# taintpro98/rnd-semantic-segmentation

Hardware: AMD Instinct MI355X
Metric: train images/sec at 769x769 bf16 (DeepLabV2-ResNet101 + ASPP) (higher is better)
Workload: dtype bf16; 1 GPU; train_src.py DeepLabV2-R101 bf16, 769x769 synthetic Cityscapes crops, batch 8 per GPU, 1xMI355X; global_batch=8, parallelism=dp1, weights=formula (synthetic), hip_graph_replay=False

## Files before the change

### include/mi355seg.h

```cpp
#ifndef MI355SEG_H
#define MI355SEG_H

#include <stddef.h>
#include <stdint.h>

#ifdef __cplusplus
extern "C" {
#endif

#define MI355SEG_VERSION 100

#define MI_OK 0
#define MI_EINVAL (-22)
#define MI_ENOMEM (-12)
#define MI_EHIP (-5)

#define MI_EPI_SCALE_BIAS 1
#define MI_EPI_RESIDUAL 2
#define MI_EPI_RELU 4
#define MI_EPI_MASK 8
#define MI_EPI_OUT_F32 16
#define MI_EPI_ZSPLIT 32
#define MI_EPI_WRITE_MASK 64
#define MI_EPI_LEAKY 256
// ... 57 lines not shown
                          const float* scale_o, int accumulate, int out_map, int ncls, size_t dw_elems,
                          void* workspace, size_t workspace_bytes, void* job, void* stream);
int mi_conv_wgrad_reduce(const void* jobs, int n, void* stream);

#define MI_ASPP_NRATES 4
#define MI_ASPP_ZGW 20
#define MI_ASPP_KPAD 704
int mi_aspp_pack_fwd(const float* w4 , void* wall_bf16, int C, int K, void* stream);
int mi_aspp_pack_dgrad(const float* w4, void* wallT_bf16, int C, int K, void* stream);
int mi_aspp_col2im(const float* z , const float* bias4 , float* low ,
                   int B, int H, int W, int K, const int* rates4 , void* stream);
int mi_aspp_im2col(const float* dlow , void* g_bf16 ,
                   int B, int H, int W, int K, const int* rates4 , void* stream);
size_t mi_colsum_workspace(int M, int N);
int mi_aspp_bias_grad(const float* dlow, float* dbias4 , int M, int K, int accumulate,
                      void* workspace, size_t workspace_bytes, void* stream);

int mi_upsample_ac_fwd(const float* low, float* up, int B, int h, int w, int K, int H, int W, void* stream);
int mi_upsample_ac_bwd(const float* dup, float* dlow, int B, int h, int w, int K, int H, int W, void* stream);

size_t mi_ce_workspace(int B, int H, int W);
int mi_softmax_ce_fwd(const float* logits, const int64_t* labels, float* loss_out ,
                      int B, int K, int H, int W, int ignore_index, void* workspace, size_t workspace_bytes, void* stream);
int mi_softmax_ce_bwd(const float* logits, const int64_t* labels, const float* loss_out, float* dlogits,
                      int B, int K, int H, int W, int ignore_index, float grad_scale, void* stream);

size_t mi_upsample_ce_workspace(int B, int h, int w, int K, int H, int W);
int mi_upsample_ce(const float* low, const int64_t* labels, float* loss_out , float* dlow,
                   int B, int h, int w, int K, int H, int W, int ignore_index, float grad_scale,
                   void* workspace, size_t workspace_bytes, void* stream);

int mi_upsample_ce_ex(const float* low, const int64_t* labels, float* loss_out , float* dlow,
                      int B, int h, int w, int K, int H, int W, int ignore_index, float grad_scale, int align_corners,
                      void* workspace, size_t workspace_bytes, void* stream);

int mi_upsample_ce_w(const float* low, const int64_t* labels, const float* class_weights , float* loss_out , float* dlow,
                     int B, int h, int w, int K, int H, int W, int ignore_index, float label_smoothing, float grad_scale, int align_corners,
                     void* workspace, size_t workspace_bytes, void* stream);

int mi_upsample_ce_focal(const float* low, const int64_t* labels, const float* class_weights , float* loss_out , float* dlow,
                         int B, int h, int w, int K, int H, int W, int ignore_index, float gamma, float grad_scale, int align_corners,
                         void* workspace, size_t workspace_bytes, void* stream);

size_t mi_upsample_ce_ohem_workspace(int B, int h, int w, int K, int H, int W);
int mi_upsample_ce_ohem(const float* low, const int64_t* labels, float* loss_out , float* dlow, float* prob ,
                        int B, int h, int w, int K, int H, int W, int ignore_index, float thresh, int64_t min_kept, float grad_scale,
                        int align_corners, void* workspace, size_t workspace_bytes, void* stream);

#define MI_GDL_SQUARE 0
#define MI_GDL_IDENTITY 1
#define MI_GDL_SQRT 2
size_t mi_upsample_gdl_workspace(int B, int h, int w, int K, int H, int W);
int mi_upsample_gdl(const float* low, const int64_t* labels, float* loss_out , float* dlow, float* sums ,
                    int B, int h, int w, int K, int H, int W, int ignore_index, int weight_type, float eps, float grad_scale,
                    int align_corners, void* workspace, size_t workspace_bytes, void* stream);

size_t mi_upsample_tversky_bce_workspace(int B, int h, int w, int H, int W);
int mi_upsample_tversky_bce(const float* low, const float* mask, float* loss_out , float* dlow, float* sums ,
                            int B, int h, int w, int H, int W, float alpha, float eps, float w_tversky, float w_bce, float grad_scale,
                            int align_corners, void* workspace, size_t workspace_bytes, void* stream);

int mi_upsample_softmax(const float* low, float* probs, uint8_t* pred, int B, int h, int w, int K, int H, int W, void* stream);

typedef struct { const float* low; int h, w; int mirror; } MiProbSource;
int mi_upsample_softmax_multi(const MiProbSource* src, int n, float* probs, int K, int H, int W, float div_a, float div_b, void* stream);

int mi_upsample_predict_score(const MiProbSource* src, int n, int K, int H, int W, float div_a, float div_b, const int64_t* labels,
                              int ignore_index, float threshold, uint8_t* pred, uint8_t* pseudo, int64_t* counts, void* stream);

int mi_upsample_predict_score_cw(const MiProbSource* src, int n, int K, int H, int W, float div_a, float div_b, const int64_t* labels,
                                 int ignore_index, const float* class_threshold, uint8_t* pred, uint8_t* pseudo, int64_t* counts, int bins,
                                 int64_t* hist, void* stream);

#define MI_POLYP_SUMS 24
#define MI_POLYP_COUNTS 4
size_t mi_polyp_score_workspace(int B, int h, int w, int H, int W);
int mi_polyp_score(const float* low, const int64_t* labels, int B, int h, int w, int H, int W, int64_t* hist, double* sums, int64_t* counts,
                   float* prob, uint8_t* pred, void* workspace, size_t workspace_bytes, void* stream);

int mi_image_resize_ac(const float* x, float* out, int B, int C, int H, int W, int Ho, int Wo, int with_mirror, void* stream);

int mi_sgd_step(float* p, const float* g, float* buf, size_t n, float lr, float momentum, float weight_decay, void* stream);
int mi_sgd_step_dev(float* p, const float* g, float* buf, size_t n, const float* hyper , void* stream);

int mi_stem_pool_fwd(const void* y, const float* scale, const float* shift, void* pool, uint8_t* idx,
                     int B, int Hc, int Wc, int C, int Hp, int Wp, void* stream);
int mi_stem_pool_bwd(const void* dpool, const uint8_t* idx, const float* scale, void* dy,
                     int B, int Hc, int Wc, int C, int Hp, int Wp, void* stream);
int mi_stem_im2col(const void* x_bf16_nhwc, void* col_bf16, int B, int H, int W, int Ho, int Wo, int ncols, void* stream);
int mi_stem_direct_enabled(void);
int mi_stem_pack_image(const void* x, int x_is_bf16_nhwc, void* x4, int B, int H, int W, void* stream);
int mi_stem_conv_fwd(const void* x4, const float* w, void* wpack, void* y, int B, int H, int W, int O, int Ho, int Wo, void* stream);
size_t mi_stem_conv_wgrad_workspace(int B, int Ho, int Wo);
int mi_stem_conv_wgrad(const void* dy, const void* x4, float* dw, int B, int H, int W, int O, int Ho, int Wo, void* workspace,
                       size_t workspace_bytes, void* stream);

int mi_bias_grad_bf16(const void* dy_bf16, float* db, int M, int N, int accumulate,
                      void* workspace , size_t workspace_bytes, void* stream);
size_t mi_upsample_softce_workspace(int B, int h, int w, int K, int H, int W);
int mi_upsample_softce(const float* seg_low, float inv_temperature, float clip, const float* d_low, int ldD, int domain,
                       float* loss_out, float* dd_low, int B, int h, int w, int K, int H, int W, float grad_scale,
                       void* workspace, size_t workspace_bytes, void* stream);
size_t mi_upsample_softce_2grid_workspace(int B, int hd, int wd, int K, int H, int W);
int mi_upsample_softce_2grid(const float* seg_low, int hs, int ws, int seg_align_corners, float inv_temperature, float clip,
                             const float* d_low, int hd, int wd, int ldD, int d_align_corners, int domain, float grad_scale,
                             float* loss_out, float* dd_low, int B, int K, int H, int W, void* workspace, size_t workspace_bytes, void* stream);
int mi_adam_step(float* p, const float* g, float* exp_avg, float* exp_avg_sq, size_t n, float lr, float beta1, float beta2,
                 float eps, int step, void* stream);
int mi_adam_step_clamped(float* p, float* g, float* exp_avg, float* exp_avg_sq, size_t n, float lr, float beta1, float beta2,
                         float eps, int step, float grad_clamp, void* stream);

int mi_adam_step_dev(float* p, float* g, float* exp_avg, float* exp_avg_sq, size_t n, const float* hyper , void* stream);

int mi_pack_weight_f32(const float* w_oihw, float* wp, int O, int I, int ksize, void* stream);
int mi_conv_f32(const float* a, const float* wp, float* out, int B, int Ha, int Wa, int Ca, int Ho, int Wo, int N,
                int ksize, int stride, int pad, int dil, const float* scale, const float* bias, const float* res,
                int flags, void* stream);
int mi_stem_f32(const float* x_nchw, const float* w, const float* scale, const float* shift, float* y_nhwc,
                int B, int H, int W, void* stream);
int mi_maxpool_f32(const float* y_nhwc, float* pool_nhwc, int B, int Hc, int Wc, int C, void* stream);

int mi_comm_unique_id(void* id128 );
int mi_comm_init_rank(void** comm , int nranks, const void* id128 , int rank);
int mi_comm_destroy(void* comm);
int mi_allreduce_bucket(void* ptr, size_t count, int dtype, int average, void* comm, void* stream);

int mi_relu_mask(const void* x_bf16, const void* msk, void* y_bf16, size_t n, int bits, void* stream);
int mi_frozen_bn_fold(const float* w, const float* b, const float* mean, const float* var, float* scale, float* shift, int n, void* stream);

size_t mi_bn_workspace(long M, int C);
int mi_bn_colsum(const void* y_bf16, const float* mean, long M, int C, float* out, void* workspace, size_t workspace_bytes, void* stream);
int mi_bn_colsum2(const void* y_bf16, const float* pilot, long M, int C, float* s1, float* s2, void* workspace, size_t workspace_bytes, void* stream);
size_t mi_conv_gemm_stats_workspace(long M, int N);
int mi_conv_gemm_stats(const void* a, const void* wp, void* out, int B, int Ha, int Wa, int Ca, int Ho, int Wo, int N, int ksize, int stride, int pad,
                       int dil, const float* pilot, float* sums, void* workspace, size_t workspace_bytes, const float* gamma, const float* beta,
                       float* running_mean, float* running_var, long long* num_batches_tracked, float momentum, float eps, float* out4, void* stream);
int mi_bn_finalize(const float* s1, const float* s2, const float* pilot, double count, const float* gamma, const float* beta, float* running_mean,
                   float* running_var, long long* num_batches_tracked, float momentum, float eps, float* out4, int C, void* stream);
int mi_bn_apply(const void* y_bf16, const float* mean, const float* scale, const float* beta, const void* res_bf16, void* out_bf16,
                void* mask_out, int relu, long M, int C, void* stream);
int mi_bn_bwd_colsums(const void* g_bf16, const void* y_bf16, const float* mean, const float* invstd, const void* relu_bits, long M, int C,
                      float* dbeta, float* dgamma, void* workspace, size_t workspace_bytes, void* stream);
int mi_bn_bwd_apply(const void* g_bf16, const void* y_bf16, const float* mean, const float* invstd, const float* gamma, const float* dbeta,
                    const float* dgamma, float inv_count, const void* relu_bits, void* dy_bf16, long M, int C, void* stream);

size_t mi_structure_loss_workspace(int B, int H, int W);
int mi_structure_loss(const float* pred, const float* mask, int B, int H, int W, float* out, float* grad, float grad_scale,
                      void* workspace, size_t workspace_bytes, void* stream);

size_t mi_gconv_pack_elems(int O, int I, int kh, int kw);
int mi_gconv_pack_multi(const float* wflat, void* wp_bf16, void* wpt_bf16, const int64_t* table_dev, int n_desc, int total_blocks, void* stream);
size_t mi_gconv_stats_elems(int B, int Ho, int Wo, int N);
int mi_gconv(const void* a, long lda, const void* wp, void* out, long ldo, int B, int Ha, int Wa, int Ca, int Ho, int Wo, int N,
             int kh, int kw, int sh, int sw, int ph, int pw, int dh, int dw, int mode, const float* bias, float* stats, int out_f32,
             void* stream);
#define MI_GROUTE_GCONV 0
#define MI_GROUTE_GCONV3 1
#define MI_GROUTE_LEN 10
int mi_gconv_route(const void* a, long lda, const void* out, long ldo, int B, int Ha, int Wa, int Ca, int Ho, int Wo, int N, int kh, int kw, int sh, int sw,
                   int ph, int pw, int dh, int dw, int mode, int out_f32, int bn_finalize, int* route);
size_t mi_gconv_wgrad_workspace(int B, int Ho, int Wo, int O, int I, int kh, int kw);
int mi_gconv_wgrad(const void* dy, long ldy, const void* x, long ldx, float* dw, int B, int Ha, int Wa, int I, int Ho, int Wo, int O,
                   int kh, int kw, int sh, int sw, int ph, int pw, int dh, int dw_, int accumulate, void* workspace, size_t workspace_bytes, unsigned* tickets, int n_tickets,
                   void* stream);
typedef struct MiWgradJob {
    const void* dy; long ldy; const void* x; long ldx; float* dw;
    int B, Ha, Wa, I, Ho, Wo, O, kh, kw, sh, sw, ph, pw, dh, dw_, accumulate;
} MiWgradJob;
size_t mi_gconv_wgrad_multi_table_bytes(int n);
size_t mi_gconv_wgrad_multi_workspace(const MiWgradJob* jobs, int n);
int mi_gconv_wgrad_multi(const MiWgradJob* jobs, int n, void* table_dev, size_t table_bytes, void* workspace, size_t workspace_bytes, void* stream);
#define MI_GWROUTE_LEN 6
int mi_gconv_wgrad_route(const void* dy, long ldy, const void* x, long ldx, int B, int Ha, int Wa, int I, int Ho, int Wo, int O, int kh, int kw, int sh, int sw,
                         int ph, int pw, int dh, int dw_, int multi, int* route);
int mi_gbn_finalize(const float* partials, int tiles, int C, long count, const float* gamma, const float* beta, float* running_mean, float* running_var,
                    float momentum, float eps, float* mean_out, float* invstd_out, float* scale_out, float* shift_out, void* stream);
int mi_gbn_fold(const float* gamma, const float* beta, const float* running_mean, const float* running_var, float eps, float* scale, float* shift, int C,
                void* stream);
int mi_gbn_apply(const void* y, long ldy, const float* scale, const float* shift, const void* add, long ldadd, void* out, long ldo, int out_f32, long M, int C,
                 int relu, void* stream);
int mi_gbn_apply_multi(const void* y, long ldy, const float* scale, const float* shift, const void* add, long ldadd, void* out, long ldo, long M, int C, int relu,
                       int n_extra, const int* c0, const int* c1, void* const* dst, const long* ldd, const void* const* add2, const long* lda2, void* stream);
size_t mi_gcolsum_workspace(long M, int C);
int mi_gbn_bwd_sums(const void* g, long ldg, int g_f32, const void* y, long ldy, const void* mask, long ldm, int mask_f32, const float* mean,
                    const float* invstd, long M, int C, float* dbeta, float* dgamma, int accumulate, void* workspace, size_t workspace_bytes, void* stream);
int mi_gbn_bwd_apply(const void* g, long ldg, int g_f32, const void* y, long ldy, const void* mask, long ldm, int mask_f32, const float* mean,
                     const float* invstd, const float* gamma, const float* dbeta, const float* dgamma, float inv_count, void* dy, long lddy, long M, int C,
                     void* stream);
int mi_gbinary(int op, int dtype, const void* a, long lda, const void* b, long ldb, void* out, long ldo, long M, int C, void* stream);
int mi_gavgpool(const void* x, long ldx, void* out, long ldo, int B, int H, int W, int C, int Ho, int Wo, int k, int stride, int pad, int include_pad,
                int backward, void* stream);
int mi_gmaxpool(const void* x, long ldx, void* out, long ldo, uint8_t* idx, int B, int H, int W, int C, int Ho, int Wo, int k, int stride, int pad, int backward,
                void* stream);
size_t mi_gce_workspace(long M);
int mi_gce(const float* logits, long ld, const int64_t* labels, long M, int K, int ignore_index, float* loss_out, float* dlogits, long ldd, float grad_scale,
           void* workspace, size_t workspace_bytes, void* stream);
int mi_gresize(const void* x, long ldx, void* out, long ldo, int f32, int B, int H, int W, int C, int Ho, int Wo, int align_corners, float scale_h, float scale_w,
               int backward, void* stream);
#define MI_GRESIZE_FWD 0
#define MI_GRESIZE_FWD8 1
#define MI_GRESIZE_BWD_GATHER 2
#define MI_GRESIZE_BWD_WAVE 3
#define MI_GRESIZE_BWD_PIX 4
#define MI_GRESIZE_BWD8 5
#define MI_GRESIZE_ROUTE_LEN 3
int mi_gresize_route(const void* x, long ldx, const void* out, long ldo, int f32, int B, int H, int W, int C, int Ho, int Wo, int align_corners, float scale_h,
                     float scale_w, int backward, int* route);
int mi_gra_fwd(const float* gate, const void* feat, long ldfeat, void* out, long ldo, long M, int C, void* stream);
int mi_gra_bwd(const float* gate, const void* feat, long ldfeat, const void* dy, long lddy, void* dfeat, long lddf, float* dgate, long M, int C, void* stream);

// ... 74 lines not shown
```

### rnd_semantic_segmentation_amd/_lib.py

```python
import ctypes
import os

import torch
from ctypes import c_char_p, c_double, c_float, c_int, c_long, c_size_t, c_void_p

_HERE = os.path.dirname(os.path.abspath(__file__))
LIB_PATH = os.environ.get("MI355SEG_LIB") or os.path.join(_HERE, "libmi355seg.so")
HEADER_PATH = os.path.join(os.path.dirname(_HERE), "include", "mi355seg.h")

P, I, F, Z, L = c_void_p, c_int, c_float, c_size_t, c_long

SIGNATURES = {
    "mi_version": (I, []),
    "mi_last_error": (c_char_p, []),
    "mi_pack_weight_fwd": (I, [P, P, I, I, I, P]),
    "mi_pack_weight_dgrad": (I, [P, P, P, I, I, I, P]),
    "mi_pack_weights_multi": (I, [P, P, P, P, P, I, I, P]),
    "mi_conv_gemm": (I, [P, P, P] + [I] * 12 + [P, P, P, P, P, I, I, F, P]),
    "mi_conv_gemm_route": (I, [I] * 10),
    "mi_conv_gemm_plan": (I, [I] * 13 + [P]),
    "mi_conv_gemm_pp": (I, [P, P, P] + [I] * 12 + [P, P, P, P, P, I, I, F, I, P]),
    "mi_conv_chain": (I, [P] * 6 + [L, I, I, I] + [P] * 8 + [I, I, P]),
    "mi_conv_wgrad_workspace": (Z, [I] * 6),
    "mi_conv_wgrad_route": (I, [I] * 12),
    "mi_conv_wgrad_plan": (I, [I] * 13 + [P]),
    "mi_conv_wgrad": (I, [P, P, P] + [I] * 11 + [P, I, I, I, Z, P, Z, P]),
    "mi_conv_wgrad_job_bytes": (Z, []),
    "mi_conv_wgrad_partial": (I, [P, P, P] + [I] * 11 + [P, I, I, I, Z, P, Z, P, P]),
    "mi_conv_wgrad_reduce": (I, [P, I, P]),
    "mi_aspp_pack_fwd": (I, [P, P, I, I, P]),
    "mi_aspp_pack_dgrad": (I, [P, P, I, I, P]),
    "mi_aspp_col2im": (I, [P, P, P, I, I, I, I, P, P]),
    "mi_aspp_im2col": (I, [P, P, I, I, I, I, P, P]),
    "mi_colsum_workspace": (Z, [I, I]),
    "mi_aspp_bias_grad": (I, [P, P, I, I, I, P, Z, P]),
    "mi_upsample_ac_fwd": (I, [P, P] + [I] * 6 + [P]),
    "mi_upsample_ac_bwd": (I, [P, P] + [I] * 6 + [P]),
    "mi_ce_workspace": (Z, [I, I, I]),
    "mi_softmax_ce_fwd": (I, [P, P, P, I, I, I, I, I, P, Z, P]),
    "mi_softmax_ce_bwd": (I, [P, P, P, P, I, I, I, I, I, F, P]),
    "mi_upsample_ce_workspace": (Z, [I] * 6),
    "mi_upsample_ce": (I, [P, P, P, P] + [I] * 7 + [F, P, Z, P]),
    "mi_upsample_ce_ex": (I, [P, P, P, P] + [I] * 7 + [F, I, P, Z, P]),
    "mi_upsample_ce_w": (I, [P, P, P, P, P] + [I] * 7 + [F, F, I, P, Z, P]),
    "mi_upsample_ce_focal": (I, [P, P, P, P, P] + [I] * 7 + [F, F, I, P, Z, P]),
    "mi_upsample_ce_ohem_workspace": (Z, [I] * 6),
    "mi_upsample_ce_ohem": (I, [P, P, P, P, P] + [I] * 7 + [F, L, F, I, P, Z, P]),
    "mi_upsample_gdl_workspace": (Z, [I] * 6),
    "mi_upsample_gdl": (I, [P, P, P, P, P] + [I] * 8 + [F, F, I, P, Z, P]),
    "mi_upsample_tversky_bce_workspace": (Z, [I] * 5),
    "mi_upsample_tversky_bce": (I, [P, P, P, P, P] + [I] * 5 + [F] * 5 + [I, P, Z, P]),
    "mi_upsample_softmax": (I, [P, P, P] + [I] * 6 + [P]),
    "mi_upsample_softmax_multi": (I, [P, I, P, I, I, I, F, F, P]),
    "mi_upsample_predict_score": (I, [P, I, I, I, I, F, F, P, I, F, P, P, P, P]),
    "mi_upsample_predict_score_cw": (I, [P, I, I, I, I, F, F, P, I, P, P, P, P, I, P, P]),
    "mi_polyp_score_workspace": (Z, [I] * 5),
    "mi_polyp_score": (I, [P, P] + [I] * 5 + [P, P, P, P, P, P, Z, P]),
    "mi_image_resize_ac": (I, [P, P] + [I] * 7 + [P]),
    "mi_stem_pool_fwd": (I, [P, P, P, P, P] + [I] * 6 + [P]),
    "mi_stem_pool_bwd": (I, [P, P, P, P] + [I] * 6 + [P]),
    "mi_stem_im2col": (I, [P, P] + [I] * 6 + [P]),
    "mi_stem_direct_enabled": (I, []),
    "mi_stem_pack_image": (I, [P, I, P, I, I, I, P]),
    "mi_stem_conv_fwd": (I, [P, P, P, P] + [I] * 6 + [P]),
    "mi_stem_conv_wgrad_workspace": (Z, [I] * 3),
    "mi_stem_conv_wgrad": (I, [P, P, P] + [I] * 6 + [P, Z, P]),
    "mi_bias_grad_bf16": (I, [P, P, I, I, I, P, Z, P]),
    "mi_upsample_softce_workspace": (Z, [I] * 6),
    "mi_upsample_softce": (I, [P, F, F, P, I, I, P, P] + [I] * 6 + [F, P, Z, P]),
    "mi_upsample_softce_2grid_workspace": (Z, [I] * 6),
    "mi_upsample_softce_2grid": (I, [P, I, I, I, F, F, P, I, I, I, I, I, F, P, P, I, I, I, I, P, Z, P]),
    "mi_adam_step": (I, [P, P, P, P, Z, F, F, F, F, I, P]),
    "mi_adam_step_clamped": (I, [P, P, P, P, Z, F, F, F, F, I, F, P]),
    "mi_adam_step_dev": (I, [P, P, P, P, Z, P, P]),
    "mi_sgd_step": (I, [P, P, P, Z, F, F, F, P]),
    "mi_sgd_step_dev": (I, [P, P, P, Z, P, P]),
    "mi_pack_weight_f32": (I, [P, P, I, I, I, P]),
    "mi_conv_f32": (I, [P, P, P] + [I] * 11 + [P, P, P, I, P]),
    "mi_stem_f32": (I, [P, P, P, P, P, I, I, I, P]),
    "mi_maxpool_f32": (I, [P, P, I, I, I, I, P]),
    "mi_comm_unique_id": (I, [P]),
    "mi_comm_init_rank": (I, [P, I, P, I]),
    "mi_comm_destroy": (I, [P]),
    "mi_allreduce_bucket": (I, [P, Z, I, I, P, P]),
    "mi_relu_mask": (I, [P, P, P, Z, I, P]),
    "mi_frozen_bn_fold": (I, [P, P, P, P, P, P, I, P]),
    "mi_structure_loss_workspace": (Z, [I, I, I]),
    "mi_structure_loss": (I, [P, P, I, I, I, P, P, F, P, Z, P]),
    "mi_bn_workspace": (Z, [L, I]),
    "mi_bn_colsum": (I, [P, P, L, I, P, P, Z, P]),
    "mi_bn_apply": (I, [P, P, P, P, P, P, P, I, L, I, P]),
    "mi_bn_colsum2": (I, [P, P, L, I, P, P, P, Z, P]),
    "mi_conv_gemm_stats_workspace": (Z, [L, I]),
    "mi_conv_gemm_stats": (I, [P, P, P] + [I] * 11 + [P, P, P, Z, P, P, P, P, P, F, F, P, P]),
    "mi_bn_finalize": (I, [P, P, P, c_double, P, P, P, P, P, F, F, P, I, P]),
    "mi_bn_bwd_colsums": (I, [P, P, P, P, P, L, I, P, P, P, Z, P]),
    "mi_bn_bwd_apply": (I, [P, P, P, P, P, P, P, F, P, P, L, I, P]),
    "mi_gconv_pack_elems": (Z, [I] * 4),
    "mi_gconv_pack_multi": (I, [P, P, P, P, I, I, P]),
    "mi_gconv_stats_elems": (Z, [I] * 4),
    "mi_gconv": (I, [P, L, P, P, L] + [I] * 16 + [P, P, I, P]),
    "mi_gconv_route": (I, [P, L, P, L] + [I] * 18 + [P]),
    "mi_gconv_wgrad_workspace": (Z, [I] * 7),
    "mi_gconv_wgrad": (I, [P, L, P, L, P] + [I] * 16 + [P, Z, P, I, P]),
    "mi_gconv_wgrad_multi_table_bytes": (Z, [I]),
    "mi_gconv_wgrad_multi_workspace": (Z, [P, I]),
    "mi_gconv_wgrad_multi": (I, [P, I, P, Z, P, Z, P]),
    "mi_gconv_wgrad_route": (I, [P, L, P, L] + [I] * 16 + [P]),
    "mi_gbn_finalize": (I, [P, I, I, L, P, P, P, P, F, F, P, P, P, P, P]),
    "mi_gbn_fold": (I, [P, P, P, P, F, P, P, I, P]),
    "mi_gbn_apply": (I, [P, L, P, P, P, L, P, L, I, L, I, I, P]),
    "mi_gbn_apply_multi": (I, [P, L, P, P, P, L, P, L, L, I, I, I, P, P, P, P, P, P, P]),
    "mi_gcolsum_workspace": (Z, [L, I]),
    "mi_gbn_bwd_sums": (I, [P, L, I, P, L, P, L, I, P, P, L, I, P, P, I, P, Z, P]),
    "mi_gbn_bwd_apply": (I, [P, L, I, P, L, P, L, I, P, P, P, P, P, F, P, L, L, I, P]),
    "mi_gbinary": (I, [I, I, P, L, P, L, P, L, L, I, P]),
    "mi_gavgpool": (I, [P, L, P, L] + [I] * 11 + [P]),
    "mi_gmaxpool": (I, [P, L, P, L, P] + [I] * 10 + [P]),
    "mi_gce_workspace": (Z, [L]),
    "mi_gce": (I, [P, L, P, L, I, I, P, P, L, F, P, Z, P]),
    "mi_gresize": (I, [P, L, P, L, I] + [I] * 7 + [F, F, I, P]),
    "mi_gresize_route": (I, [P, L, P, L, I] + [I] * 7 + [F, F, I, P]),
    "mi_gra_fwd": (I, [P, P, L, P, L, L, I, P]),
    "mi_gra_bwd": (I, [P, P, L, P, L, P, L, P, L, I, P]),
    "mi_gdwconv_stats_elems": (Z, [I] * 4),
    "mi_gdwconv": (I, [P, L, P, P, P, L] + [I] * 8 + [P, P]),
    "mi_gdwconv_dgrad": (I, [P, L, P, P, L] + [I] * 8 + [P]),
    "mi_gdwconv_wgrad_workspace": (Z, [I] * 4),
    "mi_gdwconv_wgrad": (I, [P, L, P, L, P, P] + [I] * 9 + [P, Z, P]),
    "mi_gcca_fwd": (I, [P, L, P, L, P, L, P, P, L] + [I] * 5 + [P]),
    "mi_gcca_bwd": (I, [P, L, P, L, P, L, P, P, L, P, P, L, P, L, P, L] + [I] * 5 + [P]),
    "mi_ggate": (I, [P, L, P, L, P, L, P, L, P, L, L, I, P]),
    "mi_gconv_bn_inlaunch_max_pixels": (I, []),
    "mi_gconv_bn": (I, [P, L, P, P, L] + [I] * 15 + [P, P, P, P, P, P, P, F, F, P, P]),
    "mi_gconv_f32": (I, [P, L, P, P, P, P, P, L, I, P, L] + [I] * 15 + [P]),
    "mi_gpool_f32": (I, [P, L, P, L] + [I] * 10 + [P]),
    "mi_gdwconv_f32": (I, [P, L, P, P, P, P, I, P, L] + [I] * 8 + [P]),
    "mi_gcca_f32": (I, [P, L, P, L, P, L, P, L] + [I] * 5 + [P]),
    "mi_gpoint_f32": (I, [I, P, L, P, L, P, P, I, P, L, L, I, P]),
    "mi_augment_batch": (I, [P, P, I, I, I, I, I, P, P, P]),
    "mi_augment_pra_batch": (I, [P, P, I, I, I, P, P, P]),
}

class MiProbSource(ctypes.Structure):
    _fields_ = [("low", c_void_p), ("h", c_int), ("w", c_int), ("mirror", c_int)]


class MiAugSample(ctypes.Structure):
    _fields_ = [("img", c_void_p), ("lab", c_void_p), ("jit", c_void_p), ("tmp", c_void_p), ("hcoef", c_void_p), ("hbound", c_void_p),
                ("vcoef", c_void_p), ("vbound", c_void_p), ("grey_sum", ctypes.c_uint64),
                ("H", c_int), ("W", c_int), ("sh", c_int), ("sw", c_int), ("hk", c_int), ("vk", c_int),
                ("off_y", c_int), ("off_x", c_int), ("flip", c_int),
                ("cy0", c_int), ("cy1", c_int), ("cx0", c_int), ("cx1", c_int), ("ry0", c_int), ("ry1", c_int), ("rx0", c_int), ("rx1", c_int),
                ("tstride", c_int), ("lab_sh", c_int), ("lab_sw", c_int),
                ("n_ops", c_int), ("op", c_int * 4), ("hue_shift", c_int), ("factor", c_float * 4),
                ("to_bgr255", c_int), ("mean", c_float * 3), ("std", c_float * 3), ("lab_table", ctypes.c_uint8 * 256)]


class MiPraSample(ctypes.Structure):
# ... 35 lines not shown
```

### rnd_semantic_segmentation_amd/csrc/elementwise.hip

```cpp
#include "mi_common.h"
#include <mutex>
#include <stdlib.h>
#include <string.h>

static thread_local char g_err[512] = "";

int mi_set_error(int code, const char* fmt, ...) {
    va_list ap;
    va_start(ap, fmt);
    vsnprintf(g_err, sizeof(g_err), fmt, ap);
    va_end(ap);
    return code;
}

const MiSwitches& mi_sw() {
    static MiSwitches sw;
    static std::once_flag once;
    std::call_once(once, [] {
        auto env = [](const char* name, int dflt) {
            const char* e = getenv(name);
            return e ? atoi(e) : dflt;
        };
        sw.igemm_staged = env("MI_IGEMM_STAGED", 1);
        sw.igemm_pp = env("MI_IGEMM_PP", 1);
        sw.igemm_pp_mink = env("MI_IGEMM_PP_MINK", 512);
        sw.igemm_mt = env("MI_IGEMM_MT", 0);
        sw.igemm_bn = env("MI_IGEMM_BN", 0);
        sw.igemm_pref = env("MI_IGEMM_PREF", 1);
        sw.pp_korder = env("MI_IGEMM_PP_KORDER", 1);
#ifdef MI_EXPERIMENTS
        sw.pp_loop = env("MI_IGEMM_PP_LOOP", 0);
#else
        sw.pp_loop = 0;
#endif
        sw.igemm_pw = env("MI_IGEMM_PW", 0);
        sw.wgrad_q3_slots = env("MI_WGRAD_Q3_SLOTS", 512);
        sw.wgrad_q3_slots_beside = env("MI_WGRAD_Q3_SLOTS_BESIDE", 448);
        sw.wgrad_s4_slots = env("MI_WGRAD_S4_SLOTS", 512);
        if (sw.wgrad_s4_slots < 64) sw.wgrad_s4_slots = 512;
        sw.wgrad_ti256 = env("MI_WGRAD_TI256", -1);
        sw.wgrad_p3 = env("MI_WGRAD_P3", 0);
        sw.wgrad_q3 = env("MI_WGRAD_Q3", 1);
        sw.wgrad_s4 = env("MI_WGRAD_S4", 1);
        sw.gconv_bn128 = env("MI_GCONV_BN128", 0);
        sw.gconv_kc = env("MI_GCONV_KC", 0);
        sw.gconv_remap = env("MI_GCONV_REMAP", 1);
        sw.gconv_ks2_wgs = env("MI_GCONV_KS2_WGS", 320);
        sw.gconv_kc32_wgs = env("MI_GCONV_KC32_WGS", 1536);
        sw.gconv_bn32_wgs = env("MI_GCONV_BN32_WGS", 256);
        sw.gconv_bn_any = env("MI_GCONV_BN_ANY", 1);
        sw.gconv_bn_c = env("MI_GCONV_BN_C", 64);
        sw.gconv_bn_force = env("MI_GCONV_BN_FORCE", 0);
        sw.gconv3_wgs = env("MI_GCONV3_WGS", 512);
#ifdef MI_EXPERIMENTS
        sw.gconv_dbg = env("MI_GC_DBG", 0);
        sw.gw_dbg = env("MI_GW_DBG", 0);
#else
        sw.gconv_dbg = sw.gw_dbg = 0;
#endif
        sw.gwm_steps = env("MI_GWM_STEPS", 48);
        if (sw.gwm_steps < 1) sw.gwm_steps = 48;
        sw.gwm_fused3 = env("MI_GWM_FUSED3", 1);
        sw.gwgrad3 = env("MI_GWGRAD3", 1);
#ifdef MI_EXPERIMENTS
        sw.p3_dbg = env("MI_P3_DBG", 0);
#else
        sw.p3_dbg = 0;
#endif
        sw.pp_trace_wg = env("MI_PP_TRACE_WG", 0);
        sw.stem_direct = env("MI_STEM_DIRECT", 1);
        sw.stem_wgrad_splits = env("MI_STEM_WGRAD_SPLITS", 512);
        if (sw.stem_wgrad_splits < 1 || sw.stem_wgrad_splits > 4096) sw.stem_wgrad_splits = 512;
    });
    return sw;
}

extern "C" int mi_version(void) { return MI355SEG_VERSION; }
extern "C" const char* mi_last_error(void) { return g_err; }

namespace {

__global__ void sgd_kernel(float* __restrict__ p, const float* __restrict__ g, float* __restrict__ buf, size_t n4, size_t n, float lr,
                           float mu, float wd) {
    const size_t stride = (size_t)gridDim.x * blockDim.x;
    for (size_t i = (size_t)blockIdx.x * blockDim.x + threadIdx.x; i < n4; i += stride) {
        f32x4 pv = reinterpret_cast<f32x4*>(p)[i];
        const f32x4 gv = reinterpret_cast<const f32x4*>(g)[i];
        f32x4 bv = reinterpret_cast<f32x4*>(buf)[i];
#pragma unroll
        for (int e = 0; e < 4; ++e) {
            const float gg = gv[e] + wd * pv[e];
            bv[e] = mu * bv[e] + gg;
            pv[e] = pv[e] - lr * bv[e];
        }
        reinterpret_cast<f32x4*>(buf)[i] = bv;
        reinterpret_cast<f32x4*>(p)[i] = pv;
    }
    if (blockIdx.x == 0 && threadIdx.x < (n & 3)) {
        const size_t i = (n4 << 2) + threadIdx.x;
        const float gg = g[i] + wd * p[i];
        const float b = mu * buf[i] + gg;
        buf[i] = b;
        p[i] = p[i] - lr * b;
    }
}

__global__ void sgd_dev_kernel(float* __restrict__ p, const float* __restrict__ g, float* __restrict__ buf, size_t n4, size_t n,
                               const float* __restrict__ hyper) {
    const float lr = hyper[0], mu = hyper[1], wd = hyper[2];
    const size_t stride = (size_t)gridDim.x * blockDim.x;
    for (size_t i = (size_t)blockIdx.x * blockDim.x + threadIdx.x; i < n4; i += stride) {
        f32x4 pv = reinterpret_cast<f32x4*>(p)[i];
        const f32x4 gv = reinterpret_cast<const f32x4*>(g)[i];
        f32x4 bv = reinterpret_cast<f32x4*>(buf)[i];
#pragma unroll
        for (int e = 0; e < 4; ++e) {
            const float gg = gv[e] + wd * pv[e];
            bv[e] = mu * bv[e] + gg;
            pv[e] = pv[e] - lr * bv[e];
        }
        reinterpret_cast<f32x4*>(buf)[i] = bv;
        reinterpret_cast<f32x4*>(p)[i] = pv;
    }
    if (blockIdx.x == 0 && threadIdx.x < (n & 3)) {
        const size_t i = (n4 << 2) + threadIdx.x;
        const float gg = g[i] + wd * p[i];
        const float b = mu * buf[i] + gg;
        buf[i] = b;
        p[i] = p[i] - lr * b;
    }
}

__global__ void relu_mask_kernel(const bf16x8* __restrict__ x, const bf16x8* __restrict__ m, bf16x8* __restrict__ y, size_t n8) {
    const size_t stride = (size_t)gridDim.x * blockDim.x;
    for (size_t i = (size_t)blockIdx.x * blockDim.x + threadIdx.x; i < n8; i += stride) {
        const bf16x8 xv = x[i], mv = m[i];
        bf16x8 o;
#pragma unroll
        for (int e = 0; e < 8; ++e) o[e] = ((float)mv[e] > 0.f) ? xv[e] : (__bf16)0.f;
        y[i] = o;
    }
}

__global__ void bn_fold_kernel(const float* w, const float* b, const float* mean, const float* var, float* scale, float* shift, int n) {
    const int i = blockIdx.x * blockDim.x + threadIdx.x;
    if (i >= n) return;
    const float s = w[i] * (1.0f / sqrtf(var[i]));
    scale[i] = s;
    shift[i] = b[i] - mean[i] * s;
}


extern "C" int mi_sgd_step(float* p, const float* g, float* buf, size_t n, float lr, float momentum, float weight_decay, void* stream) {
    MI_REQUIRE(p && g && buf && n > 0, "mi_sgd_step: bad argument");
    MI_REQUIRE(mi_aligned16(p) && mi_aligned16(g) && mi_aligned16(buf), "mi_sgd_step: flat buffers must be 16-byte aligned");
    const size_t n4 = n >> 2;
    size_t blocks = (n4 + 255) / 256;
    if (blocks > 2048) blocks = 2048;
    if (blocks < 1) blocks = 1;
    hipLaunchKernelGGL(sgd_kernel, dim3((unsigned)blocks), dim3(256), 0, (hipStream_t)stream, p, g, buf, n4, n, lr, momentum, weight_decay);
    MI_CHECK_LAUNCH("mi_sgd_step");
    return MI_OK;
}

extern "C" int mi_sgd_step_dev(float* p, const float* g, float* buf, size_t n, const float* hyper, void* stream) {
    MI_REQUIRE(p && g && buf && hyper && n > 0, "mi_sgd_step_dev: bad argument");
    MI_REQUIRE(mi_aligned16(p) && mi_aligned16(g) && mi_aligned16(buf), "mi_sgd_step_dev: flat buffers must be 16-byte aligned");
    const size_t n4 = n >> 2;
    size_t blocks = (n4 + 255) / 256;
    if (blocks > 2048) blocks = 2048;
    if (blocks < 1) blocks = 1;
    hipLaunchKernelGGL(sgd_dev_kernel, dim3((unsigned)blocks), dim3(256), 0, (hipStream_t)stream, p, g, buf, n4, n, hyper);
    MI_CHECK_LAUNCH("mi_sgd_step_dev");
    return MI_OK;
}

__global__ void relu_mask_bits_kernel(const bf16x8* __restrict__ x, const uint8_t* __restrict__ m, bf16x8* __restrict__ y, size_t n8) {
    const size_t stride = (size_t)gridDim.x * blockDim.x;
    for (size_t i = (size_t)blockIdx.x * blockDim.x + threadIdx.x; i < n8; i += stride) {
        const bf16x8 xv = x[i];
        const unsigned bits = m[i];
        bf16x8 o;
#pragma unroll
        for (int e = 0; e < 8; ++e) o[e] = ((bits >> e) & 1u) ? xv[e] : (__bf16)0.f;
        y[i] = o;
    }
}

}

extern "C" int mi_relu_mask(const void* x, const void* msk, void* y, size_t n, int bits, void* stream) {
    MI_REQUIRE(x && msk && y && n > 0 && n % 8 == 0, "mi_relu_mask: bad argument (n %% 8 == 0)");
    MI_REQUIRE(mi_aligned16(x) && mi_aligned16(y) && (bits || mi_aligned16(msk)), "mi_relu_mask: alignment");
    const size_t n8 = n >> 3;
    size_t blocks = (n8 + 255) / 256;
    if (blocks > 2048) blocks = 2048;
    if (bits) {
        MI_REQUIRE(n % 16 == 0, "mi_relu_mask: packed mask needs n %% 16 == 0");
        hipLaunchKernelGGL(relu_mask_bits_kernel, dim3((unsigned)blocks), dim3(256), 0, (hipStream_t)stream, (const bf16x8*)x,
                           (const uint8_t*)msk, (bf16x8*)y, n8);
        MI_CHECK_LAUNCH("mi_relu_mask (bits)");
        return MI_OK;
    }
    hipLaunchKernelGGL(relu_mask_kernel, dim3((unsigned)blocks), dim3(256), 0, (hipStream_t)stream, (const bf16x8*)x, (const bf16x8*)msk,
                       (bf16x8*)y, n8);
    MI_CHECK_LAUNCH("mi_relu_mask");
    return MI_OK;
}

extern "C" int mi_frozen_bn_fold(const float* w, const float* b, const float* mean, const float* var, float* scale, float* shift, int n,
                                 void* stream) {
    MI_REQUIRE(w && b && mean && var && scale && shift && n > 0, "mi_frozen_bn_fold: bad argument");
    hipLaunchKernelGGL(bn_fold_kernel, dim3((n + 255) / 256), dim3(256), 0, (hipStream_t)stream, w, b, mean, var, scale, shift, n);
    MI_CHECK_LAUNCH("mi_frozen_bn_fold");
    return MI_OK;
}
```

### rnd_semantic_segmentation_amd/csrc/mi_common.h

```cpp
#pragma once
#include <hip/hip_runtime.h>
#include <stdint.h>
#include <stdio.h>
#include <stdarg.h>
#include <atomic>
#include "../../include/mi355seg.h"

typedef __attribute__((ext_vector_type(8))) __bf16 bf16x8;
typedef __attribute__((ext_vector_type(4))) __bf16 bf16x4;
typedef __attribute__((ext_vector_type(2))) __bf16 bf16x2;
typedef __attribute__((ext_vector_type(4))) float f32x4;
typedef __attribute__((ext_vector_type(4))) short s16x4;
typedef __attribute__((ext_vector_type(4))) uint32_t u32x4;
typedef __attribute__((ext_vector_type(2))) uint32_t u32x2;

int mi_set_error(int code, const char* fmt, ...);

struct MiSwitches {
    int igemm_staged;
    int igemm_pp;
    int igemm_pp_mink;
    int igemm_mt;
    int igemm_bn;
    int igemm_pref;
    int pp_korder;
    int pp_loop;
    int igemm_pw;
    int wgrad_q3_slots;
    int wgrad_q3_slots_beside;
    int wgrad_s4_slots;
    int wgrad_ti256;
    int wgrad_p3;
    int wgrad_q3;
    int wgrad_s4;
    int gconv_bn128;
    int gconv_kc;
    int gconv_remap;
    int gconv_ks2_wgs;
    int gconv_kc32_wgs;
    int gconv_bn32_wgs;
    int gconv_bn_any;
    int gconv_bn_c;
    int gconv_bn_force;
    int gconv3_wgs;
    int gconv_dbg;
    int gw_dbg;
    int gwm_steps;
    int gwm_fused3;
    int gwgrad3;
    int p3_dbg;
    int pp_trace_wg;
    int stem_wgrad_splits;
    int stem_direct;
};
const MiSwitches& mi_sw();

struct MiConvStats {
    float* partial;
    const float* pilot;
    int nparts;
};
int mi_conv_gemm_impl(const void* a, const void* wp, void* out, int B, int Ha, int Wa, int Ca, int Ho, int Wo, int N, int ksize, int stride, int pad,
                      int dil, int gather_mode, const float* scale, const float* bias, const void* res, const void* msk, void* mask_out, int flags,
                      int zgw, float alpha, void* stream, MiConvStats* st);
int mi_conv_gemm_pp_impl(const void* a, const void* wp, void* out, int B, int Ha, int Wa, int Ca, int Ho, int Wo, int N, int ksize, int stride, int pad,
                         int dil, int gather_mode, const float* scale, const float* bias, const void* res, const void* msk, void* mask_out, int flags,
                         int zgw, float alpha, int mtg, void* stream, MiConvStats* st);
struct MiConvPlan {
    int kernel;
    int mt;
    int bn;
    int unit, pref, staged;
    int epi;
    int korder;
    int m_tiles, n_tiles;
    int slots, rounds;
};
int mi_conv_plan(int B, int Ha, int Wa, int Ca, int Ho, int Wo, int N, int ksize, int stride, int pad, int dil, int flags, int pp_mtg, MiConvPlan* pl);
struct MiBnFinal {
    const float* pilot;
    double count;
    const float* gamma;
    const float* beta;
    float* running_mean;
    float* running_var;
    long long* num_batches_tracked;
    float momentum, eps;
    float* out4;
};
size_t mi_bn_reduce_tmp_floats(int nparts, int C);
int mi_bn_reduce_partials(const float* partial, int nparts, int C, float* tmp, float* s1, float* s2, const MiBnFinal* fin, void* stream);

#define MI_REQUIRE(cond, ...)                         \
    do {                                              \
        if (!(cond)) return mi_set_error(MI_EINVAL, __VA_ARGS__); \
    } while (0)

#define MI_CHECK_LAUNCH(name)                                                      \
    do {                                                                           \
        hipError_t e_ = hipGetLastError();                                         \
        if (e_ != hipSuccess) return mi_set_error(MI_EHIP, "%s: %s", name, hipGetErrorString(e_)); \
    } while (0)

static inline void mi_allow_dynamic_lds(const void* kern, int bytes, std::atomic<uint64_t>& done) {
    int dev = 0;
    (void)hipGetDevice(&dev);
    const uint64_t bit = 1ull << (dev & 63);
    if (done.load(std::memory_order_acquire) & bit) return;
    (void)hipFuncSetAttribute(kern, hipFuncAttributeMaxDynamicSharedMemorySize, bytes);
    done.fetch_or(bit, std::memory_order_release);
}
constexpr int MI_LDS_MAX = 160 * 1024;

static inline bool mi_aligned16(const void* p) { return (reinterpret_cast<uintptr_t>(p) & 15) == 0; }

__device__ __forceinline__ int mi_xcd_remap(int bid, int nwg) {
    const int q = nwg >> 3, r = nwg & 7, xcd = bid & 7;
    const int base = (xcd < r) ? xcd * (q + 1) : r * (q + 1) + (xcd - r) * q;
    return base + (bid >> 3);
}

__device__ __forceinline__ float mi_bf16_to_f32(__bf16 v) { return (float)v; }

struct MiBnFin {
    float mean, invstd, scale, shift;
    double var;
};
__device__ __forceinline__ MiBnFin mi_bn_finalize_channel(double s1, double s2, double count, float eps, float gamma, float beta) {
    MiBnFin r;
    const double mean = s1 / count;
    double var = __dsub_rn(s2 / count, __dmul_rn(mean, mean));
    if (var < 0.0) var = 0.0;
    r.var = var;
    r.mean = (float)mean;
    r.invstd = (float)(1.0 / sqrt(__dadd_rn(var, (double)eps)));
    r.scale = __fmul_rn(gamma, r.invstd);
// ... 43 lines not shown
```

### rnd_semantic_segmentation_amd/csrc/stem_direct.hip

```cpp
#include "mi_common.h"

namespace {

constexpr int SD_TW = 64;
constexpr int SD_ROWPX = 136;
constexpr int SD_ROWB = SD_ROWPX * 8;
constexpr int SD_FWD_TH = 8;
constexpr int SD_FWD_ROWS = 2 * SD_FWD_TH + 5;
constexpr int SD_KB = 6;
constexpr int SD_WG_TH = 4;
constexpr int SD_WG_ROWS = 2 * SD_WG_TH + 5;
constexpr int SD_DYROWB = SD_TW * 128;
constexpr int SD_PART = 64 * 7 * 32;

__global__ __launch_bounds__(256) void stem_pack_f32_kernel(const float* __restrict__ x, bf16x4* __restrict__ x4, long HW, int B) {
    const int b = blockIdx.y;
    const float* img = x + (long)b * 3 * HW;
    const long p0 = (long)blockIdx.x * 1024 + threadIdx.x;
    float v[4][3];
#pragma unroll
    for (int j = 0; j < 4; ++j) {
        const long p = p0 + j * 256;
#pragma unroll
        for (int c = 0; c < 3; ++c) v[j][c] = p < HW ? img[c * HW + p] : 0.f;
    }
#pragma unroll
    for (int j = 0; j < 4; ++j) {
        const long p = p0 + j * 256;
        if (p < HW) {
            bf16x4 o;
            o[0] = (__bf16)v[j][0];
            o[1] = (__bf16)v[j][1];
            o[2] = (__bf16)v[j][2];
            o[3] = (__bf16)0.f;
            x4[(long)b * HW + p] = o;
        }
    }
}

__global__ __launch_bounds__(256) void stem_pack_bf16_kernel(const __bf16* __restrict__ x, bf16x4* __restrict__ x4, long n) {
    const long p = (long)blockIdx.x * 256 + threadIdx.x;
    if (p >= n) return;
    bf16x4 o;
    o[0] = x[p * 3];
    o[1] = x[p * 3 + 1];
    o[2] = x[p * 3 + 2];
    o[3] = (__bf16)0.f;
    x4[p] = o;
}

__global__ __launch_bounds__(256) void stem_pack_weight_kernel(const float* __restrict__ w, __bf16* __restrict__ wp) {
    const int i = blockIdx.x * 256 + threadIdx.x;
    if (i >= SD_KB * 64 * 32) return;
    const int kk = i & 31, o = (i >> 5) & 63, kb = i >> 11;
    const int k = kb * 32 + kk;
    wp[i] = (__bf16)(k < 147 ? w[o * 147 + k] : 0.f);
}

template <int ROWS>
struct ImageRows {
    static constexpr int N = (ROWS * SD_ROWPX + 255) / 256;
    uint2 v[N];
    __device__ __forceinline__ void load(const uint2* __restrict__ img, int h0, int c0, int H, int W, int tid) {
#pragma unroll
        for (int j = 0; j < N; ++j) {
            const int i = tid + j * 256;
            const int r = i / SD_ROWPX, c = i - r * SD_ROWPX;
            const int h = h0 + r, w = c0 + c;
            v[j] = make_uint2(0u, 0u);
            if (i < ROWS * SD_ROWPX && (unsigned)h < (unsigned)H && (unsigned)w < (unsigned)W) v[j] = img[(long)h * W + w];
        }
    }
    __device__ __forceinline__ void store(uint2* sx, int tid) const {
#pragma unroll
        for (int j = 0; j < N; ++j) {
            const int i = tid + j * 256;
            if (i < ROWS * SD_ROWPX) sx[i] = v[j];
        }
    }
};

struct StemFwdParams {
    const uint2* x4;
    const bf16x8* wp;
    __bf16* y;
    int B, H, W, Ho, Wo, tiles_x, tiles_y;
};

__global__ __launch_bounds__(256, 2) void stem_direct_fwd_kernel(StemFwdParams p) {
    __shared__ __attribute__((aligned(16))) uint2 sx[SD_FWD_ROWS * SD_ROWPX];
    const int tid = threadIdx.x, lane = tid & 63;
    const int wave = __builtin_amdgcn_readfirstlane(tid >> 6);
    const int tx = blockIdx.x % p.tiles_x, ty = (blockIdx.x / p.tiles_x) % p.tiles_y, b = blockIdx.x / (p.tiles_x * p.tiles_y);
    const int wo0 = tx * SD_TW, ho0 = ty * SD_FWD_TH;
    ImageRows<SD_FWD_ROWS> rows;
    rows.load(p.x4 + (long)b * p.H * p.W, 2 * ho0 - 3, 2 * wo0 - 3, p.H, p.W, tid);

    const int col = lane & 15, q = lane >> 4;
    bf16x8 wf[SD_KB - 1][4];
#pragma unroll
    for (int kb = 0; kb < SD_KB - 1; ++kb)
#pragma unroll
        for (int ot = 0; ot < 4; ++ot) wf[kb][ot] = p.wp[(kb * 64 + (col >> 2) * 16 + ot * 4 + (col & 3)) * 4 + q];
    int off[SD_KB - 1][8];
#pragma unroll
    for (int kb = 0; kb < SD_KB - 1; ++kb)
#pragma unroll
        for (int j = 0; j < 8; ++j) {
            const int k = kb * 32 + q * 8 + j;
            const int c = k / 49, r = k - c * 49, ky = r / 7, kx = r - ky * 7;
            off[kb][j] = k < 147 ? ky * SD_ROWB + kx * 8 + c * 2 : -1;
        }
    rows.store(sx, tid);
    __syncthreads();

    const char* sxb = reinterpret_cast<const char*>(sx);
    bf16x8 zero8;
#pragma unroll
    for (int e = 0; e < 8; ++e) zero8[e] = (__bf16)0.f;
    for (int rr = wave * 2; rr < wave * 2 + 2; ++rr) {
        const int ho = ho0 + rr;
        if (ho >= p.Ho) break;
        for (int mt = 0; mt < 4; ++mt) {
            if (wo0 + mt * 16 >= p.Wo) break;
            const char* win = sxb + 2 * rr * SD_ROWB + 16 * (mt * 16 + col);
            f32x4 acc[4];
#pragma unroll
            for (int ot = 0; ot < 4; ++ot) acc[ot] = f32x4{0.f, 0.f, 0.f, 0.f};
#pragma unroll
            for (int kb = 0; kb < SD_KB - 1; ++kb) {
                union { bf16x8 v; unsigned short s[8]; } f;
#pragma unroll
                for (int j = 0; j < 8; ++j) {
                    if (kb < 4) {
                        f.s[j] = *reinterpret_cast<const unsigned short*>(win + off[kb][j]);
                    } else {
                        const unsigned short v = *reinterpret_cast<const unsigned short*>(win + (off[kb][j] < 0 ? 0 : off[kb][j]));
                        f.s[j] = off[kb][j] < 0 ? (unsigned short)0 : v;
                    }
                }
#pragma unroll
                for (int ot = 0; ot < 4; ++ot) acc[ot] = __builtin_amdgcn_mfma_f32_16x16x32_bf16(wf[kb][ot], f.v, acc[ot], 0, 0, 0);
            }
#pragma unroll
            for (int ot = 0; ot < 4; ++ot) acc[ot] = __builtin_amdgcn_mfma_f32_16x16x32_bf16(zero8, zero8, acc[ot], 0, 0, 0);
            const int wo = wo0 + mt * 16 + col;
            if (wo < p.Wo) {
                bf16x8 o0, o1;
#pragma unroll
                for (int e = 0; e < 4; ++e) {
                    o0[e] = (__bf16)acc[0][e];
                    o0[4 + e] = (__bf16)acc[1][e];
                    o1[e] = (__bf16)acc[2][e];
                    o1[4 + e] = (__bf16)acc[3][e];
                }
                bf16x8* dst = reinterpret_cast<bf16x8*>(p.y + (((long)b * p.Ho + ho) * p.Wo + wo) * 64 + q * 16);
                dst[0] = o0;
                dst[1] = o1;
            }
        }
    }
}

template <int OFF>
__device__ __forceinline__ s16x4 sd_tr_read(unsigned lds_addr) {
    s16x4 v;
    asm volatile("ds_read_b64_tr_b16 %0, %1 offset:%2" : "=v"(v) : "v"(lds_addr), "n"(OFF));
    return v;
}

__device__ __forceinline__ unsigned sd_lds_address(const void* generic_ptr_into_lds) {
    return (unsigned)(uintptr_t)((__attribute__((address_space(3))) const char*)generic_ptr_into_lds);
}

struct StemWgradParams {
    const uint2* x4;
    const bf16x8* dy;
    float* part;
    int B, H, W, Ho, Wo, tiles_x, tiles_y, tiles, S;
};

__global__ __launch_bounds__(256, 2) void stem_direct_wgrad_kernel(StemWgradParams p) {
    __shared__ __attribute__((aligned(16))) uint2 sx[SD_WG_ROWS * SD_ROWPX];
    __shared__ __attribute__((aligned(16))) bf16x8 sdy[SD_WG_TH * SD_TW * 8];
    const int tid = threadIdx.x, lane = tid & 63;
    const int wave = __builtin_amdgcn_readfirstlane(tid >> 6);
    const int kt = wave & 1, oh = wave >> 1;
    const int s = blockIdx.x;
    const int t_begin = (int)((long)s * p.tiles / p.S), t_end = (int)((long)(s + 1) * p.tiles / p.S);
    const int g = lane >> 4, rq = (lane & 15) >> 2, pc = lane & 3;
    const int pix = 4 * g + rq;
    const unsigned sx_base = sd_lds_address(sx) + 16 * pix + 32 * kt + 8 * pc;
    const unsigned sdy_base = sd_lds_address(sdy) + 128 * pix + 8 * (pc & 1);
    const int sw = pix & 7;

    f32x4 acc[2][7];
#pragma unroll
    for (int a = 0; a < 2; ++a)
#pragma unroll
        for (int ky = 0; ky < 7; ++ky) acc[a][ky] = f32x4{0.f, 0.f, 0.f, 0.f};

    ImageRows<SD_WG_ROWS> nx;
    bf16x8 ny[8];
    auto load_tile = [&](int t) {
        const int tx = t % p.tiles_x, ty = (t / p.tiles_x) % p.tiles_y, b = t / (p.tiles_x * p.tiles_y);
        const int wo0 = tx * SD_TW, ho0 = ty * SD_WG_TH;
        nx.load(p.x4 + (long)b * p.H * p.W, 2 * ho0 - 3, 2 * wo0 - 3, p.H, p.W, tid);
#pragma unroll
        for (int j = 0; j < 8; ++j) {
            const int i = tid + j * 256;
            const int c = i & 7, P = (i >> 3) & 63, rr = i >> 9;
            const int ho = ho0 + rr, wo = wo0 + P;
#pragma unroll
            for (int e = 0; e < 8; ++e) ny[j][e] = (__bf16)0.f;
            if (ho < p.Ho && wo < p.Wo) ny[j] = p.dy[(((long)b * p.Ho + ho) * p.Wo + wo) * 8 + c];
        }
    };
    load_tile(t_begin);
    for (int t = t_begin; t < t_end; ++t) {
        const int tx = t % p.tiles_x, ty = (t / p.tiles_x) % p.tiles_y;
        const int wo0 = tx * SD_TW, ho0 = ty * SD_WG_TH;
        __syncthreads();
        nx.store(sx, tid);
#pragma unroll
        for (int j = 0; j < 8; ++j) {
            const int i = tid + j * 256;
            const int c = i & 7, P = (i >> 3) & 63, rr = i >> 9;
            sdy[(rr * SD_TW + P) * 8 + (c ^ (P & 7))] = ny[j];
        }
        __syncthreads();
        if (t + 1 < t_end) load_tile(t + 1);
        const int nrows = min(SD_WG_TH, p.Ho - ho0);
        for (int rr = 0; rr < nrows; ++rr) {
#pragma unroll
            for (int step = 0; step < 2; ++step) {
                const int left = p.Wo - (wo0 + step * 32);
                if (left <= 0) break;
                union { bf16x8 v; s16x4 h[2]; uint64_t d[2]; } yf[2], xf[7];
                const unsigned ya = sdy_base + rr * SD_DYROWB + step * 32 * 128;
#pragma unroll
                for (int a = 0; a < 2; ++a) {
                    const unsigned addr = ya + (((2 * (oh * 2 + a) + (pc >> 1)) ^ sw) << 4);
                    yf[a].h[0] = sd_tr_read<0>(addr);
                    yf[a].h[1] = sd_tr_read<16 * 128>(addr);
                }
                const unsigned xa = sx_base + 2 * rr * SD_ROWB + step * 32 * 16;
#pragma unroll
                for (int ky = 0; ky < 7; ++ky) {
                    xf[ky].h[0] = sd_tr_read<0>(xa + ky * SD_ROWB);
                    xf[ky].h[1] = sd_tr_read<16 * 16>(xa + ky * SD_ROWB);
                }
                asm volatile("s_waitcnt lgkmcnt(0)" ::: "memory");
                __builtin_amdgcn_sched_barrier(0);
                if (left < 32) {
#pragma unroll
                    for (int h = 0; h < 2; ++h) {
                        const int nv = left - (16 * h + 4 * g);
                        const uint64_t m = nv >= 4 ? ~0ull : (nv <= 0 ? 0ull : ((1ull << (16 * nv)) - 1ull));
#pragma unroll
                        for (int ky = 0; ky < 7; ++ky) xf[ky].d[h] &= m;
                    }
                }
#pragma unroll
                for (int ky = 0; ky < 7; ++ky)
#pragma unroll
                    for (int a = 0; a < 2; ++a) acc[a][ky] = __builtin_amdgcn_mfma_f32_16x16x32_bf16(yf[a].v, xf[ky].v, acc[a][ky], 0, 0, 0);
            }
        }
    }
    float* dst = p.part + (long)s * SD_PART;
#pragma unroll
    for (int a = 0; a < 2; ++a)
#pragma unroll
        for (int ky = 0; ky < 7; ++ky)
#pragma unroll
            for (int e = 0; e < 4; ++e) dst[(((oh * 2 + a) * 16 + 4 * g + e) * 7 + ky) * 32 + kt * 16 + (lane & 15)] = acc[a][ky][e];
}

__global__ __launch_bounds__(256) void stem_direct_wgrad_reduce_kernel(const float* __restrict__ part, float* __restrict__ dw, int S) {
    const int i = blockIdx.x * 256 + threadIdx.x;
    if (i >= SD_PART) return;
    const int k = i & 31, ky = (i >> 5) % 7, o = i / 224;
    const int kx = k >> 2, c = k & 3;
    if (c == 3 || kx >= 7) return;
    float sum = 0.f;
    int s = 0;
    for (; s + 64 <= S; s += 64) {
        float v[64];
#pragma unroll
        for (int j = 0; j < 64; ++j) v[j] = part[(long)(s + j) * SD_PART + i];
#pragma unroll
        for (int j = 0; j < 64; ++j) sum += v[j];
    }
    for (; s < S; ++s) sum += part[(long)s * SD_PART + i];
    dw[((o * 3 + c) * 7 + ky) * 7 + kx] = sum;
}

int stem_wgrad_splits(int B, int Ho, int Wo) {
    const long tiles = (long)B * ((Ho + SD_WG_TH - 1) / SD_WG_TH) * ((Wo + SD_TW - 1) / SD_TW);
    const long slots = mi_sw().stem_wgrad_splits;
    return (int)(tiles < slots ? tiles : slots);
}

const char* stem_direct_geometry(int B, int H, int W, int Ho, int Wo) {
    if (B <= 0 || H <= 0 || W <= 0) return "B, H, W must be positive";
    if (Ho != (H + 6 - 7) / 2 + 1 || Wo != (W + 6 - 7) / 2 + 1) return "output size must be that of a 7x7/2/3 conv";
    if ((long)B * H * W * 4 >= (1l << 31) || (long)B * Ho * Wo * 64 >= (1l << 31)) return "tensor exceeds the 32-bit offset range";
    return nullptr;
}

}

extern "C" int mi_stem_direct_enabled(void) { return mi_sw().stem_direct != 0; }

extern "C" int mi_stem_pack_image(const void* x, int x_is_bf16_nhwc, void* x4, int B, int H, int W, void* stream) {
    MI_REQUIRE(x && x4 && B > 0 && H > 0 && W > 0, "mi_stem_pack_image: bad argument");
    MI_REQUIRE(x_is_bf16_nhwc == 0 || x_is_bf16_nhwc == 1, "mi_stem_pack_image: x_is_bf16_nhwc=%d (0: fp32 NCHW, 1: bf16 NHWC)", x_is_bf16_nhwc);
    MI_REQUIRE((reinterpret_cast<uintptr_t>(x4) & 7) == 0 && (reinterpret_cast<uintptr_t>(x) & (x_is_bf16_nhwc ? 1 : 3)) == 0, "mi_stem_pack_image: alignment");
    MI_REQUIRE((long)B * H * W * 4 < (1l << 31), "mi_stem_pack_image: tensor exceeds the 32-bit offset range");
    MI_REQUIRE(B < 65536, "mi_stem_pack_image: B = %d exceeds the grid", B);
    const long HW = (long)H * W;
    if (x_is_bf16_nhwc)
        hipLaunchKernelGGL(stem_pack_bf16_kernel, dim3((unsigned)((B * HW + 255) / 256)), dim3(256), 0, (hipStream_t)stream, (const __bf16*)x, (bf16x4*)x4,
                           B * HW);
    else
        hipLaunchKernelGGL(stem_pack_f32_kernel, dim3((unsigned)((HW + 1023) / 1024), (unsigned)B), dim3(256), 0, (hipStream_t)stream, (const float*)x,
                           (bf16x4*)x4, HW, B);
    MI_CHECK_LAUNCH("mi_stem_pack_image");
    return MI_OK;
}

extern "C" int mi_stem_conv_fwd(const void* x4, const float* w, void* wpack, void* y, int B, int H, int W, int O, int Ho, int Wo, void* stream) {
    MI_REQUIRE(x4 && w && wpack && y, "mi_stem_conv_fwd: null operand");
    MI_REQUIRE(O == 64, "mi_stem_conv_fwd: O=%d (the stem has 64 output channels)", O);
    const char* bad = stem_direct_geometry(B, H, W, Ho, Wo);
    MI_REQUIRE(!bad, "mi_stem_conv_fwd: %s", bad);
    MI_REQUIRE((reinterpret_cast<uintptr_t>(x4) & 7) == 0 && mi_aligned16(wpack) && mi_aligned16(y), "mi_stem_conv_fwd: alignment");
    hipLaunchKernelGGL(stem_pack_weight_kernel, dim3(SD_KB * 64 * 32 / 256), dim3(256), 0, (hipStream_t)stream, w, (__bf16*)wpack);
    MI_CHECK_LAUNCH("mi_stem_conv_fwd (weight pack)");
    StemFwdParams p;
    p.x4 = (const uint2*)x4;
    p.wp = (const bf16x8*)wpack;
    p.y = (__bf16*)y;
    p.B = B, p.H = H, p.W = W, p.Ho = Ho, p.Wo = Wo;
    p.tiles_x = (Wo + SD_TW - 1) / SD_TW;
    p.tiles_y = (Ho + SD_FWD_TH - 1) / SD_FWD_TH;
    hipLaunchKernelGGL(stem_direct_fwd_kernel, dim3((unsigned)(B * p.tiles_x * p.tiles_y)), dim3(256), 0, (hipStream_t)stream, p);
    MI_CHECK_LAUNCH("mi_stem_conv_fwd");
    return MI_OK;
}

extern "C" size_t mi_stem_conv_wgrad_workspace(int B, int Ho, int Wo) {
    if (B <= 0 || Ho <= 0 || Wo <= 0) return 0;
    return (size_t)stem_wgrad_splits(B, Ho, Wo) * SD_PART * sizeof(float);
}

extern "C" int mi_stem_conv_wgrad(const void* dy, const void* x4, float* dw, int B, int H, int W, int O, int Ho, int Wo, void* workspace,
                                  size_t workspace_bytes, void* stream) {
    MI_REQUIRE(dy && x4 && dw && workspace, "mi_stem_conv_wgrad: null operand");
    MI_REQUIRE(O == 64, "mi_stem_conv_wgrad: O=%d (the stem has 64 output channels)", O);
    const char* bad = stem_direct_geometry(B, H, W, Ho, Wo);
    MI_REQUIRE(!bad, "mi_stem_conv_wgrad: %s", bad);
    MI_REQUIRE((reinterpret_cast<uintptr_t>(x4) & 7) == 0 && mi_aligned16(dy) && mi_aligned16(workspace) && (reinterpret_cast<uintptr_t>(dw) & 3) == 0,
               "mi_stem_conv_wgrad: alignment");
    MI_REQUIRE(workspace_bytes >= mi_stem_conv_wgrad_workspace(B, Ho, Wo), "mi_stem_conv_wgrad: workspace holds %zu bytes, %zu needed", workspace_bytes,
               mi_stem_conv_wgrad_workspace(B, Ho, Wo));
    StemWgradParams p;
    p.x4 = (const uint2*)x4;
    p.dy = (const bf16x8*)dy;
    p.part = (float*)workspace;
    p.B = B, p.H = H, p.W = W, p.Ho = Ho, p.Wo = Wo;
    p.tiles_x = (Wo + SD_TW - 1) / SD_TW;
    p.tiles_y = (Ho + SD_WG_TH - 1) / SD_WG_TH;
    p.tiles = B * p.tiles_x * p.tiles_y;
    p.S = stem_wgrad_splits(B, Ho, Wo);
    hipLaunchKernelGGL(stem_direct_wgrad_kernel, dim3((unsigned)p.S), dim3(256), 0, (hipStream_t)stream, p);
    MI_CHECK_LAUNCH("mi_stem_conv_wgrad");
    hipLaunchKernelGGL(stem_direct_wgrad_reduce_kernel, dim3(SD_PART / 256), dim3(256), 0, (hipStream_t)stream, (const float*)workspace, dw, p.S);
    MI_CHECK_LAUNCH("mi_stem_conv_wgrad (reduce)");
    return MI_OK;
}
```

### rnd_semantic_segmentation_amd/csrc/upsample_ce.hip

```cpp
#include "upsample_common.h"

namespace {

__global__ void upsample_fwd_kernel(const float* __restrict__ low, float* __restrict__ up, int B, int K, Axis ay, Axis ax) {
    const long idx = (long)blockIdx.x * blockDim.x + threadIdx.x;
    const int H = ay.n_out, W = ax.n_out, h = ay.n_in, w = ax.n_in;
    if (idx >= (long)B * H * W) return;
    const int x = (int)(idx % W), y = (int)((idx / W) % H), b = (int)(idx / ((long)W * H));
    int y0, y1, x0, x1;
    float ly, lx;
    ay.src(y, y0, y1, ly);
    ax.src(x, x0, x1, lx);
    const float* p00 = low + (((long)b * h + y0) * w + x0) * K;
    const float* p01 = low + (((long)b * h + y0) * w + x1) * K;
    const float* p10 = low + (((long)b * h + y1) * w + x0) * K;
    const float* p11 = low + (((long)b * h + y1) * w + x1) * K;
    float* o = up + ((long)b * K * H + y) * W + x;
    for (int k = 0; k < K; ++k) o[(long)k * H * W] = lerp2(p00[k], p01[k], p10[k], p11[k], lx, ly);
}

__global__ void upsample_bwd_kernel(const float* __restrict__ dup, float* __restrict__ dlow, int B, int K, Axis ay, Axis ax) {
    const long idx = (long)blockIdx.x * blockDim.x + threadIdx.x;
    const int H = ay.n_out, W = ax.n_out, h = ay.n_in, w = ax.n_in;
    if (idx >= (long)B * K * h * w) return;
    const int j = (int)(idx % w), i = (int)((idx / w) % h), k = (int)((idx / ((long)w * h)) % K), b = (int)(idx / ((long)w * h * K));
    const int ya = ay.first_with_i0_ge(i - 1), yb = ay.first_with_i0_ge(i + 1);
    const int xa = ax.first_with_i0_ge(j - 1), xb = ax.first_with_i0_ge(j + 1);
    const float* src = dup + ((long)b * K + k) * H * W;
    float s = 0.f;
    for (int y = ya; y < yb; ++y) {
        int y0, y1;
        float ly;
        ay.src(y, y0, y1, ly);
        const float wy = (y0 == i ? 1.f - ly : 0.f) + (y1 == i ? ly : 0.f);
        if (wy == 0.f && y0 != i && y1 != i) continue;
        float r = 0.f;
        for (int x = xa; x < xb; ++x) {
            int x0, x1;
            float lx;
            ax.src(x, x0, x1, lx);
            const float wx = (x0 == j ? 1.f - lx : 0.f) + (x1 == j ? lx : 0.f);
            r += wx * src[(long)y * W + x];
        }
        s += wy * r;
    }
    dlow[(((long)b * h + i) * w + j) * K + k] = s;
}

__device__ __forceinline__ void count_bad_label(long lab, int K, int ignore_index, unsigned* bad) {
    if (lab != ignore_index && (lab < 0 || lab >= K)) atomicAdd(bad, 1u);
}

__global__ void ce_fwd_kernel(const float* __restrict__ logits, const int64_t* __restrict__ labels, float* __restrict__ partial,
                              int B, int K, long HW, int ignore_index, unsigned* __restrict__ bad) {
    __shared__ float red[512];
    const long idx = (long)blockIdx.x * 256 + threadIdx.x;
    float loss = 0.f, cnt = 0.f;
    if (idx < (long)B * HW) {
        const long b = idx / HW, pix = idx - b * HW;
        const long lab = labels[idx];
        count_bad_label(lab, K, ignore_index, bad);
        if (lab != ignore_index && lab >= 0 && lab < K) {
            const float* p = logits + b * K * HW + pix;
            float mx = p[0];
            for (int k = 1; k < K; ++k) mx = fmaxf(mx, p[k * HW]);
            float se = 0.f;
            for (int k = 0; k < K; ++k) se += __expf(p[k * HW] - mx);
            loss = (mx + __logf(se)) - p[lab * HW];
            cnt = 1.f;
        }
    }
    block_sum2(loss, cnt, red);
    if (threadIdx.x == 0) {
        partial[2 * blockIdx.x] = loss;
        partial[2 * blockIdx.x + 1] = cnt;
    }
}

__global__ void ce_finalize_kernel(const float* __restrict__ partial, int n, float* __restrict__ loss_out) {
    __shared__ float red[512];
    float s = 0.f, c = 0.f;
    for (int i = threadIdx.x; i < n; i += 256) {
        s += partial[2 * i];
        c += partial[2 * i + 1];
    }
    block_sum2(s, c, red);
    if (threadIdx.x == 0) {
        loss_out[0] = s / c;
        loss_out[1] = c;
        loss_out[2] = (float)*reinterpret_cast<const unsigned*>(loss_out + 3);
    }
}

__global__ void ce_bwd_kernel(const float* __restrict__ logits, const int64_t* __restrict__ labels, const float* __restrict__ loss_out,
                              float* __restrict__ dlogits, int B, int K, long HW, int ignore_index, float grad_scale) {
    const long idx = (long)blockIdx.x * 256 + threadIdx.x;
    if (idx >= (long)B * HW) return;
    const long b = idx / HW, pix = idx - b * HW;
    const long lab = labels[idx];
    const float* p = logits + b * K * HW + pix;
    float* d = dlogits + b * K * HW + pix;
    if (lab == ignore_index || lab < 0 || lab >= K) {
        for (int k = 0; k < K; ++k) d[k * HW] = 0.f;
        return;
    }
    const float inv = grad_scale / loss_out[1];
    float mx = p[0];
    for (int k = 1; k < K; ++k) mx = fmaxf(mx, p[k * HW]);
    float se = 0.f;
    for (int k = 0; k < K; ++k) se += __expf(p[k * HW] - mx);
    const float rse = 1.f / se;
    for (int k = 0; k < K; ++k) d[k * HW] = (__expf(p[k * HW] - mx) * rse - (k == lab ? 1.f : 0.f)) * inv;
}

enum { UPCE_PLAIN = 0, UPCE_WEIGHTED = 1, UPCE_FOCAL = 2 };
struct WceArgs {
    const float* cw;
    float keep;
    float smooth;
};

struct WeightedSum {
    const float* w;
    float& s;
    __device__ __forceinline__ void operator()(int k, float zk) const { s += w[k] * zk; }
};

__host__ __device__ inline TileLds upce_lds(int npx_max, int K, int mode) {
    return TileLds(npx_max, K, true, mode == UPCE_WEIGHTED ? K + 1 : mode == UPCE_FOCAL ? K : 0);
}

__device__ __forceinline__ void focal_factors(float gamma, float u, float q, float nll, float& ug, float& m) {
    ug = u > 0.f ? exp2f(gamma * log2f(u)) : 0.f;
    const float ratio = u > 1e-30f ? nll / u : 1.f;
    m = ug * (1.f + gamma * (q * ratio));
}
__host__ __device__ inline TileLds grad_lds(int npx_max, int K) {
    return TileLds(npx_max, K, false, 0);
}

template <int KT, int MODE = UPCE_PLAIN>
__global__ __launch_bounds__(256) void upce_pass1_kernel(const float* __restrict__ low, const int64_t* __restrict__ labels,
                                                         float* __restrict__ partial, float* __restrict__ tmp, int B, int Krt, Axis ay,
                                                         Axis ax, int ignore_index, int npx_max, unsigned* __restrict__ bad, int jt_cols, WceArgs wce) {
    const int K = KT > 0 ? KT : Krt;
    constexpr int KR = kreg<KT>;
    const XTile t = xtile_begin(upce_lds(npx_max, K, MODE), low, K, ay, ax, npx_max, jt_cols);
    float* wsh = t.extra;
    if constexpr (MODE == UPCE_FOCAL) {
        if (threadIdx.x < K) wsh[threadIdx.x] = wce.cw ? wce.cw[threadIdx.x] : 1.f;
    }
    if constexpr (MODE == UPCE_WEIGHTED) {
        if (threadIdx.x < K) wsh[threadIdx.x] = wce.cw ? wce.cw[threadIdx.x] : 1.f;
        __syncthreads();
        if (threadIdx.x == 0) {
            float s = 0.f;
            for (int k = 0; k < K; ++k) s += wsh[k];
            wsh[K] = s;
        }
    }
    __syncthreads();
    float loss = 0.f, cnt = 0.f;
    for (int px = threadIdx.x; px < t.npx; px += 256) {
        const XPixel q = xtile_pixel(t, ax, K, px);
        const long lab = labels[q.pix];
// ... 890 lines not shown
```

### rnd_semantic_segmentation_amd/host/engine.py

```python
import contextlib
import os

import torch

from .. import kernels as K
from . import arch


class FlatStore:

    ALIGN = 64

    def __init__(self, named_params, device):
        self.names = [n for n, _ in named_params]
        self.params = [p for _, p in named_params]
        self.offsets = []
        off = 0
        for p in self.params:
            self.offsets.append(off)
            off += -(-p.numel() // self.ALIGN) * self.ALIGN
        self.total = off
        self.data = torch.zeros(off, dtype=torch.float32, device=device)
        self.grad = torch.zeros(off, dtype=torch.float32, device=device)
        self.written = set()
# ... 59 lines not shown
    def on(cls, device):
        if os.environ.get("MI_WGRAD_STREAM", "1") == "0" or device.type != "cuda":
            return cls(None)
        if K.PROFILE is not None:
            return cls(None)
        key = device.index if device.index is not None else torch.cuda.current_device()
        if key not in cls._streams:
            cls._streams[key] = torch.cuda.Stream(device=torch.device("cuda", key))
        return cls(cls._streams[key])

    def run(self, fn, *keep):
        if self.side is None:
            fn()
            return
        self.side.wait_stream(torch.cuda.current_stream())
        with torch.cuda.stream(self.side):
            fn()
        for t in keep:
            t.record_stream(self.side)
        self.dirty = True

    def end_block(self, batch, store, params):
        if batch is not None:
            self.run(batch.flush)
        if store is not None and store.grad_hooks:
            lo, hi = store.span(params)
            with torch.cuda.stream(self.side) if self.side is not None else contextlib.nullcontext():
                for hook in store.grad_hooks:
                    hook(store, lo, hi)

    def join(self):
        if self.dirty:
            torch.cuda.current_stream().wait_stream(self.side)
            self.dirty = False


class _Lanes:
    _by_device = {}

    @classmethod
    def get(cls, device, batch):
        if os.environ.get("MI_BATCH_LANES", "2") != "2" or device.type != "cuda" or batch < 2 or batch % 2 or K.PROFILE is not None:
            return None
        key = device.index if device.index is not None else torch.cuda.current_device()
        if key not in cls._by_device:
            cls._by_device[key] = torch.cuda.Stream(device=torch.device("cuda", key))
        return cls._by_device[key]


def bn_fold(bn):
    eps = float(getattr(bn, "eps", 0.0) or 0.0)
    var = bn.running_var if eps == 0.0 else bn.running_var + eps
    return K.frozen_bn_fold(bn.weight.detach(), bn.bias.detach(), bn.running_mean, var)


def bn_versions(bn):
    return bn.weight._version + bn.bias._version + bn.running_mean._version + bn.running_var._version


class _ConvRT:
    __slots__ = ("spec", "weight", "bn", "scale", "shift", "wp", "wpt")

    def __init__(self, spec, weight, bn):
        self.spec, self.weight, self.bn = spec, weight, bn
        self.scale = self.shift = self.wp = self.wpt = None


class StageEngine:

    def __init__(self, owner, plan):
        self.owner = owner
        self.plan = plan
        self.blocks = []
        for blk in plan:
            rts = []
            for c in arch.block_convs(blk):
                rts.append(_ConvRT(c, arch.node_at(owner.backbone, c.key).weight, arch.node_at(owner.backbone, c.bn)))
            self.blocks.append((blk, rts))
        self.convs = [rt for _, rts in self.blocks for rt in rts]
        self._bn_sig = None
        self._pack_sig = None
        self._have_dgrad = False
        self.batch_stats = False

    def _signature(self):
        store = getattr(self.convs[0].weight, "_mi_store", None)
        gen = store.generation if store is not None else -1
        return (gen, sum(rt.weight._version for rt in self.convs), self.convs[0].weight.data_ptr())

    def _build_pack_plan(self, store):
        dev = store.data.device
        n = sum(rt.weight.numel() for rt in self.convs)
        self._wp_flat = torch.empty(n, dtype=torch.bfloat16, device=dev)
        self._wpt_flat = torch.empty(n, dtype=torch.bfloat16, device=dev)
        self._scale_flat = torch.empty(sum(rt.spec.cout for rt in self.convs), dtype=torch.float32, device=dev)
        self._shift_flat = torch.empty_like(self._scale_flat)
        rows, off, soff, blk = [], 0, 0, 0
        for rt in self.convs:
            c = rt.spec
            T = c.k * c.k
            assert T <= 9, "mi_pack_weights_multi packs 1x1 and 3x3 convs"
            rows.append([rt.weight._mi_off, soff, off, off, c.cout, c.cin, T, blk])
            rt.wp = self._wp_flat[off:off + rt.weight.numel()].view(T, c.cout, c.cin)
            rt.wpt = self._wpt_flat[off:off + rt.weight.numel()].view(T, c.cin, c.cout)
            rt.scale = self._scale_flat[soff:soff + c.cout]
            rt.shift = self._shift_flat[soff:soff + c.cout]
            off += rt.weight.numel()
            soff += c.cout
            blk += -(-c.cout // 32) * -(-c.cin // 128)
        self._pack_blocks = blk
        self._table_train = torch.tensor(rows, dtype=torch.int64, device=dev)
        self._table_batch = torch.tensor([r[:1] + [-1] + r[2:] for r in rows], dtype=torch.int64, device=dev)
        for r in rows:
            r[3] = -1
        self._table_eval = torch.tensor(rows, dtype=torch.int64, device=dev)
        self._plan_store = store

    def prepare(self, train):
        store = getattr(self.convs[0].weight, "_mi_store", None)
        if store is None or not store.intact():
            raise RuntimeError("backbone parameters are not in their flat store; call ensure_flat() after moving the module")
        if getattr(self, "_plan_store", None) is not store:
            self._build_pack_plan(store)
            self._bn_sig = self._pack_sig = None
        refold = False
        if not self.batch_stats:
            bn_sig = (sum(bn_versions(rt.bn) for rt in self.convs), self.convs[0].bn.weight.data_ptr())
            refold = bn_sig != self._bn_sig
            if refold:
                for rt in self.convs:
                    sc, sh = bn_fold(rt.bn)
                    rt.scale.copy_(sc)
                    rt.shift.copy_(sh)
                self._bn_sig = bn_sig
        sig = self._signature() + (self.batch_stats,)
        if sig != self._pack_sig or refold or (train and not self._have_dgrad):
            table = self._table_batch if self.batch_stats else (self._table_train if train else self._table_eval)
            K.pack_weights_multi(store.data, self._scale_flat, self._wp_flat, self._wpt_flat, table, len(self.convs), self._pack_blocks)
            self._pack_sig = sig
            self._have_dgrad = train

    @staticmethod
    def chain_mode():
        return os.environ.get("MI_CHAIN", "0")

    def _chain_pair(self, bi):
        if bi < 0 or bi + 1 >= len(self.blocks) or self.batch_stats:
            return None
        (_, rts), (nblk, nrts) = self.blocks[bi], self.blocks[bi + 1]
        c3, c1 = rts[2].spec, nrts[0].spec
        ok = (not nblk.down and c3.k == 1 and c1.k == 1 and c3.stride == 1 and c1.stride == 1 and (c3.cin, c3.cout) == (256, 1024)
              and (c1.cin, c1.cout) == (1024, 256))
        return (rts[2], nrts[0]) if ok else None

    @staticmethod
    def _chain_fits(x):
        return x.is_cuda and x.shape[0] * x.shape[1] * x.shape[2] * 2048 < 2 ** 31

    @staticmethod
    def _fwd_conv(x, rt, relu, res=None, want_mask=False):
        c = rt.spec
        hw = arch.out_hw(x.shape[1], x.shape[2], c)
        bits = torch.empty((x.shape[0], hw[0], hw[1], c.cout // 16), dtype=torch.int16, device=x.device) if want_mask else None
        y = K.conv_gemm(x, rt.wp, hw, c.k, c.stride, c.pad, c.dil, K.GATHER_FWD, scale=rt.scale, bias=rt.shift, res=res, relu=relu,
                        mask_out=bits)
        return (y, bits) if want_mask else y

    @staticmethod
    def _conv_into(x, rt, relu, y, bits=None, res=None):
        c = rt.spec
        K.conv_gemm(x, rt.wp, (y.shape[1], y.shape[2]), c.k, c.stride, c.pad, c.dil, K.GATHER_FWD, scale=rt.scale, bias=rt.shift, res=res,
                    relu=relu, mask_out=bits, out=y)

    def _forward_lanes(self, x, save, extra):
        B, dev = x.shape[0], x.device
        halves = (slice(0, B // 2), slice(B // 2, B))
        main = torch.cuda.current_stream()

        def new(like_hw, ch, dtype=torch.bfloat16):
            return torch.empty((B, like_hw[0], like_hw[1], ch), dtype=dtype, device=dev)

        plan, hw = [], (x.shape[1], x.shape[2])
        for blk, rts in self.blocks:
            hw1 = arch.out_hw(hw[0], hw[1], rts[0].spec)
            hw2 = arch.out_hw(hw1[0], hw1[1], rts[1].spec)
            hw3 = arch.out_hw(hw2[0], hw2[1], rts[2].spec)
            t = {"a1": new(hw1, rts[0].spec.cout), "a2": new(hw2, rts[1].spec.cout), "out": new(hw3, rts[2].spec.cout),
                 "idn": new(arch.out_hw(hw[0], hw[1], rts[3].spec), rts[3].spec.cout) if blk.down else None}
            if save:
                t.update(b1=new(hw1, rts[0].spec.cout // 16, torch.int16), b2=new(hw2, rts[1].spec.cout // 16, torch.int16),
                         ob=new(hw3, rts[2].spec.cout // 16, torch.int16))
            plan.append(t)
            hw = hw3
        fork = torch.cuda.Event()
        fork.record(main)
        extra.wait_event(fork)
        xin = x
        chain = save and self.chain_mode() in ("all", "fwd") and self._chain_fits(x)
        ahead = False
        for bi, ((blk, rts), t) in enumerate(zip(self.blocks, plan)):
            pair = self._chain_pair(bi) if chain else None
            tn = plan[bi + 1] if pair is not None else None
            for lane, h in enumerate(halves):
                with torch.cuda.stream(extra) if lane else contextlib.nullcontext():
                    sl = lambda name: None if t.get(name) is None else t[name][h]
                    if not ahead:
                        self._conv_into(xin[h], rts[0], True, sl("a1"), sl("b1"))
                    self._conv_into(sl("a1"), rts[1], True, sl("a2"), sl("b2"))
                    if blk.down:
                        self._conv_into(xin[h], rts[3], False, sl("idn"))
                    res = sl("idn") if blk.down else xin[h]
                    if pair is not None:
                        K.conv_chain(sl("a2"), pair[0].wp, res, pair[1].wp, pair[0].scale, pair[0].shift, pair[1].scale, pair[1].shift,
                                     mid=sl("out"), out=tn["a1"][h], bits1_out=sl("ob"), bits2_out=tn["b1"][h])
                    else:
                        self._conv_into(sl("a2"), rts[2], True, sl("out"), sl("ob"), res=res)
            ahead = pair is not None
            xin = t["out"]
        main.wait_stream(extra)
        saved, xbits, xin = [], None, x
        if save:
            for t in plan:
                saved.append((xin, t["a1"], t["a2"], xbits, t["b1"], t["b2"]))
                xbits, xin = t["ob"], t["out"]
        return plan[-1]["out"], saved, (plan[-1]["ob"] if save else None)

    def forward(self, x, save):
        extra = _Lanes.get(x.device, x.shape[0])
        if extra is not None:
            return self._forward_lanes(x, save, extra)
        saved = []
        xbits = None
        chain = save and self.chain_mode() in ("all", "fwd") and self._chain_fits(x)
        ahead = None
        for bi, (blk, rts) in enumerate(self.blocks):
            if ahead is not None:
                a1, b1 = ahead
                a2, b2 = self._fwd_conv(a1, rts[1], True, want_mask=True)
            elif save:
                a1, b1 = self._fwd_conv(x, rts[0], True, want_mask=True)
                a2, b2 = self._fwd_conv(a1, rts[1], True, want_mask=True)
            else:
                a1 = self._fwd_conv(x, rts[0], True)
                a2 = self._fwd_conv(a1, rts[1], True)
                b1 = b2 = None
            idn = self._fwd_conv(x, rts[3], False) if blk.down else x
            pair = self._chain_pair(bi) if chain else None
            ahead = None
            if pair is not None:
                out, a1n, obits, b1n = K.conv_chain(a2, pair[0].wp, idn, pair[1].wp, pair[0].scale, pair[0].shift, pair[1].scale, pair[1].shift)
                ahead = (a1n, b1n)
                saved.append((x, a1, a2, xbits, b1, b2))
                xbits = obits
            elif save:
                out, obits = self._fwd_conv(a2, rts[2], True, res=idn, want_mask=True)
                saved.append((x, a1, a2, xbits, b1, b2))
                xbits = obits
            else:
                out = self._fwd_conv(a2, rts[2], True, res=idn)
            x = out
        return x, saved, xbits

    @staticmethod
    def _wgrad(dy, xin, rt, batch=None):
        c = rt.spec
        dw, acc = grad_slot(rt.weight)
        K.conv_wgrad(dy, xin, dw, c.k, c.stride, c.pad, c.dil, scale=rt.scale, accumulate=acc, batch=batch)

    @staticmethod
    def _dgrad(dy, rt, in_hw, res=None, bits=None):
        c = rt.spec
        return K.conv_gemm(dy, rt.wpt, in_hw, c.k, c.stride, c.pad, c.dil, K.GATHER_DGRAD, res=res, bits=bits)

    def backward(self, saved, fbits, dfeat, need_dx):
        g = K.relu_mask(dfeat, fbits)
        store = getattr(self.convs[0].weight, "_mi_store", None)
        sched = WgradScheduler.on(dfeat.device)
        chain = self.chain_mode() in ("all", "bwd") and self._chain_fits(dfeat)
        ga2_ahead = None
        for bi in range(len(self.blocks) - 1, -1, -1):
            blk, rts = self.blocks[bi]
            x, a1, a2, xb, b1, b2 = saved[bi]
            first = bi == 0
            hw_in = (x.shape[1], x.shape[2])
            hw_mid = (a1.shape[1], a1.shape[2])
            wb = K.WgradBatch() if K.PROFILE is None else None
            sched.run(lambda: self._wgrad(g, a2, rts[2], wb), g, a2)
            if ga2_ahead is not None:
                ga2, ga2_ahead = ga2_ahead, None
            else:
                ga2 = self._dgrad(g, rts[2], (a2.shape[1], a2.shape[2]), bits=b2)
            sched.run(lambda: self._wgrad(ga2, a1, rts[1], wb), ga2, a1)
            ga1 = self._dgrad(ga2, rts[1], hw_mid, bits=b1)
            if blk.down:
                sched.run(lambda: self._wgrad(g, x, rts[3], wb), g, x)
            sched.run(lambda: self._wgrad(ga1, x, rts[0], wb), ga1, x)
            sched.end_block(wb, store, [rt.weight for rt in rts])
            pair = self._chain_pair(bi - 1) if chain and not first and not blk.down else None
            if first and not need_dx:
                g = None
            elif pair is not None:
                g, ga2_ahead = K.conv_chain(ga1, rts[0].wpt, g, pair[0].wpt, bits1=xb, bits2=saved[bi - 1][5])
            else:
                skip = self._dgrad(g, rts[3], hw_in) if blk.down else g
                g = self._dgrad(ga1, rts[0], hw_in, res=skip, bits=None if first else xb)
            saved[bi] = None
        sched.join()
        return g



    @staticmethod
    def _bn_unit(x, rt, relu, res=None):
        c = rt.spec
        synced = _bn_synced(rt.bn)
        y, sums, fin = K.conv_gemm_stats(x, rt.wp, arch.out_hw(x.shape[1], x.shape[2], c), c.k, c.stride, c.pad, c.dil, bn_pilot(rt.bn, x.device),
                                         bn=None if synced else rt.bn)
        if synced:
            fin, count = bn_batch_statistics(y, rt.bn, (sums[0], sums[1]))
        else:
            count = y.numel() // y.shape[-1]
        if relu:
            out, bits = K.bn_apply(y, fin[0], fin[2], rt.bn.bias.detach(), res=res, relu=True, want_mask=True)
        else:
            out, bits = K.bn_apply(y, fin[0], fin[2], rt.bn.bias.detach(), res=res, relu=False), None
        return out, y, fin, count, bits

    def forward_batchnorm(self, x):
        saved, xbits = [], None
        for blk, rts in self.blocks:
            u1 = self._bn_unit(x, rts[0], True)
            u2 = self._bn_unit(u1[0], rts[1], True)
            ud = self._bn_unit(x, rts[3], False) if blk.down else None
            u3 = self._bn_unit(u2[0], rts[2], True, res=ud[0] if blk.down else x)
            saved.append((x, xbits, [u1, u2, u3, ud]))
            x, xbits = u3[0], u3[4]
        return x, saved, xbits

    def backward_batchnorm(self, saved, fbits, dfeat, need_dx):
        g = K.relu_mask(dfeat, fbits)
        store = getattr(self.convs[0].weight, "_mi_store", None)
        sched = WgradScheduler.on(dfeat.device)

        def wgrad(dy, xin, rt, wb):
            c = rt.spec

            def go():
                dw, acc = grad_slot(rt.weight)
                K.conv_wgrad(dy, xin, dw, c.k, c.stride, c.pad, c.dil, accumulate=acc, batch=wb)
            sched.run(go, dy, xin)

        for bi in range(len(self.blocks) - 1, -1, -1):
            blk, rts = self.blocks[bi]
            x, xb, (u1, u2, u3, ud) = saved[bi]
            first = bi == 0
            hw_in = (x.shape[1], x.shape[2])
            wb = K.WgradBatch() if K.PROFILE is None else None
            dy3 = bn_backward(g, u3[1], u3[2], u3[3], rts[2].bn)
# ... 128 lines not shown
        self._sig = sig

    def _conv(self, x, c, relu, res=None):
        wp, sc, sh = self._packs[c.key]
        return K.conv_f32(x, wp, arch.out_hw(x.shape[1], x.shape[2], c), c.k, c.stride, c.pad, c.dil, scale=sc, bias=sh, res=res, relu=relu)

    def forward(self, x):
        self.prepare()
        w, sc, sh = self._stem
        y = K.maxpool_f32(K.stem_f32(x.contiguous(), w, sc, sh))
        for blk in self.plan:
            c1, c2, c3 = arch.block_convs(blk)[:3]
            a1 = self._conv(y, c1, True)
            a2 = self._conv(a1, c2, True)
            idn = self._conv(y, arch.block_convs(blk)[3], False) if blk.down else y
            y = self._conv(a2, c3, True, res=idn)
        return y


class Fp32Aspp:

    def __init__(self, owner, rates):
        self.owner, self.rates = owner, rates
        self._sig = None

    def prepare(self):
        convs = [getattr(self.owner.conv2d_list, str(i)) for i in range(4)]
        store = getattr(convs[0].weight, "_mi_store", None)
        sig = (store.generation if store is not None else -1, sum(c.weight._version + c.bias._version for c in convs), convs[0].weight.data_ptr())
        if sig != self._sig:
            self._wp = [K.pack_weight_f32(c.weight.detach().contiguous()) for c in convs]
            self._b = [c.bias.detach().contiguous() for c in convs]
            self._sig = sig

    def forward(self, x):
        self.prepare()
        h, w = x.shape[1], x.shape[2]
        out = None
        for wp, b, d in zip(self._wp, self._b, self.rates):
            out = K.conv_f32(x, wp, (h, w), 3, 1, d, d, bias=b, res=out)
        return out


def stem_conv_forward(x, weight):
    if K.stem_direct_enabled():
        x4 = K.stem_pack_image(x)
        return K.stem_conv_direct(x4, weight), (x4,)
    y, col = K.stem_conv_fwd(x.to(dtype=torch.bfloat16).contiguous(memory_format=torch.channels_last), weight)
    return y, (col,)


def stem_conv_wgrad(dy_nhwc, saved):
    if K.stem_direct_enabled():
        return K.stem_wgrad_direct(dy_nhwc, saved[0])
    return K.stem_wgrad(dy_nhwc, col=saved[0])


class StemConvFn(torch.autograd.Function):

    @staticmethod
    def forward(ctx, x, weight):
        y, saved = stem_conv_forward(x, weight)
        ctx.save_for_backward(*saved)
        return y

    @staticmethod
    def backward(ctx, dy):
        return None, stem_conv_wgrad(dy.contiguous(), ctx.saved_tensors)


class StemFn(torch.autograd.Function):

    @staticmethod
    def forward(ctx, x, weight, scale, shift):
        y, saved = stem_conv_forward(x, weight)
        pool, idx = K.stem_pool_fwd(y, scale, shift)
        ctx.save_for_backward(idx, scale, *saved)
        ctx.conv_hw = (y.shape[1], y.shape[2])
        return pool

    @staticmethod
    def backward(ctx, dpool):
        idx, scale = ctx.saved_tensors[:2]
        dy = K.stem_pool_bwd(dpool.contiguous(), idx, scale, ctx.conv_hw)
        return None, stem_conv_wgrad(dy, ctx.saved_tensors[2:]), None, None


class StagesFn(torch.autograd.Function):

    @staticmethod
    def forward(ctx, x, eng, *weights):
        train = any(ctx.needs_input_grad)
        eng.prepare(train)
        feat, saved, fbits = eng.forward(x, save=train)
        ctx.eng, ctx.saved, ctx.fbits = eng, saved, fbits
        return feat

    @staticmethod
    def backward(ctx, dfeat):
        dfeat = dfeat.contiguous()
        dx = ctx.eng.backward(ctx.saved, ctx.fbits, dfeat, ctx.needs_input_grad[0])
        ctx.saved = ctx.fbits = None
        return (dx, None) + (None,) * (len(ctx.needs_input_grad) - 2)


class AsppEngine:

    def __init__(self, owner, rates, num_classes, in_channels):
        self.owner, self.rates, self.K, self.C = owner, tuple(int(r) for r in rates), num_classes, in_channels
        self.wall = self.wallT = None
        self._sig = None
        self._have_dgrad = False

    @staticmethod
    def _room(t):
        return t.untyped_storage().nbytes() // t.element_size() - t.storage_offset()

    def _w4(self):
        ws = [getattr(self.owner.conv2d_list, str(i)).weight for i in range(4)]
        n = ws[0].numel()
        base = ws[0].data_ptr()
        if all(w.data_ptr() == base + 4 * n * i for i, w in enumerate(ws)) and self._room(ws[0]) >= 4 * n:
            return torch.as_strided(ws[0].detach(), (4,) + tuple(ws[0].shape), (n,) + tuple(ws[0].stride())), ws
        return torch.stack([w.detach() for w in ws]).contiguous(), ws

    def _b4(self):
        bs = [getattr(self.owner.conv2d_list, str(i)).bias for i in range(4)]
        base = bs[0].data_ptr()
        if all(b.data_ptr() == base + 4 * self.K * i for i, b in enumerate(bs)) and self._room(bs[0]) >= 4 * self.K:
            return torch.as_strided(bs[0].detach(), (4, self.K), (self.K, 1)), bs
        return torch.stack([b.detach() for b in bs]).contiguous(), bs

    def prepare(self, train):
        w4, ws = self._w4()
        store = getattr(ws[0], "_mi_store", None)
        sig = (store.generation if store is not None else -1, sum(w._version for w in ws), ws[0].data_ptr())
        if sig != self._sig or (train and not self._have_dgrad):
            self.wall = K.aspp_pack_fwd(w4, out=self.wall)
            if train:
                self.wallT = K.aspp_pack_dgrad(w4, out=self.wallT)
            self._sig = sig
            self._have_dgrad = train

    def forward(self, x):
        B, h, w, _ = x.shape
        z = K.conv_gemm(x, self.wall, (h, w), zsplit=K.ASPP_ZGW, flop_cols=self.K)
        b4, _ = self._b4()
        return K.aspp_col2im(z, b4, B, h, w, self.K, self.rates)

    def backward(self, x, dlow, need_dx, msk=None):
        h, w = x.shape[1], x.shape[2]
        g = K.aspp_im2col(dlow, self.rates)
        w4, ws = self._w4()
        b4, bs = self._b4()
        sched = WgradScheduler.on(x.device)

        def weight_and_bias_grads():
            slots = [grad_slot(p) for p in ws]
            n = ws[0].numel()
            base = slots[0][0].data_ptr()
            stacked = all(s[0].data_ptr() == base + 4 * n * i for i, s in enumerate(slots)) and len({s[1] for s in slots}) == 1
            if stacked:
                dw4 = torch.as_strided(slots[0][0], (4,) + tuple(ws[0].shape), (n,) + tuple(ws[0].stride()))
                K.conv_wgrad(g, x, dw4, out_map=1, ncls=self.K, accumulate=slots[0][1])
            else:
                dw4 = torch.empty((4,) + tuple(ws[0].shape), dtype=torch.float32, device=x.device)
                K.conv_wgrad(g, x, dw4, out_map=1, ncls=self.K)
                for i, (slot, acc) in enumerate(slots):
                    slot.add_(dw4[i]) if acc else slot.copy_(dw4[i])
            bslots = [grad_slot(p) for p in bs]
            bbase = bslots[0][0].data_ptr()
            if all(s[0].data_ptr() == bbase + 4 * self.K * i for i, s in enumerate(bslots)) and len({s[1] for s in bslots}) == 1:
                K.aspp_bias_grad(dlow, torch.as_strided(bslots[0][0], (4, self.K), (self.K, 1)), accumulate=bslots[0][1])
            else:
                db4 = torch.empty((4, self.K), dtype=torch.float32, device=x.device)
                K.aspp_bias_grad(dlow, db4)
                for i, (slot, acc) in enumerate(bslots):
                    slot.add_(db4[i]) if acc else slot.copy_(db4[i])

        sched.run(weight_and_bias_grads, g, x, dlow)
        dx = K.conv_gemm(g, self.wallT, (h, w), msk=msk, flop_cols=36 * self.K) if need_dx else None
        sched.join()
        store = getattr(ws[0], "_mi_store", None)
        if store is not None and store.grad_hooks:
            for hook in store.grad_hooks:
                hook(store, 0, store.total)
        return dx


class AsppFn(torch.autograd.Function):

    @staticmethod
    def forward(ctx, x, eng, *params):
        train = any(ctx.needs_input_grad)
        eng.prepare(train)
        ctx.eng, ctx.x = eng, (x if train else None)
        return eng.forward(x)

    @staticmethod
    def backward(ctx, dlow):
        dx = ctx.eng.backward(ctx.x, dlow.contiguous().float(), ctx.needs_input_grad[0])
        ctx.x = None
        return (dx, None) + (None,) * (len(ctx.needs_input_grad) - 2)


class AsppLossFn(torch.autograd.Function):

    @staticmethod
    def forward(ctx, x, labels, eng, ignore_index, temperature, class_weights, label_smoothing, *params):
        train = any(ctx.needs_input_grad)
        eng.prepare(train)
        low = eng.forward(x)
        eng.last_low = low
        if temperature != 1.0:
            loss_out, dlow = K.upsample_ce(low * (1.0 / temperature), labels, want_grad=train, grad_scale=1.0 / temperature,
                                           ignore_index=ignore_index, class_weights=class_weights, label_smoothing=label_smoothing)
        else:
            loss_out, dlow = K.upsample_ce(low, labels, want_grad=train, ignore_index=ignore_index, class_weights=class_weights,
                                           label_smoothing=label_smoothing)
        ctx.eng, ctx.x, ctx.dlow = eng, (x if train else None), dlow
        ctx.loss_out = eng.last_loss_out = loss_out
        bad = getattr(eng, "bad_labels", None)
        if bad is None or bad.device != loss_out.device:
            bad = eng.bad_labels = torch.zeros(1, dtype=torch.float32, device=loss_out.device)
        bad.add_(loss_out[2:3])
        return loss_out[0].clone()

    @staticmethod
    def backward(ctx, gout):
        dlow = ctx.dlow * gout
        dx = ctx.eng.backward(ctx.x, dlow, ctx.needs_input_grad[0])
        ctx.x = ctx.dlow = None
        return (dx, None, None, None, None, None, None) + (None,) * (len(ctx.needs_input_grad) - 7)


class AsppOhemLossFn(AsppLossFn):

    @staticmethod
    def forward(ctx, x, labels, eng, ignore_index, temperature, thresh, min_kept, *params):
        train = any(ctx.needs_input_grad)
        eng.prepare(train)
        low = eng.forward(x)
        eng.last_low = low
        inv_t = 1.0 / temperature
        loss_out, dlow, _ = K.upsample_ce_ohem(low if temperature == 1.0 else low * inv_t, labels, thresh, min_kept, want_grad=train,
                                               grad_scale=1.0 if temperature == 1.0 else inv_t, ignore_index=ignore_index)
        ctx.eng, ctx.x, ctx.dlow = eng, (x if train else None), dlow
        ctx.loss_out = eng.last_loss_out = loss_out
        bad = getattr(eng, "bad_labels", None)
        if bad is None or bad.device != loss_out.device:
            bad = eng.bad_labels = torch.zeros(1, dtype=torch.float32, device=loss_out.device)
        bad.add_(loss_out[2:3])
        return loss_out[0].clone()


class AsppFocalLossFn(AsppLossFn):

    @staticmethod
    def forward(ctx, x, labels, eng, ignore_index, temperature, class_weights, gamma, *params):
        train = any(ctx.needs_input_grad)
        eng.prepare(train)
        low = eng.forward(x)
        eng.last_low = low
        inv_t = 1.0 / temperature
        loss_out, dlow = K.upsample_ce_focal(low if temperature == 1.0 else low * inv_t, labels, gamma, want_grad=train,
                                             grad_scale=1.0 if temperature == 1.0 else inv_t, ignore_index=ignore_index, class_weights=class_weights)
        ctx.eng, ctx.x, ctx.dlow = eng, (x if train else None), dlow
        ctx.loss_out = eng.last_loss_out = loss_out
        bad = getattr(eng, "bad_labels", None)
        if bad is None or bad.device != loss_out.device:
            bad = eng.bad_labels = torch.zeros(1, dtype=torch.float32, device=loss_out.device)
        bad.add_(loss_out[2:3])
        return loss_out[0].clone()


class UpsampleFn(torch.autograd.Function):

    @staticmethod
    def forward(ctx, low, size):
        ctx.hw = (low.shape[1], low.shape[2])
        return K.upsample_ac_fwd(low, tuple(int(s) for s in size))

    @staticmethod
    def backward(ctx, dup):
        return K.upsample_ac_bwd(dup.contiguous(), ctx.hw), None


class SoftmaxCEFn(torch.autograd.Function):

    @staticmethod
    def forward(ctx, logits, labels, ignore_index):
        logits = logits.contiguous()
        out = K.softmax_ce_fwd(logits, labels, ignore_index)
        K.check_labels(out, logits.shape[1], "CrossEntropyLoss target")
        ctx.save_for_backward(logits, labels, out)
        ctx.ignore_index = ignore_index
        return out[0].clone()

    @staticmethod
    def backward(ctx, gout):
        logits, labels, out = ctx.saved_tensors
        d = K.softmax_ce_bwd(logits, labels, out, 1.0, ctx.ignore_index)
        return d * gout, None, None
```

### rnd_semantic_segmentation_amd/host/modules.py

```python
import logging
import os

import torch
import torch.nn as nn
import torch.nn.functional as F

from .. import _lib
from . import arch, engine


class FrozenBatchNorm2d(nn.Module):

    def __init__(self, n):
        super().__init__()
        self.register_buffer("weight", torch.ones(n))
        self.register_buffer("bias", torch.zeros(n))
        self.register_buffer("running_mean", torch.zeros(n))
        self.register_buffer("running_var", torch.ones(n))

    def fold(self):
        scale = self.weight * self.running_var.rsqrt()
        return scale, self.bias - self.running_mean * scale

    def forward(self, x):
# ... 6 lines not shown
        raise _lib.MiError("%s runs on the MI355X only (got a %s tensor); the CPU restatement of this path is "
                           "oracle/ref_model.py and is test infrastructure, not a fallback" % (who, x.device))
    _lib.lib()


class resnet_feature_extractor(nn.Module):

    def __init__(self, backbone_name, pretrained_weights=None, aux=False, pretrained_backbone=True, freeze_bn=False,
                 layers=None):
        super().__init__()
        self.freeze_bn = bool(freeze_bn)
        if aux:
            raise NotImplementedError("aux (layer3) output is not used by any DeepLab config")
        if layers is None:
            if backbone_name not in arch.LAYERS:
                raise NotImplementedError("backbone %r (have: %s)" % (backbone_name, sorted(arch.LAYERS)))
            layers = arch.LAYERS[backbone_name]
        self.plan = arch.bottleneck_plan(layers)
        self.out_channels = self.plan[-1].cout
        self.backbone = arch.Holder()
        self._add_conv(arch.STEM)
        for blk in self.plan:
            for c in arch.block_convs(blk):
                self._add_conv(c)
        self._engine = engine.StageEngine(self, self.plan)
        self._fp32 = engine.Fp32Backbone(self, self.plan)
        self.precision = "bf16"
        self._store = None
        if pretrained_backbone and pretrained_weights:
            self._load_pretrained(pretrained_weights)

    def set_precision(self, precision):
        if precision not in ("bf16", "fp32"):
            raise ValueError("precision %r (bf16 | fp32)" % (precision,))
        self.precision = precision
        return self

    def _add_conv(self, c):
        node = arch.node_at(self.backbone, c.key)
        w = torch.empty(c.cout, c.cin, c.k, c.k)
        nn.init.kaiming_normal_(w, mode="fan_out", nonlinearity="relu")
        node.weight = nn.Parameter(w)
        parent, leaf = c.bn.rsplit(".", 1) if "." in c.bn else ("", c.bn)
        holder = arch.node_at(self.backbone, parent) if parent else self.backbone
        holder.add_module(leaf, FrozenBatchNorm2d(c.cout) if self.freeze_bn else nn.BatchNorm2d(c.cout))

    def _load_pretrained(self, src):
        log = logging.getLogger(__name__)
        if "://" in src:
            log.warning("MODEL.WEIGHTS=%s is a URL; offline build - keeping the initialised weights", src)
            return
        if not os.path.exists(src):
            raise FileNotFoundError(src)
        sd = torch.load(src, map_location="cpu")
        sd = sd.get("state_dict", sd)
        own = self.backbone.state_dict()
        picked = {k: v for k, v in sd.items() if k in own and own[k].shape == v.shape}
        self.backbone.load_state_dict(picked, strict=False)
        log.info("loaded %d/%d backbone tensors from %s", len(picked), len(own), src)

    def engine_parameters(self):
        return [(k, p) for k, p in self.named_parameters()]

    def ensure_flat(self):
        dev = self.backbone.conv1.weight.device
        if self._store is None or not self._store.intact() or self._store.data.device != dev:
            self._store = engine.FlatStore(self.engine_parameters(), dev)
        return self._store

    def _stem_fold(self):
        bn = self.backbone.bn1
        sig = (engine.bn_versions(bn), bn.weight.data_ptr())
        if getattr(self, "_stem_sig", None) != sig:
            self._stem_scale, self._stem_shift = engine.bn_fold(bn)
            self._stem_sig = sig
        return self._stem_scale, self._stem_shift

    def sync_batchnorm(self, on=True):
        for m in self.backbone.modules():
            if isinstance(m, nn.BatchNorm2d):
                m._mi_sync = bool(on)
        return self

    def forward(self, x):
        _require_gpu(x, "resnet_feature_extractor")
        if self.precision == "fp32":
            if torch.is_grad_enabled() and any(p.requires_grad for p in self.parameters()):
                raise _lib.MiError("the fp32 path is forward-only (evaluation): call it under torch.no_grad(), or "
                                   "set_precision('bf16') to train")
            return self._fp32.forward(x.float()).permute(0, 3, 1, 2)
        self.ensure_flat()
        bb = self.backbone
        xb = x
        self._engine.batch_stats = (not self.freeze_bn) and self.training
        if self._engine.batch_stats:
            y = engine.BnStemFn.apply(xb, bb.conv1.weight, bb.bn1.weight, bb.bn1.bias, bb.bn1)
            params = [p for rt in self._engine.convs for p in (rt.weight, rt.bn.weight, rt.bn.bias)]
            return engine.BnStagesFn.apply(y, self._engine, *params).permute(0, 3, 1, 2)
        scale, shift = self._stem_fold()
        y = engine.StemFn.apply(xb, bb.conv1.weight, scale, shift)
        weights = [rt.weight for rt in self._engine.convs]
        feat = engine.StagesFn.apply(y, self._engine, *weights)
        return feat.permute(0, 3, 1, 2)


class ASPP_Classifier_V2(nn.Module):

    def __init__(self, in_channels, dilation_series, padding_series, num_classes):
        super().__init__()
        if list(dilation_series) != list(padding_series) or len(dilation_series) != 4:
            raise NotImplementedError("ASPP engine expects 4 branches with padding == dilation (build.py:26-28 passes "
                                      "[6, 12, 18, 24] twice)")
        self.in_channels, self.num_classes = in_channels, num_classes
        self.rates = tuple(int(d) for d in dilation_series)
        self.conv2d_list = arch.Holder()
        for i in range(4):
            node = arch.Holder()
            node.weight = nn.Parameter(torch.randn(num_classes, in_channels, 3, 3) * 0.01)
            self.conv2d_list.add_module(str(i), node)
        bound = 1.0 / (in_channels * 9) ** 0.5
        for i in range(4):
            getattr(self.conv2d_list, str(i)).bias = nn.Parameter(torch.empty(num_classes).uniform_(-bound, bound))
        self._engine = engine.AsppEngine(self, self.rates, num_classes, in_channels)
        self._fp32 = engine.Fp32Aspp(self, self.rates)
        self.precision = "bf16"
        self._store = None

    def set_precision(self, precision):
        if precision not in ("bf16", "fp32"):
            raise ValueError("precision %r (bf16 | fp32)" % (precision,))
        self.precision = precision
        return self

    def _low_fp32(self, x):
        if torch.is_grad_enabled() and any(p.requires_grad for p in self.parameters()):
            raise _lib.MiError("the fp32 path is forward-only (evaluation): call it under torch.no_grad()")
        return self._fp32.forward(x.float().permute(0, 2, 3, 1).contiguous())

    def engine_parameters(self):
        named = dict(self.named_parameters())
        order = ["conv2d_list.%d.weight" % i for i in range(4)] + ["conv2d_list.%d.bias" % i for i in range(4)]
        return [(k, named[k]) for k in order]

    def ensure_flat(self):
        dev = self.conv2d_list._modules["0"].weight.device
        if self._store is None or not self._store.intact() or self._store.data.device != dev:
            self._store = engine.FlatStore(self.engine_parameters(), dev)
        return self._store

    def _params(self):
        return [p for _, p in self.engine_parameters()]

    @staticmethod
    def _nhwc(x):
        return x.permute(0, 2, 3, 1).contiguous().to(torch.bfloat16) if x.dtype != torch.bfloat16 else x.permute(0, 2, 3, 1).contiguous()

    def forward(self, x, size=None):
        _require_gpu(x, "ASPP_Classifier_V2")
        if self.precision == "fp32":
            low = self._low_fp32(x)
            if size is not None:
                from .. import kernels
                return kernels.upsample_ac_fwd(low, tuple(int(s) for s in size))
            return low.permute(0, 3, 1, 2)
        self.ensure_flat()
        low = engine.AsppFn.apply(self._nhwc(x), self._engine, *self._params())
        if size is not None:
            return engine.UpsampleFn.apply(low, tuple(int(s) for s in size))
        return low.permute(0, 3, 1, 2)

    def loss(self, x, label, ignore_index=255, temperature=1.0, class_weights=None, label_smoothing=0.0, ohem=None, focal_gamma=0.0):
        engine.K.refuse_ohem_with_weights(ohem, class_weights, label_smoothing)
        focal_gamma = engine.K.refuse_focal_with(focal_gamma, ohem, label_smoothing)
        _require_gpu(x, "ASPP_Classifier_V2")
        self.ensure_flat()
        if focal_gamma > 0.0:
            out = engine.AsppFocalLossFn.apply(self._nhwc(x), label.long().contiguous(), self._engine, int(ignore_index), float(temperature),
                                               class_weights, focal_gamma, *self._params())
            self.last_low = self._engine.last_low.detach().permute(0, 3, 1, 2)
            return out
        if ohem is not None:
            thresh, min_kept = engine.K.check_ohem(ohem)
            out = engine.AsppOhemLossFn.apply(self._nhwc(x), label.long().contiguous(), self._engine, int(ignore_index), float(temperature),
                                              thresh, min_kept, *self._params())
            self.last_low = self._engine.last_low.detach().permute(0, 3, 1, 2)
            return out
        out = engine.AsppLossFn.apply(self._nhwc(x), label.long().contiguous(), self._engine, int(ignore_index), float(temperature),
                                      class_weights, float(label_smoothing), *self._params())
        self.last_low = self._engine.last_low.detach().permute(0, 3, 1, 2)
        return out

    def predict_probs(self, x, size):
        _require_gpu(x, "ASPP_Classifier_V2")
        from .. import kernels
        with torch.no_grad():
            if self.precision == "fp32":
                low = self._low_fp32(x)
            else:
                self._engine.prepare(False)
                low = self._engine.forward(self._nhwc(x))
            probs, _ = kernels.upsample_softmax(low, tuple(int(s) for s in size), want_pred=False)
        return probs

    def _lows_multi(self, feats, mirrors, who):
        lows, flags = [], []
        for feat, mm in zip(feats, mirrors):
            _require_gpu(feat, "ASPP_Classifier_V2")
            if feat.shape[0] != len(mm):
                raise ValueError("%s: %d images but %d mirror flags" % (who, feat.shape[0], len(mm)))
            if self.precision == "fp32":
                low = self._low_fp32(feat)
            else:
                self._engine.prepare(False)
                low = self._engine.forward(self._nhwc(feat))
            lows += list(low.unbind(0))
            flags += list(mm)
        return lows, flags

    def predict_probs_multi(self, feats, mirrors, size, divisors):
        from .. import kernels
        with torch.no_grad():
            lows, flags = self._lows_multi(feats, mirrors, "predict_probs_multi")
            return kernels.upsample_softmax_multi(lows, flags, tuple(int(s) for s in size), float(divisors[0]), float(divisors[1]))

    def predict_mask_multi(self, feats, mirrors, size, divisors, labels=None, ignore_index=255, threshold=0.0, want_pseudo=False, class_threshold=None,
                           hist=None):
        from .. import kernels
        with torch.no_grad():
            lows, flags = self._lows_multi(feats, mirrors, "predict_mask_multi")
            return kernels.upsample_predict_score(lows, flags, tuple(int(s) for s in size), float(divisors[0]), float(divisors[1]), labels=labels,
                                                  ignore_index=ignore_index, threshold=threshold, want_pseudo=want_pseudo,
                                                  class_threshold=class_threshold, hist=hist)

    def predict_mask(self, x, size, labels=None, ignore_index=255, threshold=0.0, want_pseudo=False, class_threshold=None, hist=None):
        _require_gpu(x, "ASPP_Classifier_V2")
        from .. import kernels
        with torch.no_grad():
            if self.precision == "fp32":
                low = self._low_fp32(x)
            else:
                self._engine.prepare(False)
                low = self._engine.forward(self._nhwc(x))
            return kernels.upsample_predict_score([low[0]], [False], tuple(int(s) for s in size), 1.0, 1.0, labels=labels,
                                                  ignore_index=ignore_index, threshold=threshold, want_pseudo=want_pseudo,
                                                  class_threshold=class_threshold, hist=hist)


class CrossEntropyLoss(nn.Module):

    def __init__(self, ignore_index=255):
        super().__init__()
        self.ignore_index = ignore_index

    def forward(self, logits, target):
        _require_gpu(logits, "CrossEntropyLoss")
        return engine.SoftmaxCEFn.apply(logits.float(), target.long().contiguous(), self.ignore_index)


# ... 19 lines not shown
```

### rnd_semantic_segmentation_amd/host/sgd.py

```python
import torch

from .. import kernels as K


class FusedSGD(torch.optim.SGD):
    def __init__(self, params, lr, momentum=0.0, weight_decay=0.0, dampening=0, nesterov=False):
        if dampening != 0 or nesterov:
            raise NotImplementedError("FusedSGD implements the reference's configuration: dampening=0, nesterov=False")
        super().__init__(params, lr=lr, momentum=momentum, weight_decay=weight_decay)
        self._flat_mom = {}
        self.device_hyper = None

    def set_device_hyper(self, enable=True):
        if not enable:
            self.device_hyper = None
            return
        dev = self.param_groups[0]["params"][0].device
        g = self.param_groups[0]
        self.device_hyper = torch.tensor([g["lr"], g["momentum"], g["weight_decay"]], dtype=torch.float32, device=dev)

    def push_hyper(self):
        self.device_hyper[0:1].fill_(float(self.param_groups[0]["lr"]))

    def zero_grad(self, set_to_none=True):
        stores = set()
        for group in self.param_groups:
            for p in group["params"]:
                st = getattr(p, "_mi_store", None)
                if st is not None and st.owns(p):
                    stores.add(st)
                    if id(p) in st.written:
                        continue
                    if p.grad is not None:
                        p.grad.zero_()
                elif p.grad is not None:
                    p.grad = None if set_to_none else p.grad.zero_()
        for st in stores:
            st.written.clear()

    def _momentum_view(self, p, st):
        flat = self._flat_mom.get(id(st))
        if flat is None:
            flat = self._flat_mom[id(st)] = torch.zeros_like(st.data)
        view = flat[p._mi_off:p._mi_off + p.numel()].view_as(p)
        state = self.state[p]
        cur = state.get("momentum_buffer")
        if cur is None:
            state["momentum_buffer"] = view
        elif cur.data_ptr() != view.data_ptr():
            view.copy_(cur)
            state["momentum_buffer"] = view
        return flat

    @torch.no_grad()
    def step(self, closure=None):
        loss = closure() if closure is not None else None
        for group in self.param_groups:
            lr, mu, wd = group["lr"], group["momentum"], group["weight_decay"]
            params = [p for p in group["params"] if p.grad is not None]
            if not params:
                continue
            if not params[0].is_cuda:
                raise RuntimeError("FusedSGD updates parameters on the MI355X; got %s" % params[0].device)
            st = getattr(params[0], "_mi_store", None)
            whole = (st is not None and len(params) == len(st.params) and {id(p) for p in params} == {id(q) for q in st.params}
                     and st.intact() and all(p.grad.data_ptr() == st.grad.data_ptr() + 4 * p._mi_off for p in params))
            if whole:
                for p in params:
                    flat = self._momentum_view(p, st)
                if self.device_hyper is not None:
                    if not torch.cuda.is_current_stream_capturing():
                        self.push_hyper()
                    K.sgd_step_dev(st.data, st.grad, flat, self.device_hyper)
                else:
                    K.sgd_step(st.data, st.grad, flat, lr, mu, wd)
                st.generation += 1
            else:
                for p in params:
                    state = self.state[p]
                    if "momentum_buffer" not in state:
                        state["momentum_buffer"] = torch.zeros_like(p, memory_format=torch.contiguous_format)
                    g = p.grad if p.grad.is_contiguous() else p.grad.contiguous()
                    K.sgd_step(p.data, g, state["momentum_buffer"], lr, mu, wd)
                    ps = getattr(p, "_mi_store", None)
                    if ps is not None:
                        ps.generation += 1
        return loss
```

### rnd_semantic_segmentation_amd/host/trainer.py

```python
import datetime
import os
import time

import torch
import torch.distributed as dist

from . import ddp
from .metrics import MetricLogger, adjust_learning_rate, dump_json, strip_prefix_if_present
from .modules import build_classifier, build_feature_extractor
from .plugin import BaseTrainer
from .sgd import FusedSGD


class ASPPTrainer(BaseTrainer):
    MINED = ("ohem",)

    def __init__(self, name, cfg, train_loader, local_rank, logger=None):
        super(ASPPTrainer, self).__init__(name, cfg, train_loader, local_rank, logger)

    build_feature_extractor = staticmethod(build_feature_extractor)
    build_classifier = staticmethod(build_classifier)

    def make_optimizer(self, params, lr):
        cls = FusedSGD if self.device.type == "cuda" else torch.optim.SGD
        return cls(params, lr=lr, momentum=self.cfg.SOLVER.MOMENTUM, weight_decay=self.cfg.SOLVER.WEIGHT_DECAY)

    def init_params(self):
        self.feature_extractor = self.build_feature_extractor(self.cfg)
        self.feature_extractor.to(self.device)
        self.classifier = self.build_classifier(self.cfg)
        self.classifier.to(self.device)
        if self.ce_kwargs and not (hasattr(self.classifier, "loss") and self.device.type == "cuda"):
            raise NotImplementedError("SOLVER.LOSS 'ohem' and SOLVER.CLASS_WEIGHTS / SOLVER.LABEL_SMOOTHING run inside the fused head (classifier.loss on the GPU); "
                                      "this classifier / device trains through the unfused fallback, which does not know them")
        for m in (self.feature_extractor, self.classifier):
            if hasattr(m, "ensure_flat") and self.device.type == "cuda":
                m.ensure_flat()
        self.optimizer_fea = self.make_optimizer(self._ordered_params(self.feature_extractor), self.cfg.SOLVER.BASE_LR)
        self.optimizer_cls = self.make_optimizer(self._ordered_params(self.classifier), self.cfg.SOLVER.BASE_LR * 10)
        self.iteration = 0
        self.world_size = dist.get_world_size() if dist.is_available() and dist.is_initialized() else 1
        self.rank = dist.get_rank() if self.world_size > 1 else 0
        self.distributed = self.world_size > 1
        self.reducer = None
        if self.distributed or (dist.is_available() and dist.is_initialized() and os.environ.get("MI_DDP_FORCE") == "1"):
            stores = [m.ensure_flat() if hasattr(m, "ensure_flat") else _cpu_store(m) for m in (self.classifier, self.feature_extractor)]
            self.reducer = ddp.GradAllReducer(stores)
            self.reducer.broadcast_parameters(0, modules=(self.feature_extractor, self.classifier))
            if hasattr(self.feature_extractor, "sync_batchnorm") and not self.cfg.MODEL.FREEZE_BN:
                self.feature_extractor.sync_batchnorm(True)

    @staticmethod
    def _ordered_params(module):
        return list(module.parameters())

    def _load_checkpoint(self):
        self.checkpoint = torch.load(self.cfg.resume, map_location=self.device)
        self.feature_extractor.load_state_dict(strip_prefix_if_present(self.checkpoint["feature_extractor"], "module."))
        self.classifier.load_state_dict(strip_prefix_if_present(self.checkpoint["classifier"], "module."))
        if "optimizer_fea" in self.checkpoint:
            self.logger.info("Loading optimizer_fea from {}".format(self.cfg.resume))
            self.optimizer_fea.load_state_dict(self.checkpoint["optimizer_fea"])
        if "optimizer_cls" in self.checkpoint:
            self.logger.info("Loading optimizer_cls from {}".format(self.cfg.resume))
            self.optimizer_cls.load_state_dict(self.checkpoint["optimizer_cls"])
        if "iteration" in self.checkpoint:
            self.iteration = self.checkpoint["iteration"]
        if "epoch" in self.checkpoint:
            self.start_epoch = self.checkpoint["epoch"] + 1

    def _save_checkpoint(self, epoch, save_path):
        clone = lambda sd: {k: v.detach().clone() for k, v in sd.items()}
        checkpoint = {
            "epoch": epoch,
            "iteration": self.iteration,
            "feature_extractor": clone(self.feature_extractor.state_dict()),
            "classifier": clone(self.classifier.state_dict()),
            "optimizer_fea": self.optimizer_fea.state_dict(),
            "optimizer_cls": self.optimizer_cls.state_dict(),
        }
        torch.save(checkpoint, save_path)

    GRAPH_WARMUP = 3

    def _graph_enabled(self):
        return (os.environ.get("MI_GRAPH") == "1" and self.device.type == "cuda" and self.reducer is None
                and isinstance(self.optimizer_fea, FusedSGD) and hasattr(self.classifier, "loss"))

    def _graph_signature(self):
        from . import engine
        fe, cls = self.feature_extractor, self.classifier
        sig = [getattr(m, "_store", None) is not None and m._store.data.data_ptr() for m in (fe, cls)]
        eng = getattr(fe, "_engine", None)
        if eng is not None:
            sig.append(sum(engine.bn_versions(rt.bn) for rt in eng.convs) if getattr(fe, "freeze_bn", True) else -1)
            sig.append(bool(eng._have_dgrad))
        return tuple(sig)

    def _graph_step(self, src_input, src_label, current_lr):
        st = getattr(self, "_graph", None)
        if st is None:
            st = self._graph = {"eager": 0, "graph": None}
        if st["graph"] is None:
            if st["eager"] < self.GRAPH_WARMUP or src_input.shape != st.get("shape", src_input.shape):
                st["eager"] += 1
                st["shape"] = src_input.shape
                return None
            st["x"] = torch.empty_like(src_input, device=self.device)
            st["y"] = torch.empty(src_label.shape, dtype=torch.int64, device=self.device)
            for opt in (self.optimizer_fea, self.optimizer_cls):
                opt.set_device_hyper(True)
            st["x"].copy_(src_input, non_blocking=True)
            st["y"].copy_(src_label, non_blocking=True)
            torch.cuda.synchronize()
            g = torch.cuda.CUDAGraph()
            with torch.cuda.graph(g):
                st["loss"] = self._step_core(st["x"], st["y"])
            st["graph"] = g
            st["sig"] = self._graph_signature()
        if src_input.shape != st["x"].shape or self._graph_signature() != st["sig"]:
            self._graph = {"eager": 0, "graph": None}
            return None
        st["x"].copy_(src_input, non_blocking=True)
        st["y"].copy_(src_label, non_blocking=True)
        self.optimizer_fea.push_hyper()
        self.optimizer_cls.push_hyper()
        st["graph"].replay()
        return st["loss"].clone()

    def _step_core(self, src_input, src_label):
        self.optimizer_fea.zero_grad()
        self.optimizer_cls.zero_grad()
        feat = self.feature_extractor(src_input)
        loss = self.classifier.loss(feat, src_label, self.cfg.INPUT.IGNORE_LABEL, **self.ce_kwargs)
        loss.backward()
        self.optimizer_fea.step()
        self.optimizer_cls.step()
        return loss.detach()

    RUN_AHEAD = 2

    def _throttle(self):
        if self.device.type != "cuda":
            return
        q = self.__dict__.setdefault("_inflight", [])
        if len(q) >= self.RUN_AHEAD:
            q.pop(0).synchronize()
        ev = torch.cuda.Event()
        ev.record(torch.cuda.current_stream(self.device))
        q.append(ev)

    def train_step(self, src_input, src_label, max_iter):
        self._throttle()
        current_lr = adjust_learning_rate(self.cfg.SOLVER.LR_METHOD, self.cfg.SOLVER.BASE_LR, self.iteration, max_iter,
                                          power=self.cfg.SOLVER.LR_POWER)
        for group in self.optimizer_fea.param_groups:
            group["lr"] = current_lr
        for group in self.optimizer_cls.param_groups:
            group["lr"] = current_lr * 10
        if self._graph_enabled():
            loss = self._graph_step(src_input.to(self.device, non_blocking=True), src_label.to(self.device, non_blocking=True).long(), current_lr)
            if loss is not None:
                return loss, current_lr
        self.optimizer_fea.zero_grad()
        self.optimizer_cls.zero_grad()
        src_input = src_input.to(self.device, non_blocking=True)
        src_label = src_label.to(self.device, non_blocking=True).long()
        feat = self.feature_extractor(src_input)
        if hasattr(self.classifier, "loss"):
            loss = self.classifier.loss(feat, src_label, self.cfg.INPUT.IGNORE_LABEL, **self.ce_kwargs)
        else:
            output = self.classifier(feat, src_label.shape[-2:])
            loss = torch.nn.functional.cross_entropy(output, src_label, ignore_index=self.cfg.INPUT.IGNORE_LABEL)
        loss.backward()
        if self.reducer is not None:
            self.reducer.finish()
        self.optimizer_fea.step()
        self.optimizer_cls.step()
        return loss.detach(), current_lr

    def train(self):
        output_dir = self.cfg.OUTPUT_DIR
        save_to_disk = self.local_rank == 0 and self.rank == 0
        self.iteration = (self.start_epoch - 1) * len(self.train_loader)
        max_iter = self.cfg.SOLVER.EPOCHS * len(self.train_loader)
        if self.rank == 0:
            self.logger.info("#" * 20 + " Start Training " + "#" * 20)
        meters = MetricLogger(delimiter="  ")
        self.feature_extractor.train()
        self.classifier.train()
        start_training_time = time.time()
        end = time.time()
        pending = []
        images = 0

        def flush():
            bad = getattr(getattr(self.classifier, "_engine", None), "bad_labels", None)
            if bad is not None and pending:
                if self.world_size > 1 and torch.distributed.is_initialized():
                    torch.distributed.all_reduce(bad)
                n = int(bad.item())
                bad.zero_()
                if n:
                    raise ValueError("train labels: %d label values in the last %d steps lie outside [0, %d) and are not ignore_index - "
                                     "torch.nn.CrossEntropyLoss would raise a device assert; map the label ids to train ids first"
                                     % (n, len(pending), self.cfg.MODEL.NUM_CLASSES))
            for l, lr in pending:
                v = float(l)
                meters.update(loss_seg=v)
                self.loss_data.append(v)
                self.lr_data.append(lr)
            pending.clear()

        for epoch in range(self.start_epoch, self.cfg.SOLVER.EPOCHS + 1):
            sampler = getattr(self.train_loader, "sampler", None)
            if hasattr(sampler, "set_epoch"):
                sampler.set_epoch(epoch)
            for i, (src_input, src_label, _) in enumerate(self.train_loader):
                data_time = time.time() - end
                loss, lr = self.train_step(src_input, src_label, max_iter)
                pending.append((loss, lr))
                self.iteration += 1
                images += src_input.shape[0] * self.world_size
                log_now = self.iteration % 20 == 0 or self.iteration == max_iter
                if log_now:
                    flush()
                batch_time = time.time() - end
                end = time.time()
                meters.update(time=batch_time, data=data_time)
                if log_now and self.rank == 0:
                    eta_seconds = meters.time.global_avg * (max_iter - self.iteration)
                    mem = torch.cuda.max_memory_allocated() / 1024.0 / 1024.0 if self.device.type == "cuda" else 0.0
                    self.logger.info(meters.delimiter.join([
                        "Epoch: {epoch}", "eta: {eta}", "iter: {iter}", "{meters}", "lr: {lr:.6f}", "max mem: {memory:.0f}",
                        "img/s: {ips:.2f}"]).format(
                        epoch=epoch, eta=str(datetime.timedelta(seconds=int(eta_seconds))), iter=self.iteration, meters=str(meters),
                        lr=self.optimizer_fea.param_groups[0]["lr"], memory=mem, ips=images / max(time.time() - start_training_time, 1e-9)))
            flush()
            if epoch % self.cfg.SOLVER.CHECKPOINT_PERIOD == 0 and save_to_disk:
                os.makedirs(output_dir, exist_ok=True)
                self._save_checkpoint(epoch, os.path.join(output_dir, "Aspp-{}.pth".format(epoch)))
        total_training_time = time.time() - start_training_time
        if self.rank == 0:
            self.logger.info("Total training time: {} ({:.4f} s / epoch)".format(
                str(datetime.timedelta(seconds=total_training_time)), total_training_time / max(self.cfg.SOLVER.EPOCHS, 1)))
        if save_to_disk:
            os.makedirs(output_dir, exist_ok=True)
            dump_json(os.path.join(output_dir, "aspp_chart_params.json"), {"learning rate": self.lr_data, "loss": self.loss_data})


def _cpu_store(module):
    from .engine import FlatStore
    named = list(module.named_parameters())
# ... 2 lines not shown
```

### rnd_semantic_segmentation_amd/kernels.py

```python
import collections
import ctypes

import torch

from . import _lib
from ._lib import check

EPI_SCALE_BIAS, EPI_RESIDUAL, EPI_RELU, EPI_MASK, EPI_OUT_F32, EPI_ZSPLIT, EPI_WRITE_MASK, EPI_BITMASK, EPI_LEAKY = 1, 2, 4, 8, 16, 32, 64, 128, 256
GATHER_FWD, GATHER_DGRAD = 0, 1
ASPP_ZGW, ASPP_KPAD = 20, 704


def _stream():
    return ctypes.c_void_p(torch.cuda.current_stream().cuda_stream)


PROFILE = None


def _timed(name, flops, launch, tag=None):
    if PROFILE is None:
        return launch()
    e0, e1 = torch.cuda.Event(enable_timing=True), torch.cuda.Event(enable_timing=True)
    e0.record()
# ... 674 lines not shown
    xn = x.permute(0, 2, 3, 1)
    if not xn.is_contiguous():
        xn = xn.contiguous()
    col = torch.empty((B, Ho, Wo, ncols), dtype=torch.bfloat16, device=x.device)
    check(_lib.lib().mi_stem_im2col(_p(xn), _p(col), B, H, W, Ho, Wo, ncols, _stream()), "mi_stem_im2col")
    return col


def stem_conv_fwd(x, weight):
    col = stem_im2col(x, 192)
    O = weight.shape[0]
    wp = torch.zeros((1, O, 192), dtype=torch.bfloat16, device=x.device)
    wp[0, :, :147] = weight.detach().reshape(O, 147).to(torch.bfloat16)
    return conv_gemm(col, wp, (col.shape[1], col.shape[2]), 1, 1, 0, 1, GATHER_FWD), col


def stem_wgrad(dy, x=None, col=None):
    _chk(dy, torch.bfloat16, "dy")
    if col is None:
        col = stem_im2col(x, 160)
    O, n = dy.shape[-1], col.shape[-1]
    dw = torch.empty((O, n, 1, 1), dtype=torch.float32, device=dy.device)
    conv_wgrad(dy, col, dw, 1, 1, 0, 1)
    return dw.view(O, n)[:, :147].reshape(O, 3, 7, 7)


def stem_direct_enabled():
    return bool(_lib.lib().mi_stem_direct_enabled())


def _stem_out_hw(H, W):
    return (H + 6 - 7) // 2 + 1, (W + 6 - 7) // 2 + 1


def stem_pack_image(x):
    if not x.is_cuda:
        raise _lib.MiError("stem_pack_image: x must live on the GPU (no CPU path exists)")
    if x.dim() != 4 or x.shape[1] != 3:
        raise _lib.MiError("stem_pack_image: x must be [B,3,H,W], got %s" % (tuple(x.shape),))
    B, _, H, W = x.shape
    if x.dtype == torch.float32 and x.is_contiguous():
        src, nhwc = x, 0
    else:
        src = x.to(dtype=torch.bfloat16).permute(0, 2, 3, 1)
        if not src.is_contiguous():
            src = src.contiguous()
        nhwc = 1
    x4 = torch.empty((B, H, W, 4), dtype=torch.bfloat16, device=x.device)
    check(_lib.lib().mi_stem_pack_image(_p(src), nhwc, _p(x4), B, H, W, _stream()), "mi_stem_pack_image")
    return x4


def stem_conv_direct(x4, weight):
    _chk(x4, torch.bfloat16, "x4")
    w = _chk(weight.detach(), torch.float32, "weight")
    B, H, W, C4 = x4.shape
    if C4 != 4 or tuple(w.shape[1:]) != (3, 7, 7):
        raise _lib.MiError("stem_conv_direct: x4 %s, weight %s" % (tuple(x4.shape), tuple(w.shape)))
    O = w.shape[0]
    Ho, Wo = _stem_out_hw(H, W)
    y = torch.empty((B, Ho, Wo, O), dtype=torch.bfloat16, device=x4.device)
    wpack = _workspace(6 * 64 * 32 * 2, x4.device, "stem_wpack")
    check(_timed("stem_direct_fwd_kernel", 2.0 * B * Ho * Wo * O * 147, lambda: _lib.lib().mi_stem_conv_fwd(
        _p(x4), _p(w), _p(wpack), _p(y), B, H, W, O, Ho, Wo, _stream()), tag=("fwd", 7, 4, O, B * Ho * Wo, 0, 1)), "mi_stem_conv_fwd")
    return y


def stem_wgrad_direct(dy, x4):
    _chk(dy, torch.bfloat16, "dy")
    _chk(x4, torch.bfloat16, "x4")
    B, H, W, C4 = x4.shape
    Ho, Wo = _stem_out_hw(H, W)
    O = dy.shape[-1]
    if C4 != 4 or tuple(dy.shape[:3]) != (B, Ho, Wo):
        raise _lib.MiError("stem_wgrad_direct: dy %s does not belong to x4 %s" % (tuple(dy.shape), tuple(x4.shape)))
    L = _lib.lib()
    dw = torch.empty((O, 3, 7, 7), dtype=torch.float32, device=dy.device)
    ws = _workspace(L.mi_stem_conv_wgrad_workspace(B, Ho, Wo), dy.device, "stem_wgrad")
    check(_timed("stem_direct_wgrad_kernel+reduce", 2.0 * B * Ho * Wo * O * 147, lambda: L.mi_stem_conv_wgrad(
        _p(dy), _p(x4), _p(dw), B, H, W, O, Ho, Wo, _p(ws), ws.numel(), _stream()), tag=("wgrad", 7, 4, O, B * Ho * Wo, 0, 1)), "mi_stem_conv_wgrad")
    return dw


def bias_grad_bf16(dy, db, accumulate=False):
    _chk(dy, torch.bfloat16, "dy")
    _chk(db, torch.float32, "db")
    N = dy.shape[-1]
    L = _lib.lib()
    ws = _workspace(L.mi_colsum_workspace(dy.numel() // N, N), dy.device, "colsum")
    check(L.mi_bias_grad_bf16(_p(dy), _p(db), dy.numel() // N, N, int(accumulate), _p(ws), ws.numel(), _stream()), "mi_bias_grad_bf16")
    return db


def upsample_softce(seg_low, d_low, size, domain, temperature=1.8, clip=0.9, want_grad=True, grad_scale=1.0):
    _chk(seg_low, torch.float32, "seg_low")
    _chk(d_low, torch.float32, "d_low")
    B, h, w, Kc = seg_low.shape
    ldD = d_low.shape[-1]
    H, W = size
    L = _lib.lib()
    ws = _workspace(L.mi_upsample_softce_workspace(B, h, w, Kc, H, W), seg_low.device, "softce")
    out = torch.empty(2, dtype=torch.float32, device=seg_low.device)
    dd = torch.empty_like(d_low) if want_grad else None
    check(L.mi_upsample_softce(_p(seg_low), 1.0 / float(temperature), float(clip), _p(d_low), ldD, int(domain), _p(out), _p(dd), B, h, w, Kc,
                               H, W, float(grad_scale), _p(ws), ws.numel(), _stream()), "mi_upsample_softce")
    return out, dd


def upsample_softce_2grid(seg_low, d_low, size, domain, temperature=1.8, clip=0.9, want_grad=True, grad_scale=1.0, seg_align_corners=False,
                          d_align_corners=True):
    _chk(seg_low, torch.float32, "seg_low")
    _chk(d_low, torch.float32, "d_low")
    B, hs, ws, Kc = seg_low.shape
    Bd, hd, wd, ldD = d_low.shape
    if Bd != B:
        raise _lib.MiError("upsample_softce_2grid: seg_low holds %d images, d_low %d" % (B, Bd))
    H, W = size
    L = _lib.lib()
    ws_buf = _workspace(L.mi_upsample_softce_2grid_workspace(B, hd, wd, Kc, H, W), seg_low.device, "softce2")
    out = torch.empty(2, dtype=torch.float32, device=seg_low.device)
    dd = torch.empty_like(d_low) if want_grad else None
    check(L.mi_upsample_softce_2grid(_p(seg_low), hs, ws, int(bool(seg_align_corners)), 1.0 / float(temperature), float(clip), _p(d_low), hd, wd,
                                     ldD, int(bool(d_align_corners)), int(domain), float(grad_scale), _p(out), _p(dd), B, Kc, H, W, _p(ws_buf),
                                     ws_buf.numel(), _stream()), "mi_upsample_softce_2grid")
    return out, dd


def adam_step(p, g, exp_avg, exp_avg_sq, lr, beta1, beta2, eps, step, grad_clamp=None):
    for t, n in ((p, "p"), (g, "g"), (exp_avg, "exp_avg"), (exp_avg_sq, "exp_avg_sq")):
        _chk(t, torch.float32, n)
    if grad_clamp is not None:
        check(_lib.lib().mi_adam_step_clamped(_p(p), _p(g), _p(exp_avg), _p(exp_avg_sq), p.numel(), float(lr), float(beta1), float(beta2), float(eps),
                                              int(step), float(grad_clamp), _stream()), "mi_adam_step_clamped")
        return
    check(_lib.lib().mi_adam_step(_p(p), _p(g), _p(exp_avg), _p(exp_avg_sq), p.numel(), float(lr), float(beta1), float(beta2), float(eps),
                                  int(step), _stream()), "mi_adam_step")


def adam_step_dev(p, g, exp_avg, exp_avg_sq, hyper):
    for t, n in ((p, "p"), (g, "g"), (exp_avg, "exp_avg"), (exp_avg_sq, "exp_avg_sq"), (hyper, "hyper")):
        _chk(t, torch.float32, n)
    check(_lib.lib().mi_adam_step_dev(_p(p), _p(g), _p(exp_avg), _p(exp_avg_sq), p.numel(), _p(hyper), _stream()), "mi_adam_step_dev")


def sgd_step(p, g, buf, lr, momentum, weight_decay):
    for t, n in ((p, "p"), (g, "g"), (buf, "buf")):
        _chk(t, torch.float32, n)
    check(_lib.lib().mi_sgd_step(_p(p), _p(g), _p(buf), p.numel(), float(lr), float(momentum), float(weight_decay), _stream()),
          "mi_sgd_step")


def sgd_step_dev(p, g, buf, hyper):
    for t, n in ((p, "p"), (g, "g"), (buf, "buf"), (hyper, "hyper")):
        _chk(t, torch.float32, n)
    check(_lib.lib().mi_sgd_step_dev(_p(p), _p(g), _p(buf), p.numel(), _p(hyper), _stream()), "mi_sgd_step_dev")


def relu_mask(x, msk, out=None):
    _chk(x, torch.bfloat16, "x")
    bits = msk.dtype == torch.int16
    _chk(msk, torch.int16 if bits else torch.bfloat16, "msk")
    if out is None:
        out = torch.empty_like(x)
    check(_lib.lib().mi_relu_mask(_p(x), _p(msk), _p(out), x.numel(), int(bits), _stream()), "mi_relu_mask")
    return out


def frozen_bn_fold(w, b, mean, var):
    for t in (w, b, mean, var):
        _chk(t, torch.float32, "bn buffer")
    scale, shift = torch.empty_like(w), torch.empty_like(w)
    check(_lib.lib().mi_frozen_bn_fold(_p(w), _p(b), _p(mean), _p(var), _p(scale), _p(shift), w.numel(), _stream()),
          "mi_frozen_bn_fold")
    return scale, shift


def structure_loss(pred, mask, want_grad=True, grad_scale=1.0):
    _chk(pred, torch.float32, "pred")
    _chk(mask, torch.float32, "mask")
    if pred.shape != mask.shape or (pred.dim() == 4 and pred.shape[1] != 1):
        raise _lib.MiError("structure_loss: pred / mask must be [B,1,H,W] of the same shape, got %s / %s" % (tuple(pred.shape), tuple(mask.shape)))
    B, H, W = pred.shape[0], pred.shape[-2], pred.shape[-1]
    L = _lib.lib()
    ws = torch.empty(int(L.mi_structure_loss_workspace(B, H, W)), dtype=torch.uint8, device=pred.device)
    out = torch.empty(1 + 2 * B, dtype=torch.float32, device=pred.device)
    grad = torch.empty_like(pred) if want_grad else None
    check(L.mi_structure_loss(_p(pred), _p(mask), B, H, W, _p(out), _p(grad), ctypes.c_float(grad_scale), _p(ws), ws.numel(), _stream()),
          "mi_structure_loss")
    return out[0], grad


_bn_ws = {}


def _bn_workspace(dev, M, C):
    need = int(_lib.lib().mi_bn_workspace(M, C))
    key = (dev, torch.cuda.current_stream(dev).cuda_stream)
    w = _bn_ws.get(key)
    if w is None or w.numel() < need:
        w = _bn_ws[key] = torch.empty(need, dtype=torch.uint8, device=dev)
    return w


def bn_colsum(y, mean=None):
    _chk(y, torch.bfloat16, "y")
    C = y.shape[-1]
    M = y.numel() // C
    out = torch.empty(C, dtype=torch.float32, device=y.device)
    ws = _bn_workspace(y.device, M, C)
    _timed("bn_kernels", 0.0, lambda: check(_lib.lib().mi_bn_colsum(_p(y), _p(mean), M, C, _p(out), _p(ws), ws.numel(), _stream()), "mi_bn_colsum"),
           ("bn", 0, C, C, M, 0, 0))
    return out


def bn_colsum2(y, pilot):
    _chk(y, torch.bfloat16, "y")
    C = y.shape[-1]
    M = y.numel() // C
    s1, s2 = torch.empty((2, C), dtype=torch.float32, device=y.device)
    ws = _bn_workspace(y.device, M, C)
    _timed("bn_kernels", 0.0, lambda: check(_lib.lib().mi_bn_colsum2(_p(y), _p(pilot), M, C, _p(s1), _p(s2), _p(ws), ws.numel(), _stream()), "mi_bn_colsum2"),
           ("bn", 4, C, C, M, 0, 0))
    return s1, s2


def bn_finalize(s1, s2, pilot, count, bn):
    C = s1.numel()
    out = torch.empty((4, C), dtype=torch.float32, device=s1.device)
    track = bn.track_running_stats and bn.running_mean is not None
    if track and bn.momentum is None:
        raise NotImplementedError("BatchNorm2d(momentum=None) (cumulative average) is not used by the reference")
    check(_lib.lib().mi_bn_finalize(_p(s1), _p(s2), _p(pilot), float(count), _p(bn.weight.detach()), _p(bn.bias.detach()),
                                    _p(bn.running_mean) if track else None, _p(bn.running_var) if track else None,
                                    _p(bn.num_batches_tracked) if track else None, float(bn.momentum or 0.0), float(bn.eps), _p(out), C, _stream()),
          "mi_bn_finalize")
    return out


# ... 132 lines not shown
```

Measured before the change: 301.9 images/s.

## Fuse SGD step with bf16 weight packing, stem pool into wgrad, head mask

Adds a fused SGD kernel that updates fp32 parameters and also writes the packed bf16 forward weights and the scaled transposed copies, so the separate repack pass after each step goes away. It also folds the stem maxpool backward into the stem weight-gradient kernel, and passes the backbone's final ReLU mask to the ASPP head so the feature map is used by one consumer only. All three are on by default through env switches. The fused SGD kernel does more per-block work, relies on a descriptor table and gap ranges being built correctly, and changes the FMA rounding of the update.

```diff
diff --git a/include/mi355seg.h b/include/mi355seg.h
--- a/include/mi355seg.h
+++ b/include/mi355seg.h
@@ -163,6 +163,11 @@
 
 int mi_sgd_step(float* p, const float* g, float* buf, size_t n, float lr, float momentum, float weight_decay, void* stream);
 int mi_sgd_step_dev(float* p, const float* g, float* buf, size_t n, const float* hyper , void* stream);
+int mi_sgd_pack_enabled(void);
+int mi_sgd_step_pack(float* p, const float* g, float* buf, size_t n, float lr, float momentum, float weight_decay, const float* sflat, void* wp,
+                     void* wpt, const int64_t* table_dev, int n_desc, int total_blocks, const int64_t* gaps_dev, int n_gaps, void* stream);
+int mi_sgd_step_pack_dev(float* p, const float* g, float* buf, size_t n, const float* hyper , const float* sflat, void* wp, void* wpt,
+                         const int64_t* table_dev, int n_desc, int total_blocks, const int64_t* gaps_dev, int n_gaps, void* stream);
 
 int mi_stem_pool_fwd(const void* y, const float* scale, const float* shift, void* pool, uint8_t* idx,
                      int B, int Hc, int Wc, int C, int Hp, int Wp, void* stream);
@@ -175,6 +180,9 @@
 size_t mi_stem_conv_wgrad_workspace(int B, int Ho, int Wo);
 int mi_stem_conv_wgrad(const void* dy, const void* x4, float* dw, int B, int H, int W, int O, int Ho, int Wo, void* workspace,
                        size_t workspace_bytes, void* stream);
+int mi_stem_pool_wgrad_enabled(void);
+int mi_stem_conv_wgrad_pool(const void* dpool, const uint8_t* idx, const float* scale, const void* x4, float* dw, int B, int H, int W, int O,
+                            int Ho, int Wo, int Hp, int Wp, void* workspace, size_t workspace_bytes, void* stream);
 
 int mi_bias_grad_bf16(const void* dy_bf16, float* db, int M, int N, int accumulate,
                       void* workspace , size_t workspace_bytes, void* stream);
@@ -207,6 +215,7 @@
 int mi_allreduce_bucket(void* ptr, size_t count, int dtype, int average, void* comm, void* stream);
 
 int mi_relu_mask(const void* x_bf16, const void* msk, void* y_bf16, size_t n, int bits, void* stream);
+int mi_head_mask_enabled(void);
 int mi_frozen_bn_fold(const float* w, const float* b, const float* mean, const float* var, float* scale, float* shift, int n, void* stream);
 
 size_t mi_bn_workspace(long M, int C);
diff --git a/rnd_semantic_segmentation_amd/_lib.py b/rnd_semantic_segmentation_amd/_lib.py
--- a/rnd_semantic_segmentation_amd/_lib.py
+++ b/rnd_semantic_segmentation_amd/_lib.py
@@ -65,6 +65,9 @@
     "mi_stem_conv_fwd": (I, [P, P, P, P] + [I] * 6 + [P]),
     "mi_stem_conv_wgrad_workspace": (Z, [I] * 3),
     "mi_stem_conv_wgrad": (I, [P, P, P] + [I] * 6 + [P, Z, P]),
+    "mi_stem_pool_wgrad_enabled": (I, []),
+    "mi_stem_conv_wgrad_pool": (I, [P, P, P, P, P] + [I] * 8 + [P, Z, P]),
+    "mi_head_mask_enabled": (I, []),
     "mi_bias_grad_bf16": (I, [P, P, I, I, I, P, Z, P]),
     "mi_upsample_softce_workspace": (Z, [I] * 6),
     "mi_upsample_softce": (I, [P, F, F, P, I, I, P, P] + [I] * 6 + [F, P, Z, P]),
@@ -75,6 +78,9 @@
     "mi_adam_step_dev": (I, [P, P, P, P, Z, P, P]),
     "mi_sgd_step": (I, [P, P, P, Z, F, F, F, P]),
     "mi_sgd_step_dev": (I, [P, P, P, Z, P, P]),
+    "mi_sgd_pack_enabled": (I, []),
+    "mi_sgd_step_pack": (I, [P, P, P, Z, F, F, F, P, P, P, P, I, I, P, I, P]),
+    "mi_sgd_step_pack_dev": (I, [P, P, P, Z, P, P, P, P, P, I, I, P, I, P]),
     "mi_pack_weight_f32": (I, [P, P, I, I, I, P]),
     "mi_conv_f32": (I, [P, P, P] + [I] * 11 + [P, P, P, I, P]),
     "mi_stem_f32": (I, [P, P, P, P, P, I, I, I, P]),
diff --git a/rnd_semantic_segmentation_amd/csrc/elementwise.hip b/rnd_semantic_segmentation_amd/csrc/elementwise.hip
--- a/rnd_semantic_segmentation_amd/csrc/elementwise.hip
+++ b/rnd_semantic_segmentation_amd/csrc/elementwise.hip
@@ -69,6 +69,9 @@
 #endif
         sw.pp_trace_wg = env("MI_PP_TRACE_WG", 0);
         sw.stem_direct = env("MI_STEM_DIRECT", 1);
+        sw.stem_pool_wgrad = env("MI_STEM_POOL_WGRAD", 1);
+        sw.head_mask = env("MI_HEAD_MASK", 1);
+        sw.sgd_pack = env("MI_SGD_PACK", 1);
         sw.stem_wgrad_splits = env("MI_STEM_WGRAD_SPLITS", 512);
         if (sw.stem_wgrad_splits < 1 || sw.stem_wgrad_splits > 4096) sw.stem_wgrad_splits = 512;
     });
@@ -128,6 +131,162 @@
         const float b = mu * buf[i] + gg;
         buf[i] = b;
         p[i] = p[i] - lr * b;
+    }
+}
+
+__device__ __forceinline__ void sgd_update(float& p, float g, float& b, float lr, float mu, float wd) {
+    const float gg = __builtin_fmaf(wd, p, g);
+    b = __builtin_fmaf(mu, b, gg);
+    p = __builtin_fmaf(-lr, b, p);
+}
+__device__ __forceinline__ void sgd_update_tail(float& p, float g, float& b, float lr, float mu, float wd) {
+    const float gg = __fadd_rn(g, __fmul_rn(wd, p));
+    b = __fadd_rn(__fmul_rn(mu, b), gg);
+    p = __builtin_fmaf(-lr, b, p);
+}
+
+struct SgdPackArgs {
+    float* p;
+    const float* g;
+    float* buf;
+    size_t n;
+    const float* sflat;
+    __bf16* wp;
+    __bf16* wpt;
+    const long* table;
+    const long* gaps;
+    int n_desc, pack_blocks, n_gaps;
+    float lr, mu, wd;
+    const float* hyper;
+};
+
+constexpr int SP_TILES = 4;
+constexpr int SP_BATCH = 3;
+
+template <bool DEV>
+__global__ __launch_bounds__(256) void sgd_pack_kernel(SgdPackArgs a) {
+    __shared__ float tile[32][32 * 9 + 1];
+    __shared__ float ssc[32];
+    const float lr = DEV ? a.hyper[0] : a.lr, mu = DEV ? a.hyper[1] : a.mu, wd = DEV ? a.hyper[2] : a.wd;
+    const int tid = threadIdx.x;
+    const size_t n_vec = a.n & ~(size_t)3;
+    if ((int)blockIdx.x >= a.pack_blocks) {
+        const long first = ((long)blockIdx.x - a.pack_blocks) * 256 + tid, stride = ((long)gridDim.x - a.pack_blocks) * 256;
+        for (int k = 0; k < a.n_gaps; ++k) {
+            const long lo = a.gaps[2 * k], hi = a.gaps[2 * k + 1];
+            for (long i = lo + first; i < hi; i += stride) {
+                float pv = a.p[i], bv = a.buf[i];
+                if ((size_t)i < n_vec) sgd_update(pv, a.g[i], bv, lr, mu, wd); else sgd_update_tail(pv, a.g[i], bv, lr, mu, wd);
+                a.buf[i] = bv;
+                a.p[i] = pv;
+            }
+        }
+        return;
+    }
+    int lo = 0, hi = a.n_desc - 1;
+    while (lo < hi) {
+        const int mid = (lo + hi + 1) >> 1;
+        if (a.table[mid * 8 + 7] <= (long)blockIdx.x) lo = mid; else hi = mid - 1;
+    }
+    const long* d = a.table + lo * 8;
+    const int O = (int)d[4], I = (int)d[5], T = (int)d[6];
+    const int tiles_i = (I + 31) >> 5, groups_i = (tiles_i + SP_TILES - 1) / SP_TILES;
+    const int local = (int)((long)blockIdx.x - d[7]);
+    const int ot = local / groups_i;
+    const int o0 = ot * 32, it0 = (local - ot * groups_i) * SP_TILES;
+    if (o0 >= O) return;
+    const int no = min(32, O - o0);
+    const long plane = (long)O * I;
+    const bool have_t = d[3] >= 0;
+    const bool vec_ld = ((d[0] | ((long)I * T)) & 3) == 0;
+    const bool vec_wp = ((d[2] | (long)I) & 7) == 0;
+    const bool vec_wpt = have_t && ((d[3] | (long)O) & 7) == 0;
+    if (tid < 32) ssc[tid] = (have_t && d[1] >= 0 && tid < no) ? a.sflat[d[1] + o0 + tid] : 1.f;
+    for (int it = it0; it < it0 + SP_TILES && it < tiles_i; ++it) {
+        const int i0 = it * 32;
+        const int ni = min(32, I - i0);
+        const int rowlen = ni * T;
+        if (it != it0) __syncthreads();
+        if (vec_ld) {
+            const int r4 = rowlen >> 2, items = no * r4;
+            for (int base = tid; base < items; base += 256 * SP_BATCH) {
+                f32x4 pv[SP_BATCH], gv[SP_BATCH], bv[SP_BATCH];
+                long idx[SP_BATCH];
+                int oo[SP_BATCH], ee[SP_BATCH];
+#pragma unroll
+                for (int j = 0; j < SP_BATCH; ++j) {
+                    const int item = base + j * 256;
+                    oo[j] = item / r4;
+                    ee[j] = (item - oo[j] * r4) << 2;
+                    idx[j] = d[0] + ((long)(o0 + oo[j]) * I + i0) * T + ee[j];
+                    if (item < items) {
+                        pv[j] = *reinterpret_cast<const f32x4*>(a.p + idx[j]);
+                        gv[j] = *reinterpret_cast<const f32x4*>(a.g + idx[j]);
+                        bv[j] = *reinterpret_cast<const f32x4*>(a.buf + idx[j]);
+                    }
+                }
+#pragma unroll
+                for (int j = 0; j < SP_BATCH; ++j) {
+                    if (base + j * 256 < items) {
+#pragma unroll
+                        for (int e = 0; e < 4; ++e) {
+                            float pe = pv[j][e], be = bv[j][e];
+                            sgd_update(pe, gv[j][e], be, lr, mu, wd);
+                            pv[j][e] = pe;
+                            bv[j][e] = be;
+                            tile[oo[j]][ee[j] + e] = pe;
+                        }
+                        *reinterpret_cast<f32x4*>(a.buf + idx[j]) = bv[j];
+                        *reinterpret_cast<f32x4*>(a.p + idx[j]) = pv[j];
+                    }
+                }
+            }
+        } else {
+            for (int item = tid; item < no * rowlen; item += 256) {
+                const int o = item / rowlen, e = item - o * rowlen;
+                const long idx = d[0] + ((long)(o0 + o) * I + i0) * T + e;
+                float pv = a.p[idx], bv = a.buf[idx];
+                if ((size_t)idx < n_vec) sgd_update(pv, a.g[idx], bv, lr, mu, wd); else sgd_update_tail(pv, a.g[idx], bv, lr, mu, wd);
+                a.buf[idx] = bv;
+                a.p[idx] = pv;
+                tile[o][e] = pv;
+            }
+        }
+        __syncthreads();
+        if (vec_wp) {
+            const int c8n = ni >> 3, per_t = no * c8n;
+            for (int item = tid; item < T * per_t; item += 256) {
+                const int t = item / per_t, rem = item - t * per_t;
+                const int o = rem / c8n, c = (rem - o * c8n) << 3;
+                bf16x8 v;
+#pragma unroll
+                for (int k = 0; k < 8; ++k) v[k] = (__bf16)tile[o][(c + k) * T + t];
+                *reinterpret_cast<bf16x8*>(a.wp + d[2] + t * plane + (long)(o0 + o) * I + i0 + c) = v;
+            }
+        } else {
+            for (int item = tid; item < T * no * ni; item += 256) {
+                const int t = item / (no * ni), rem = item - t * (no * ni);
+                const int o = rem / ni, c = rem - o * ni;
+                a.wp[d[2] + t * plane + (long)(o0 + o) * I + i0 + c] = (__bf16)tile[o][c * T + t];
+            }
+        }
+        if (vec_wpt) {
+            const int o8n = no >> 3, per_t = ni * o8n;
+            for (int item = tid; item < T * per_t; item += 256) {
+                const int t = item / per_t, rem = item - t * per_t;
+                const int i = rem / o8n, o = (rem - i * o8n) << 3;
+                bf16x8 v;
+#pragma unroll
+                for (int k = 0; k < 8; ++k) v[k] = (__bf16)__fmul_rn(tile[o + k][i * T + t], ssc[o + k]);
+                *reinterpret_cast<bf16x8*>(a.wpt + d[3] + t * plane + (long)(i0 + i) * O + o0 + o) = v;
+            }
+        } else if (have_t) {
+            for (int item = tid; item < T * ni * no; item += 256) {
+                const int t = item / (ni * no), rem = item - t * (ni * no);
+                const int i = rem / no, o = rem - i * no;
+                a.wpt[d[3] + t * plane + (long)(i0 + i) * O + o0 + o] = (__bf16)__fmul_rn(tile[o][i * T + t], ssc[o]);
+            }
+        }
     }
 }
 
@@ -175,6 +334,41 @@
     return MI_OK;
 }
 
+int sgd_pack_launch(const char* who, float* p, const float* g, float* buf, size_t n, float lr, float mu, float wd, const float* hyper, bool dev,
+                    const float* sflat, void* wp, void* wpt, const int64_t* table_dev, int n_desc, int total_blocks, const int64_t* gaps_dev, int n_gaps,
+                    void* stream) {
+    MI_REQUIRE(p && g && buf && n > 0 && wp && table_dev && n_desc > 0 && total_blocks > 0 && (!dev || hyper), "%s: bad argument", who);
+    MI_REQUIRE(n_gaps >= 0 && (n_gaps == 0 || gaps_dev), "%s: n_gaps=%d without a gap table", who, n_gaps);
+    MI_REQUIRE(mi_aligned16(p) && mi_aligned16(g) && mi_aligned16(buf) && mi_aligned16(wp) && mi_aligned16(wpt), "%s: buffers must be 16-byte aligned", who);
+    SgdPackArgs a;
+    a.p = p, a.g = g, a.buf = buf, a.n = n;
+    a.sflat = sflat, a.wp = (__bf16*)wp, a.wpt = (__bf16*)wpt;
+    a.table = (const long*)table_dev, a.gaps = (const long*)gaps_dev;
+    a.n_desc = n_desc, a.pack_blocks = total_blocks, a.n_gaps = n_gaps;
+    a.lr = lr, a.mu = mu, a.wd = wd, a.hyper = hyper;
+    const unsigned grid = (unsigned)total_blocks + (n_gaps > 0 ? 64u : 0u);
+    if (dev)
+        hipLaunchKernelGGL(sgd_pack_kernel<true>, dim3(grid), dim3(256), 0, (hipStream_t)stream, a);
+    else
+        hipLaunchKernelGGL(sgd_pack_kernel<false>, dim3(grid), dim3(256), 0, (hipStream_t)stream, a);
+    MI_CHECK_LAUNCH(who);
+    return MI_OK;
+}
+
+extern "C" int mi_sgd_pack_enabled(void) { return mi_sw().sgd_pack != 0; }
+
+extern "C" int mi_sgd_step_pack(float* p, const float* g, float* buf, size_t n, float lr, float momentum, float weight_decay, const float* sflat, void* wp,
+                                void* wpt, const int64_t* table_dev, int n_desc, int total_blocks, const int64_t* gaps_dev, int n_gaps, void* stream) {
+    return sgd_pack_launch("mi_sgd_step_pack", p, g, buf, n, lr, momentum, weight_decay, nullptr, false, sflat, wp, wpt, table_dev, n_desc, total_blocks,
+                           gaps_dev, n_gaps, stream);
+}
+
+extern "C" int mi_sgd_step_pack_dev(float* p, const float* g, float* buf, size_t n, const float* hyper, const float* sflat, void* wp, void* wpt,
+                                    const int64_t* table_dev, int n_desc, int total_blocks, const int64_t* gaps_dev, int n_gaps, void* stream) {
+    return sgd_pack_launch("mi_sgd_step_pack_dev", p, g, buf, n, 0.f, 0.f, 0.f, hyper, true, sflat, wp, wpt, table_dev, n_desc, total_blocks, gaps_dev,
+                           n_gaps, stream);
+}
+
 __global__ void relu_mask_bits_kernel(const bf16x8* __restrict__ x, const uint8_t* __restrict__ m, bf16x8* __restrict__ y, size_t n8) {
     const size_t stride = (size_t)gridDim.x * blockDim.x;
     for (size_t i = (size_t)blockIdx.x * blockDim.x + threadIdx.x; i < n8; i += stride) {
@@ -188,6 +382,8 @@
 }
 
 }
+
+extern "C" int mi_head_mask_enabled(void) { return mi_sw().head_mask != 0; }
 
 extern "C" int mi_relu_mask(const void* x, const void* msk, void* y, size_t n, int bits, void* stream) {
     MI_REQUIRE(x && msk && y && n > 0 && n % 8 == 0, "mi_relu_mask: bad argument (n %% 8 == 0)");
diff --git a/rnd_semantic_segmentation_amd/csrc/mi_common.h b/rnd_semantic_segmentation_amd/csrc/mi_common.h
--- a/rnd_semantic_segmentation_amd/csrc/mi_common.h
+++ b/rnd_semantic_segmentation_amd/csrc/mi_common.h
@@ -52,6 +52,9 @@
     int pp_trace_wg;
     int stem_wgrad_splits;
     int stem_direct;
+    int stem_pool_wgrad;
+    int sgd_pack;
+    int head_mask;
 };
 const MiSwitches& mi_sw();
 
diff --git a/rnd_semantic_segmentation_amd/csrc/stem_direct.hip b/rnd_semantic_segmentation_amd/csrc/stem_direct.hip
--- a/rnd_semantic_segmentation_amd/csrc/stem_direct.hip
+++ b/rnd_semantic_segmentation_amd/csrc/stem_direct.hip
@@ -12,6 +12,9 @@
 constexpr int SD_WG_ROWS = 2 * SD_WG_TH + 5;
 constexpr int SD_DYROWB = SD_TW * 128;
 constexpr int SD_PART = 64 * 7 * 32;
+constexpr int SD_PP_ROWS = SD_WG_TH / 2 + 1;
+constexpr int SD_PP_COLS = SD_TW / 2 + 1;
+constexpr int SD_PP_ITEMS = SD_PP_ROWS * SD_PP_COLS * 8;
 
 __global__ __launch_bounds__(256) void stem_pack_f32_kernel(const float* __restrict__ x, bf16x4* __restrict__ x4, long HW, int B) {
     const int b = blockIdx.y;
@@ -178,11 +181,59 @@
     const bf16x8* dy;
     float* part;
     int B, H, W, Ho, Wo, tiles_x, tiles_y, tiles, S;
+    const bf16x8* dpool;
+    const uint2* idx;
+    const float* scale;
+    int Hp, Wp;
 };
 
+struct PoolPatch {
+    static constexpr int N = (SD_PP_ITEMS + 255) / 256;
+    bf16x8 g[N];
+    uint2 ib[N];
+    __device__ __forceinline__ void load(const bf16x8* __restrict__ dpool, const uint2* __restrict__ idx, int b, int hp0, int wp0, int Hp, int Wp, int tid) {
+#pragma unroll
+        for (int j = 0; j < N; ++j) {
+            const int i = tid + j * 256;
+            const int c = i & 7, px = i >> 3;
+            const int pr = px / SD_PP_COLS, pc = px - pr * SD_PP_COLS;
+            const int hp = hp0 + pr, wp = wp0 + pc;
+#pragma unroll
+            for (int e = 0; e < 8; ++e) g[j][e] = (__bf16)0.f;
+            ib[j] = make_uint2(~0u, ~0u);
+            if (i < SD_PP_ITEMS && hp < Hp && wp < Wp) {
+                const long off = (((long)b * Hp + hp) * Wp + wp) * 8 + c;
+                g[j] = dpool[off];
+                ib[j] = idx[off];
+            }
+        }
+    }
+    static __device__ __forceinline__ unsigned nibbles(unsigned x) {
+        unsigned t = (x >> 4) & 0x0f0f0f0fu;
+        t |= t >> 1;
+        t |= t >> 2;
+        x = (x & 0x0f0f0f0fu) | ((t & 0x01010101u) * 15u);
+        x = (x | (x >> 4)) & 0x00ff00ffu;
+        return (x | (x >> 8)) & 0xffffu;
+    }
+    __device__ __forceinline__ void store(bf16x8* sdp, unsigned* sidx, int tid) const {
+#pragma unroll
+        for (int j = 0; j < N; ++j) {
+            const int i = tid + j * 256;
+            if (i < SD_PP_ITEMS) {
+                sdp[i] = g[j];
+                sidx[i] = nibbles(ib[j].x) | (nibbles(ib[j].y) << 16);
+            }
+        }
+    }
+};
+
+template <bool POOL>
 __global__ __launch_bounds__(256, 2) void stem_direct_wgrad_kernel(StemWgradParams p) {
     __shared__ __attribute__((aligned(16))) uint2 sx[SD_WG_ROWS * SD_ROWPX];
     __shared__ __attribute__((aligned(16))) bf16x8 sdy[SD_WG_TH * SD_TW * 8];
+    __shared__ __attribute__((aligned(16))) bf16x8 sdp[POOL ? SD_PP_ITEMS : 1];
+    __shared__ unsigned sidx[POOL ? SD_PP_ITEMS : 1];
     const int tid = threadIdx.x, lane = tid & 63;
     const int wave = __builtin_amdgcn_readfirstlane(tid >> 6);
     const int kt = wave & 1, oh = wave >> 1;
@@ -201,19 +252,29 @@
         for (int ky = 0; ky < 7; ++ky) acc[a][ky] = f32x4{0.f, 0.f, 0.f, 0.f};
 
     ImageRows<SD_WG_ROWS> nx;
-    bf16x8 ny[8];
+    bf16x8 ny[POOL ? 1 : 8];
+    PoolPatch np;
+    float sc[8];
+    if constexpr (POOL) {
+#pragma unroll
+        for (int e = 0; e < 8; ++e) sc[e] = p.scale[(tid & 7) * 8 + e];
+    }
     auto load_tile = [&](int t) {
         const int tx = t % p.tiles_x, ty = (t / p.tiles_x) % p.tiles_y, b = t / (p.tiles_x * p.tiles_y);
         const int wo0 = tx * SD_TW, ho0 = ty * SD_WG_TH;
         nx.load(p.x4 + (long)b * p.H * p.W, 2 * ho0 - 3, 2 * wo0 - 3, p.H, p.W, tid);
-#pragma unroll
-        for (int j = 0; j < 8; ++j) {
-            const int i = tid + j * 256;
-            const int c = i & 7, P = (i >> 3) & 63, rr = i >> 9;
-            const int ho = ho0 + rr, wo = wo0 + P;
-#pragma unroll
-            for (int e = 0; e < 8; ++e) ny[j][e] = (__bf16)0.f;
-            if (ho < p.Ho && wo < p.Wo) ny[j] = p.dy[(((long)b * p.Ho + ho) * p.Wo + wo) * 8 + c];
+        if constexpr (POOL) {
+            np.load(p.dpool, p.idx, b, ho0 >> 1, wo0 >> 1, p.Hp, p.Wp, tid);
+        } else {
+#pragma unroll
+            for (int j = 0; j < 8; ++j) {
+                const int i = tid + j * 256;
+                const int c = i & 7, P = (i >> 3) & 63, rr = i >> 9;
+                const int ho = ho0 + rr, wo = wo0 + P;
+#pragma unroll
+                for (int e = 0; e < 8; ++e) ny[j][e] = (__bf16)0.f;
+                if (ho < p.Ho && wo < p.Wo) ny[j] = p.dy[(((long)b * p.Ho + ho) * p.Wo + wo) * 8 + c];
+            }
         }
     };
     load_tile(t_begin);
@@ -222,14 +283,48 @@
         const int wo0 = tx * SD_TW, ho0 = ty * SD_WG_TH;
         __syncthreads();
         nx.store(sx, tid);
-#pragma unroll
-        for (int j = 0; j < 8; ++j) {
-            const int i = tid + j * 256;
-            const int c = i & 7, P = (i >> 3) & 63, rr = i >> 9;
-            sdy[(rr * SD_TW + P) * 8 + (c ^ (P & 7))] = ny[j];
+        if constexpr (POOL) {
+            np.store(sdp, sidx, tid);
+        } else {
+#pragma unroll
+            for (int j = 0; j < 8; ++j) {
+                const int i = tid + j * 256;
+                const int c = i & 7, P = (i >> 3) & 63, rr = i >> 9;
+                sdy[(rr * SD_TW + P) * 8 + (c ^ (P & 7))] = ny[j];
+            }
         }
         __syncthreads();
         if (t + 1 < t_end) load_tile(t + 1);
+        if constexpr (POOL) {
+            const int c = tid & 7;
+#pragma unroll
+            for (int j = 0; j < 8; ++j) {
+                const int rr = j >> 1, P = (tid >> 3) + 32 * (j & 1);
+                bf16x8 o;
+#pragma unroll
+                for (int e = 0; e < 8; ++e) o[e] = (__bf16)0.f;
+                if (ho0 + rr < p.Ho && wo0 + P < p.Wo) {
+                    float a[8] = {0.f, 0.f, 0.f, 0.f, 0.f, 0.f, 0.f, 0.f};
+#pragma unroll
+                    for (int hl = rr >> 1; hl <= ((rr + 1) >> 1); ++hl) {
+                        const int ky = rr - 2 * hl + 1;
+                        for (int wl = P >> 1; wl <= ((P + 1) >> 1); ++wl) {
+                            const unsigned tap = (unsigned)(ky * 3 + (P - 2 * wl + 1));
+                            const int it = (hl * SD_PP_COLS + wl) * 8 + c;
+                            const bf16x8 gv = sdp[it];
+                            const unsigned nib = sidx[it];
+#pragma unroll
+                            for (int e = 0; e < 8; ++e)
+                                if (((nib >> (4 * e)) & 15u) == tap) a[e] += (float)gv[e];
+                        }
+                    }
+#pragma unroll
+                    for (int e = 0; e < 8; ++e) o[e] = (__bf16)(a[e] * sc[e]);
+                }
+                sdy[(rr * SD_TW + P) * 8 + (c ^ (P & 7))] = o;
+            }
+            __syncthreads();
+        }
         const int nrows = min(SD_WG_TH, p.Ho - ho0);
         for (int rr = 0; rr < nrows; ++rr) {
 #pragma unroll
@@ -355,28 +450,51 @@
     return (size_t)stem_wgrad_splits(B, Ho, Wo) * SD_PART * sizeof(float);
 }
 
-extern "C" int mi_stem_conv_wgrad(const void* dy, const void* x4, float* dw, int B, int H, int W, int O, int Ho, int Wo, void* workspace,
-                                  size_t workspace_bytes, void* stream) {
-    MI_REQUIRE(dy && x4 && dw && workspace, "mi_stem_conv_wgrad: null operand");
-    MI_REQUIRE(O == 64, "mi_stem_conv_wgrad: O=%d (the stem has 64 output channels)", O);
+namespace {
+int stem_wgrad_launch(const char* who, bool pool, const void* dy, const void* dpool, const uint8_t* idx, const float* scale, const void* x4, float* dw, int B,
+                      int H, int W, int O, int Ho, int Wo, int Hp, int Wp, void* workspace, size_t workspace_bytes, void* stream) {
+    MI_REQUIRE((pool ? dpool && idx && scale : dy != nullptr) && x4 && dw && workspace, "%s: null operand", who);
+    MI_REQUIRE(O == 64, "%s: O=%d (the stem has 64 output channels)", who, O);
     const char* bad = stem_direct_geometry(B, H, W, Ho, Wo);
-    MI_REQUIRE(!bad, "mi_stem_conv_wgrad: %s", bad);
-    MI_REQUIRE((reinterpret_cast<uintptr_t>(x4) & 7) == 0 && mi_aligned16(dy) && mi_aligned16(workspace) && (reinterpret_cast<uintptr_t>(dw) & 3) == 0,
-               "mi_stem_conv_wgrad: alignment");
-    MI_REQUIRE(workspace_bytes >= mi_stem_conv_wgrad_workspace(B, Ho, Wo), "mi_stem_conv_wgrad: workspace holds %zu bytes, %zu needed", workspace_bytes,
+    MI_REQUIRE(!bad, "%s: %s", who, bad);
+    MI_REQUIRE(!pool || (Hp == (Ho + 2 - 3) / 2 + 1 && Wp == (Wo + 2 - 3) / 2 + 1), "%s: pooled size must be that of a 3x3/2/1 max-pool of the conv output", who);
+    MI_REQUIRE((reinterpret_cast<uintptr_t>(x4) & 7) == 0 && mi_aligned16(workspace) && (reinterpret_cast<uintptr_t>(dw) & 3) == 0 &&
+                   (pool ? mi_aligned16(dpool) && (reinterpret_cast<uintptr_t>(idx) & 7) == 0 && (reinterpret_cast<uintptr_t>(scale) & 3) == 0 : mi_aligned16(dy)),
+               "%s: alignment", who);
+    MI_REQUIRE(workspace_bytes >= mi_stem_conv_wgrad_workspace(B, Ho, Wo), "%s: workspace holds %zu bytes, %zu needed", who, workspace_bytes,
                mi_stem_conv_wgrad_workspace(B, Ho, Wo));
     StemWgradParams p;
     p.x4 = (const uint2*)x4;
     p.dy = (const bf16x8*)dy;
+    p.dpool = (const bf16x8*)dpool;
+    p.idx = (const uint2*)idx;
+    p.scale = scale;
+    p.Hp = Hp, p.Wp = Wp;
     p.part = (float*)workspace;
     p.B = B, p.H = H, p.W = W, p.Ho = Ho, p.Wo = Wo;
     p.tiles_x = (Wo + SD_TW - 1) / SD_TW;
     p.tiles_y = (Ho + SD_WG_TH - 1) / SD_WG_TH;
     p.tiles = B * p.tiles_x * p.tiles_y;
     p.S = stem_wgrad_splits(B, Ho, Wo);
-    hipLaunchKernelGGL(stem_direct_wgrad_kernel, dim3((unsigned)p.S), dim3(256), 0, (hipStream_t)stream, p);
-    MI_CHECK_LAUNCH("mi_stem_conv_wgrad");
+    if (!pool)
+        hipLaunchKernelGGL(stem_direct_wgrad_kernel<false>, dim3((unsigned)p.S), dim3(256), 0, (hipStream_t)stream, p);
+    else
+        hipLaunchKernelGGL(stem_direct_wgrad_kernel<true>, dim3((unsigned)p.S), dim3(256), 0, (hipStream_t)stream, p);
+    MI_CHECK_LAUNCH(who);
     hipLaunchKernelGGL(stem_direct_wgrad_reduce_kernel, dim3(SD_PART / 256), dim3(256), 0, (hipStream_t)stream, (const float*)workspace, dw, p.S);
-    MI_CHECK_LAUNCH("mi_stem_conv_wgrad (reduce)");
+    MI_CHECK_LAUNCH(who);
     return MI_OK;
 }
+}
+
+extern "C" int mi_stem_conv_wgrad(const void* dy, const void* x4, float* dw, int B, int H, int W, int O, int Ho, int Wo, void* workspace,
+                                  size_t workspace_bytes, void* stream) {
+    return stem_wgrad_launch("mi_stem_conv_wgrad", false, dy, nullptr, nullptr, nullptr, x4, dw, B, H, W, O, Ho, Wo, 0, 0, workspace, workspace_bytes, stream);
+}
+
+extern "C" int mi_stem_pool_wgrad_enabled(void) { return mi_sw().stem_pool_wgrad != 0; }
+
+extern "C" int mi_stem_conv_wgrad_pool(const void* dpool, const uint8_t* idx, const float* scale, const void* x4, float* dw, int B, int H, int W, int O,
+                                       int Ho, int Wo, int Hp, int Wp, void* workspace, size_t workspace_bytes, void* stream) {
+    return stem_wgrad_launch("mi_stem_conv_wgrad_pool", true, nullptr, dpool, idx, scale, x4, dw, B, H, W, O, Ho, Wo, Hp, Wp, workspace, workspace_bytes, stream);
+}
diff --git a/rnd_semantic_segmentation_amd/csrc/upsample_ce.hip b/rnd_semantic_segmentation_amd/csrc/upsample_ce.hip
--- a/rnd_semantic_segmentation_amd/csrc/upsample_ce.hip
+++ b/rnd_semantic_segmentation_amd/csrc/upsample_ce.hip
@@ -80,7 +80,19 @@
 __global__ void ce_finalize_kernel(const float* __restrict__ partial, int n, float* __restrict__ loss_out) {
     __shared__ float red[512];
     float s = 0.f, c = 0.f;
-    for (int i = threadIdx.x; i < n; i += 256) {
+    const float2* pairs = reinterpret_cast<const float2*>(partial);
+    int i = threadIdx.x;
+    for (; i + 15 * 256 < n; i += 16 * 256) {
+        float2 v[16];
+#pragma unroll
+        for (int j = 0; j < 16; ++j) v[j] = pairs[i + j * 256];
+#pragma unroll
+        for (int j = 0; j < 16; ++j) {
+            s += v[j].x;
+            c += v[j].y;
+        }
+    }
+    for (; i < n; i += 256) {
         s += partial[2 * i];
         c += partial[2 * i + 1];
     }
diff --git a/rnd_semantic_segmentation_amd/host/engine.py b/rnd_semantic_segmentation_amd/host/engine.py
--- a/rnd_semantic_segmentation_amd/host/engine.py
+++ b/rnd_semantic_segmentation_amd/host/engine.py
@@ -165,6 +165,8 @@
         self._pack_sig = None
         self._have_dgrad = False
         self.batch_stats = False
+        self.eval_mode = False
+        self._fused_current = False
 
     def _signature(self):
         store = getattr(self.convs[0].weight, "_mi_store", None)
@@ -193,11 +195,25 @@
             blk += -(-c.cout // 32) * -(-c.cin // 128)
         self._pack_blocks = blk
         self._table_train = torch.tensor(rows, dtype=torch.int64, device=dev)
+        gaps = K.pack_table_gaps(rows, store.total)
+        self._gaps = torch.tensor(gaps, dtype=torch.int64, device=dev) if gaps else None
         self._table_batch = torch.tensor([r[:1] + [-1] + r[2:] for r in rows], dtype=torch.int64, device=dev)
         for r in rows:
             r[3] = -1
         self._table_eval = torch.tensor(rows, dtype=torch.int64, device=dev)
         self._plan_store = store
+        self._fused_current = False
+        store.pack_plan = self
+
+    def fused_step_args(self, store):
+        if (getattr(self, "_plan_store", None) is not store or self.batch_stats or not self._have_dgrad
+                or self._pack_sig != self._signature() + (False,)):
+            return None
+        return self._scale_flat, self._wp_flat, self._wpt_flat, self._table_train, len(self.convs), self._pack_blocks, self._gaps
+
+    def mark_packed(self):
+        self._pack_sig = self._signature() + (False,)
+        self._fused_current = True
 
     def prepare(self, train):
         store = getattr(self.convs[0].weight, "_mi_store", None)
@@ -217,7 +233,9 @@
                     rt.shift.copy_(sh)
                 self._bn_sig = bn_sig
         sig = self._signature() + (self.batch_stats,)
-        if sig != self._pack_sig or refold or (train and not self._have_dgrad):
+        stale = self._fused_current and (self.eval_mode or not train)
+        if sig != self._pack_sig or refold or stale or (train and not self._have_dgrad):
+            self._fused_current = False
             table = self._table_batch if self.batch_stats else (self._table_train if train else self._table_eval)
             K.pack_weights_multi(store.data, self._scale_flat, self._wp_flat, self._wpt_flat, table, len(self.convs), self._pack_blocks)
             self._pack_sig = sig
@@ -355,8 +373,8 @@
         c = rt.spec
         return K.conv_gemm(dy, rt.wpt, in_hw, c.k, c.stride, c.pad, c.dil, K.GATHER_DGRAD, res=res, bits=bits)
 
-    def backward(self, saved, fbits, dfeat, need_dx):
-        g = K.relu_mask(dfeat, fbits)
+    def backward(self, saved, fbits, dfeat, need_dx, premasked=False):
+        g = dfeat if premasked else K.relu_mask(dfeat, fbits)
         store = getattr(self.convs[0].weight, "_mi_store", None)
         sched = WgradScheduler.on(dfeat.device)
         chain = self.chain_mode() in ("all", "bwd") and self._chain_fits(dfeat)
@@ -651,8 +669,16 @@
     @staticmethod
     def backward(ctx, dpool):
         idx, scale = ctx.saved_tensors[:2]
+        if K.stem_direct_enabled() and K.stem_pool_wgrad_enabled():
+            return None, K.stem_wgrad_pool(dpool.contiguous(), idx, scale.contiguous(), ctx.saved_tensors[2]), None, None
         dy = K.stem_pool_bwd(dpool.contiguous(), idx, scale, ctx.conv_hw)
         return None, stem_conv_wgrad(dy, ctx.saved_tensors[2:]), None, None
+
+
+class FeatureMask:
+
+    def __init__(self, bits, sole):
+        self.bits, self.sole, self.applied = bits, bool(sole), False
 
 
 class StagesFn(torch.autograd.Function):
@@ -663,13 +689,16 @@
         eng.prepare(train)
         feat, saved, fbits = eng.forward(x, save=train)
         ctx.eng, ctx.saved, ctx.fbits = eng, saved, fbits
+        ctx.fmask = eng.feature_mask = FeatureMask(fbits, getattr(eng, "sole_consumer_next", False)) if train else None
+        eng.sole_consumer_next = False
         return feat
 
     @staticmethod
     def backward(ctx, dfeat):
         dfeat = dfeat.contiguous()
-        dx = ctx.eng.backward(ctx.saved, ctx.fbits, dfeat, ctx.needs_input_grad[0])
-        ctx.saved = ctx.fbits = None
+        fm = ctx.fmask
+        dx = ctx.eng.backward(ctx.saved, ctx.fbits, dfeat, ctx.needs_input_grad[0], premasked=fm is not None and fm.sole and fm.applied)
+        ctx.saved = ctx.fbits = ctx.fmask = None
         return (dx, None) + (None,) * (len(ctx.needs_input_grad) - 2)
 
 
@@ -717,7 +746,11 @@
         b4, _ = self._b4()
         return K.aspp_col2im(z, b4, B, h, w, self.K, self.rates)
 
-    def backward(self, x, dlow, need_dx, msk=None):
+    def take_feature_mask(self):
+        fm, self.feature_mask_next = getattr(self, "feature_mask_next", None), None
+        return fm
+
+    def backward(self, x, dlow, need_dx, msk=None, fmask=None):
         h, w = x.shape[1], x.shape[2]
         g = K.aspp_im2col(dlow, self.rates)
         w4, ws = self._w4()
@@ -748,7 +781,10 @@
                     slot.add_(db4[i]) if acc else slot.copy_(db4[i])
 
         sched.run(weight_and_bias_grads, g, x, dlow)
-        dx = K.conv_gemm(g, self.wallT, (h, w), msk=msk, flop_cols=36 * self.K) if need_dx else None
+        bits = fmask.bits if fmask is not None and msk is None else None
+        dx = K.conv_gemm(g, self.wallT, (h, w), msk=msk, bits=bits, flop_cols=36 * self.K) if need_dx else None
+        if bits is not None and need_dx:
+            fmask.applied = True
         sched.join()
         store = getattr(ws[0], "_mi_store", None)
         if store is not None and store.grad_hooks:
@@ -787,7 +823,7 @@
         else:
             loss_out, dlow = K.upsample_ce(low, labels, want_grad=train, ignore_index=ignore_index, class_weights=class_weights,
                                            label_smoothing=label_smoothing)
-        ctx.eng, ctx.x, ctx.dlow = eng, (x if train else None), dlow
+        ctx.eng, ctx.x, ctx.dlow, ctx.fmask = eng, (x if train else None), dlow, eng.take_feature_mask()
         ctx.loss_out = eng.last_loss_out = loss_out
         bad = getattr(eng, "bad_labels", None)
         if bad is None or bad.device != loss_out.device:
@@ -798,8 +834,8 @@
     @staticmethod
     def backward(ctx, gout):
         dlow = ctx.dlow * gout
-        dx = ctx.eng.backward(ctx.x, dlow, ctx.needs_input_grad[0])
-        ctx.x = ctx.dlow = None
+        dx = ctx.eng.backward(ctx.x, dlow, ctx.needs_input_grad[0], fmask=ctx.fmask)
+        ctx.x = ctx.dlow = ctx.fmask = None
         return (dx, None, None, None, None, None, None) + (None,) * (len(ctx.needs_input_grad) - 7)
 
 
@@ -814,7 +850,7 @@
         inv_t = 1.0 / temperature
         loss_out, dlow, _ = K.upsample_ce_ohem(low if temperature == 1.0 else low * inv_t, labels, thresh, min_kept, want_grad=train,
                                                grad_scale=1.0 if temperature == 1.0 else inv_t, ignore_index=ignore_index)
-        ctx.eng, ctx.x, ctx.dlow = eng, (x if train else None), dlow
+        ctx.eng, ctx.x, ctx.dlow, ctx.fmask = eng, (x if train else None), dlow, eng.take_feature_mask()
         ctx.loss_out = eng.last_loss_out = loss_out
         bad = getattr(eng, "bad_labels", None)
         if bad is None or bad.device != loss_out.device:
@@ -834,7 +870,7 @@
         inv_t = 1.0 / temperature
         loss_out, dlow = K.upsample_ce_focal(low if temperature == 1.0 else low * inv_t, labels, gamma, want_grad=train,
                                              grad_scale=1.0 if temperature == 1.0 else inv_t, ignore_index=ignore_index, class_weights=class_weights)
-        ctx.eng, ctx.x, ctx.dlow = eng, (x if train else None), dlow
+        ctx.eng, ctx.x, ctx.dlow, ctx.fmask = eng, (x if train else None), dlow, eng.take_feature_mask()
         ctx.loss_out = eng.last_loss_out = loss_out
         bad = getattr(eng, "bad_labels", None)
         if bad is None or bad.device != loss_out.device:
diff --git a/rnd_semantic_segmentation_amd/host/modules.py b/rnd_semantic_segmentation_amd/host/modules.py
--- a/rnd_semantic_segmentation_amd/host/modules.py
+++ b/rnd_semantic_segmentation_amd/host/modules.py
@@ -112,8 +112,9 @@
                 m._mi_sync = bool(on)
         return self
 
-    def forward(self, x):
+    def forward(self, x, sole_consumer=False):
         _require_gpu(x, "resnet_feature_extractor")
+        self._engine.feature_mask = None
         if self.precision == "fp32":
             if torch.is_grad_enabled() and any(p.requires_grad for p in self.parameters()):
                 raise _lib.MiError("the fp32 path is forward-only (evaluation): call it under torch.no_grad(), or "
@@ -123,6 +124,7 @@
         bb = self.backbone
         xb = x
         self._engine.batch_stats = (not self.freeze_bn) and self.training
+        self._engine.eval_mode = not self.training
         if self._engine.batch_stats:
             y = engine.BnStemFn.apply(xb, bb.conv1.weight, bb.bn1.weight, bb.bn1.bias, bb.bn1)
             params = [p for rt in self._engine.convs for p in (rt.weight, rt.bn.weight, rt.bn.bias)]
@@ -130,8 +132,13 @@
         scale, shift = self._stem_fold()
         y = engine.StemFn.apply(xb, bb.conv1.weight, scale, shift)
         weights = [rt.weight for rt in self._engine.convs]
+        self._engine.sole_consumer_next = bool(sole_consumer)
         feat = engine.StagesFn.apply(y, self._engine, *weights)
         return feat.permute(0, 3, 1, 2)
+
+
+    def feature_mask(self):
+        return getattr(self._engine, "feature_mask", None)
 
 
 class ASPP_Classifier_V2(nn.Module):
@@ -199,11 +206,13 @@
             return engine.UpsampleFn.apply(low, tuple(int(s) for s in size))
         return low.permute(0, 3, 1, 2)
 
-    def loss(self, x, label, ignore_index=255, temperature=1.0, class_weights=None, label_smoothing=0.0, ohem=None, focal_gamma=0.0):
+    def loss(self, x, label, ignore_index=255, temperature=1.0, class_weights=None, label_smoothing=0.0, ohem=None, focal_gamma=0.0,
+             feature_mask=None):
         engine.K.refuse_ohem_with_weights(ohem, class_weights, label_smoothing)
         focal_gamma = engine.K.refuse_focal_with(focal_gamma, ohem, label_smoothing)
         _require_gpu(x, "ASPP_Classifier_V2")
         self.ensure_flat()
+        self._engine.feature_mask_next = feature_mask
         if focal_gamma > 0.0:
             out = engine.AsppFocalLossFn.apply(self._nhwc(x), label.long().contiguous(), self._engine, int(ignore_index), float(temperature),
                                                class_weights, focal_gamma, *self._params())
diff --git a/rnd_semantic_segmentation_amd/host/sgd.py b/rnd_semantic_segmentation_amd/host/sgd.py
--- a/rnd_semantic_segmentation_amd/host/sgd.py
+++ b/rnd_semantic_segmentation_amd/host/sgd.py
@@ -68,13 +68,19 @@
             if whole:
                 for p in params:
                     flat = self._momentum_view(p, st)
-                if self.device_hyper is not None:
-                    if not torch.cuda.is_current_stream_capturing():
-                        self.push_hyper()
+                plan = getattr(st, "pack_plan", None)
+                fused = plan.fused_step_args(st) if plan is not None and K.sgd_pack_enabled() else None
+                if self.device_hyper is not None and not torch.cuda.is_current_stream_capturing():
+                    self.push_hyper()
+                if fused is not None:
+                    K.sgd_step_pack(st.data, st.grad, flat, self.device_hyper if self.device_hyper is not None else lr, mu, wd, *fused)
+                elif self.device_hyper is not None:
                     K.sgd_step_dev(st.data, st.grad, flat, self.device_hyper)
                 else:
                     K.sgd_step(st.data, st.grad, flat, lr, mu, wd)
                 st.generation += 1
+                if fused is not None:
+                    plan.mark_packed()
             else:
                 for p in params:
                     state = self.state[p]
diff --git a/rnd_semantic_segmentation_amd/host/trainer.py b/rnd_semantic_segmentation_amd/host/trainer.py
--- a/rnd_semantic_segmentation_amd/host/trainer.py
+++ b/rnd_semantic_segmentation_amd/host/trainer.py
@@ -5,9 +5,10 @@
 import torch
 import torch.distributed as dist
 
+from .. import kernels as _kernels
 from . import ddp
 from .metrics import MetricLogger, adjust_learning_rate, dump_json, strip_prefix_if_present
-from .modules import build_classifier, build_feature_extractor
+from .modules import ASPP_Classifier_V2, build_classifier, build_feature_extractor
 from .plugin import BaseTrainer
 from .sgd import FusedSGD
 
@@ -128,11 +129,19 @@
         st["graph"].replay()
         return st["loss"].clone()
 
+    def _feature(self, src_input):
+        fe = self.feature_extractor
+        if not (hasattr(fe, "feature_mask") and isinstance(self.classifier, ASPP_Classifier_V2) and _kernels.head_mask_enabled()):
+            return fe(src_input), {}
+        feat = fe(src_input, sole_consumer=True)
+        fm = fe.feature_mask()
+        return feat, ({} if fm is None else {"feature_mask": fm})
+
     def _step_core(self, src_input, src_label):
         self.optimizer_fea.zero_grad()
         self.optimizer_cls.zero_grad()
-        feat = self.feature_extractor(src_input)
-        loss = self.classifier.loss(feat, src_label, self.cfg.INPUT.IGNORE_LABEL, **self.ce_kwargs)
+        feat, fmask = self._feature(src_input)
+        loss = self.classifier.loss(feat, src_label, self.cfg.INPUT.IGNORE_LABEL, **self.ce_kwargs, **fmask)
         loss.backward()
         self.optimizer_fea.step()
         self.optimizer_cls.step()
@@ -166,9 +175,9 @@
         self.optimizer_cls.zero_grad()
         src_input = src_input.to(self.device, non_blocking=True)
         src_label = src_label.to(self.device, non_blocking=True).long()
-        feat = self.feature_extractor(src_input)
+        feat, fmask = self._feature(src_input)
         if hasattr(self.classifier, "loss"):
-            loss = self.classifier.loss(feat, src_label, self.cfg.INPUT.IGNORE_LABEL, **self.ce_kwargs)
+            loss = self.classifier.loss(feat, src_label, self.cfg.INPUT.IGNORE_LABEL, **self.ce_kwargs, **fmask)
         else:
             output = self.classifier(feat, src_label.shape[-2:])
             loss = torch.nn.functional.cross_entropy(output, src_label, ignore_index=self.cfg.INPUT.IGNORE_LABEL)
diff --git a/rnd_semantic_segmentation_amd/kernels.py b/rnd_semantic_segmentation_amd/kernels.py
--- a/rnd_semantic_segmentation_amd/kernels.py
+++ b/rnd_semantic_segmentation_amd/kernels.py
@@ -780,6 +780,35 @@
     return dw
 
 
+def stem_pool_wgrad_enabled():
+    return bool(_lib.lib().mi_stem_pool_wgrad_enabled())
+
+
+def stem_wgrad_pool(dpool, idx, scale, x4):
+    _chk(dpool, torch.bfloat16, "dpool")
+    _chk(idx, torch.uint8, "idx")
+    _chk(scale, torch.float32, "scale")
+    _chk(x4, torch.bfloat16, "x4")
+    B, H, W, C4 = x4.shape
+    Ho, Wo = _stem_out_hw(H, W)
+    Hp, Wp = (Ho - 1) // 2 + 1, (Wo - 1) // 2 + 1
+    O = dpool.shape[-1]
+    if C4 != 4 or tuple(dpool.shape[:3]) != (B, Hp, Wp) or idx.shape != dpool.shape or scale.numel() != O:
+        raise _lib.MiError("stem_wgrad_pool: dpool %s / idx %s / scale %s do not belong to x4 %s" % (
+            tuple(dpool.shape), tuple(idx.shape), tuple(scale.shape), tuple(x4.shape)))
+    L = _lib.lib()
+    dw = torch.empty((O, 3, 7, 7), dtype=torch.float32, device=dpool.device)
+    ws = _workspace(L.mi_stem_conv_wgrad_workspace(B, Ho, Wo), dpool.device, "stem_wgrad")
+    check(_timed("stem_direct_wgrad_kernel<pool>+reduce", 2.0 * B * Ho * Wo * O * 147, lambda: L.mi_stem_conv_wgrad_pool(
+        _p(dpool), _p(idx), _p(scale), _p(x4), _p(dw), B, H, W, O, Ho, Wo, Hp, Wp, _p(ws), ws.numel(), _stream()),
+        tag=("wgrad", 7, 4, O, B * Ho * Wo, 0, 1)), "mi_stem_conv_wgrad_pool")
+    return dw
+
+
+def head_mask_enabled():
+    return bool(_lib.lib().mi_head_mask_enabled())
+
+
 def bias_grad_bf16(dy, db, accumulate=False):
     _chk(dy, torch.bfloat16, "dy")
     _chk(db, torch.float32, "db")
@@ -852,6 +881,41 @@
     for t, n in ((p, "p"), (g, "g"), (buf, "buf"), (hyper, "hyper")):
         _chk(t, torch.float32, n)
     check(_lib.lib().mi_sgd_step_dev(_p(p), _p(g), _p(buf), p.numel(), _p(hyper), _stream()), "mi_sgd_step_dev")
+
+
+def sgd_pack_enabled():
+    return bool(_lib.lib().mi_sgd_pack_enabled())
+
+
+def pack_table_gaps(rows, n):
+    gaps, pos = [], 0
+    for lo, hi in sorted((int(r[0]), int(r[0]) + int(r[4]) * int(r[5]) * int(r[6])) for r in rows):
+        if lo < pos or hi > n:
+            raise _lib.MiError("pack table: row [%d, %d) overlaps its neighbour or leaves the store of %d floats" % (lo, hi, n))
+        if lo > pos:
+            gaps.append([pos, lo])
+        pos = hi
+    if pos < n:
+        gaps.append([pos, n])
+    return gaps
+
+
+def sgd_step_pack(p, g, buf, hyper_or_lr, momentum, weight_decay, sflat, wp, wpt, table_dev, n_desc, total_blocks, gaps_dev):
+    for t, n in ((p, "p"), (g, "g"), (buf, "buf")):
+        _chk(t, torch.float32, n)
+    _chk(wp, torch.bfloat16, "wp")
+    _chk(table_dev, torch.int64, "table")
+    n_gaps = 0 if gaps_dev is None else int(gaps_dev.shape[0])
+    if n_gaps:
+        _chk(gaps_dev, torch.int64, "gaps")
+    L = _lib.lib()
+    if torch.is_tensor(hyper_or_lr):
+        _chk(hyper_or_lr, torch.float32, "hyper")
+        check(L.mi_sgd_step_pack_dev(_p(p), _p(g), _p(buf), p.numel(), _p(hyper_or_lr), _p(sflat), _p(wp), _p(wpt), _p(table_dev), int(n_desc),
+                                     int(total_blocks), _p(gaps_dev) if n_gaps else None, n_gaps, _stream()), "mi_sgd_step_pack_dev")
+    else:
+        check(L.mi_sgd_step_pack(_p(p), _p(g), _p(buf), p.numel(), float(hyper_or_lr), float(momentum), float(weight_decay), _p(sflat), _p(wp), _p(wpt),
+                                 _p(table_dev), int(n_desc), int(total_blocks), _p(gaps_dev) if n_gaps else None, n_gaps, _stream()), "mi_sgd_step_pack")
 
 
 def relu_mask(x, msk, out=None):
```

New measurement: 305.6 images/s, median of 6. +1.2%, better.
